# polli-labs/linnaeus

Measured on AMD Instinct MI355X. Metric: images/sec (train fwd+bwd) mFormerV1_sm 3x224x224, higher is better.
Workload: dtype bf16; 1 GPU; mFormerV1_sm train step (forward + 4-task CE loss + backward + AdamW (one HIP launch)), bf16 operands / fp32 accumulate+residual, batch 256/GPU, 3x224x224 synthetic, DropPath 0.2, gradient checkpointing off; per_gpu_batch=256, global_batch=256, parallelism=dp1, grad_mode=direct

## Files before the change

include/lnx.h:

```cpp
#ifndef LNX_H
#define LNX_H
#include <stdint.h>

#ifdef __cplusplus
extern "C" {
#endif

#define LNX_F32 0
#define LNX_BF16 1

const char* lnx_last_error(void);
int lnx_version(void);
int lnx_device_cus(void);
int lnx_set_cu_margin(int cus);

typedef struct lnx_rowmap {
    int group, pad, off;
} lnx_rowmap;

enum { LNX_ACT_NONE = 0, LNX_ACT_GELU = 1, LNX_ACT_RELU = 2, LNX_ACT_GELU_BWD = 3, LNX_ACT_RELU_BWD = 4,
       LNX_ACT_GELU_D = 5, LNX_ACT_MUL_AUX = 6 };
enum { LNX_ADDR_PLAIN = 0, LNX_ADDR_PATCH2 = 1 };

typedef struct lnx_gemm_args {
// ... 238 lines not shown
    int B, Cin, H, W, Cout;
    float eps;
} lnx_stem_args;
int lnx_stem_fwd_ok(int dtype, int Cin, int H, int W, int Cout);
int lnx_stem_fwd(const lnx_stem_args* args, void* stream);

int lnx_scale_cast(const float* in, int64_t ldin, lnx_rowmap in_map, const float* rowscale, int rows_per_sample, void* out,
                   int out_dtype, int64_t ldout, int M, int C, void* stream);

int lnx_layerscale_bwd(const float* g, const void* z, int dtype, const float* gamma, const float* rowscale,
                       int rows_per_sample, void* dz, float* dgamma, int M, int C, void* stream);

int lnx_layerscale_apply_wgrad(const float* s, const float* t, int64_t lds, const float* w, const float* b, int64_t ldw, const float* gamma, float* dw, float* db,
                               int64_t lddw, float* dgamma, int C, int K, void* stream);

int lnx_dropout_mul(void* x, int dtype, const unsigned char* mask, float inv_keep, int M, int C, void* stream);
int lnx_dropout_residual(const void* z, int z_dtype, const unsigned char* mask, float inv_keep, const float* rowscale, int rows_per_sample,
                         const float* res, float* out, int M, int C, void* stream);

int lnx_fill_rows(const float* vec, float* out, int64_t ldout, lnx_rowmap map, int M, int C, void* stream);
int lnx_colsum_rows(const float* in, int64_t ldin, lnx_rowmap map, float* out, int M, int C, void* stream);

int lnx_agg2_fwd(const float* a, const float* b, const float* w2, const float* bias1, float* out, int M, int C, void* stream);
int lnx_agg2_bwd(const float* dout, const float* a, const float* b, const float* w2, float* da, float* db_, float* dw2,
                 float* dbias1, int M, int C, void* stream);

int lnx_pack_meta(const float* meta, int width, int off, int dim, void* out, int dtype, int B, void* stream);

typedef struct lnx_meta_head_args {
    int B, C;
    int dim, off;
    const float* meta;
    int meta_width;
    float eps;
    const float* w0;
    int ldw0;
    const float *b0, *ln0_w, *ln0_b;
    const float* w1;
    int ldw1;
    const float *b1, *ln1_w, *ln1_b;
    const float* w2;
    int ldw2;
    const float *b2, *ln2_w, *ln2_b;
    float* t0;
    float *h0, *x, *h1, *n1, *h2;
    float *m0, *r0, *m1, *r1, *m2, *r2;
    float* tok;
    int64_t tok_row_stride, tok_row_offset;
} lnx_meta_head_args;
int lnx_meta_heads_supported(int C);
int lnx_meta_heads_fwd(const lnx_meta_head_args* heads, int n_heads, void* stream);

typedef struct lnx_meta_head_bwd_args {
    int B, C, dim;
    const float* g;
    int64_t g_row_stride, g_row_offset;
    const float* w1t;
    int ldw1t;
    const float* w2t;
    int ldw2t;
    const float *ln0_w, *ln1_w, *ln2_w;
    const float *t0, *h0, *x, *h1, *n1, *h2, *m0, *r0, *m1, *r1, *m2, *r2;
    float *dp2, *dp1, *dp0;
    float* part;
    float* d_w0;
    float *d_b0, *d_ln0_w, *d_ln0_b;
    float* d_w1;
    float *d_b1, *d_ln1_w, *d_ln1_b;
    float* d_w2;
    float *d_b2, *d_ln2_w, *d_ln2_b;
} lnx_meta_head_bwd_args;
int64_t lnx_meta_heads_bwd_part_floats(int B, int C);
int lnx_meta_heads_bwd(const lnx_meta_head_bwd_args* heads, int n_heads, void* stream);

enum { LNX_PREP_CAST = 0, LNX_PREP_CONV_PERM = 1, LNX_PREP_DW49 = 2 };
typedef struct lnx_prep_desc {
    const float* src;
    void* dst;
    void* dst_t;
    int rows, cols;
    int ld, ld_t;
    int P;
    int mode;
    int block_start;
} lnx_prep_desc;
int lnx_prep_weights(const lnx_prep_desc* descs_dev, int ndesc, int total_blocks, int dtype, void* stream);
int lnx_prep_blocks(int rows, int ld, int cols, int ld_t, int has_t);



typedef struct lnx_softce_args {
    int B, C;
    const float* logits;
    int64_t ld;
    const int64_t* target;
    const float* soft;
    float smoothing;
    const float* class_weight;
    int64_t ignore_index;
    const float* row_scale;
    float scale;
    float* loss;
    float* loss_sum;
    float* dlogits;
    int64_t ldd;
} lnx_softce_args;
int lnx_softce(const lnx_softce_args* args, void* stream);
#define LNX_SOFTCE_MAX_TASKS 8
int lnx_softce_multi(const lnx_softce_args* args, int n, void* stream);

typedef struct lnx_mix_args {
    const float* x;
    const int64_t* perm;
    const unsigned char* valid;
    float* out;
    int B;
    int64_t row;
    int H, W;
    float lam;
    int h0, h1, w0, w1;
    int mode;
} lnx_mix_args;
int lnx_mix_rows(const lnx_mix_args* args, void* stream);
int lnx_mix_meta(const float* aux, const unsigned char* mask, const int64_t* perm, const float* pick, const int* bounds_dev, int nchunk, int B, int D,
                 float* out_aux, unsigned char* out_mask, void* stream);

enum {
    LNX_AUG_CLAMP = 0,
    LNX_AUG_POSTERIZE = 1,
    LNX_AUG_SOLARIZE = 2,
    LNX_AUG_SOLARIZE_ADD = 3,
    LNX_AUG_INVERT = 4,
    LNX_AUG_BRIGHTNESS = 5,
    LNX_AUG_CONTRAST = 6
};
int lnx_aug_pointwise(float* x, int64_t n, int64_t per_image, int op, float p0, float p1, const float* per_image_scalar, void* stream);
int lnx_aug_saturation(float* x, int B, int64_t hw, float factor, void* stream);
int lnx_aug_rowstat(const float* x, int rows, int64_t cols, int kind, float* out, void* stream);
int lnx_aug_rescale(float* x, int64_t rows, int64_t cols, const float* minmax, void* stream);
int lnx_aug_affine(const float* x, float* y, int planes, int H, int W, const float* m6, void* stream);
int lnx_aug_stencil(const float* x, float* y, int planes, int H, int W, const float* taps_dev, int k, int mode, float ratio, void* stream);
int lnx_erase_rects(float* x, int B, int C, int H, int W, const int* rects_dev, const float* values_dev, int n_rects, void* stream);
int lnx_u8hwc_to_f32chw(const unsigned char* src, float* dst, int B, int H, int W, int C, void* stream);

#define LNX_ADAMW_MAX_GROUPS 16
typedef struct lnx_adamw_desc {
    float* p;
    float* m;
    float* v;
    const float* g;
    int64_t n;
    int group;
    int block_start;
} lnx_adamw_desc;
typedef struct lnx_adamw_hyper {
    int ngroups;
    float lr[LNX_ADAMW_MAX_GROUPS], beta1[LNX_ADAMW_MAX_GROUPS], beta2[LNX_ADAMW_MAX_GROUPS], eps[LNX_ADAMW_MAX_GROUPS],
        weight_decay[LNX_ADAMW_MAX_GROUPS];
    float bias_c1[LNX_ADAMW_MAX_GROUPS], bias_c2[LNX_ADAMW_MAX_GROUPS];
    float omb1[LNX_ADAMW_MAX_GROUPS], omb2[LNX_ADAMW_MAX_GROUPS];
} lnx_adamw_hyper;
int lnx_adamw_blocks(int64_t numel);
int lnx_grad_sumsq(const lnx_adamw_desc* descs_dev, int ndesc, int total_blocks, float* out, float* ws, void* stream);
int lnx_adamw_step(const lnx_adamw_desc* descs_dev, int ndesc, int total_blocks, const lnx_adamw_hyper* hyper, const float* sumsq, float max_norm,
                   void* stream);

typedef struct lnx_ademamix_hyper {
    int ngroups;
    float lr[LNX_ADAMW_MAX_GROUPS], beta1[LNX_ADAMW_MAX_GROUPS], beta2[LNX_ADAMW_MAX_GROUPS], eps[LNX_ADAMW_MAX_GROUPS],
        weight_decay[LNX_ADAMW_MAX_GROUPS];
    float bias_c1[LNX_ADAMW_MAX_GROUPS], bias_c2[LNX_ADAMW_MAX_GROUPS];
    float omb1[LNX_ADAMW_MAX_GROUPS], omb2[LNX_ADAMW_MAX_GROUPS];
    float alpha_t[LNX_ADAMW_MAX_GROUPS], beta3_t[LNX_ADAMW_MAX_GROUPS], omb3[LNX_ADAMW_MAX_GROUPS];
} lnx_ademamix_hyper;
int lnx_ademamix_step(const lnx_adamw_desc* descs_dev, float* const* slow_dev, int ndesc, int total_blocks, const lnx_ademamix_hyper* hyper,
                      const float* sumsq, float max_norm, void* stream);

int lnx_gradnorm_sumsq(const lnx_adamw_desc* descs_dev, int ndesc, int total_blocks, int ntasks, int64_t task_stride, float* sumsq, float* norm,
                       float* ws, void* stream);
typedef struct lnx_gradnorm_args {
    int T;
    float alpha;
    const float* norm;
    const float* loss_sum;
    const float* count;
    const float* init_loss;
    float* weights;
    float* initial_losses;
    int* initted;
    float* metrics;
} lnx_gradnorm_args;
int lnx_gradnorm_update(const lnx_gradnorm_args* args, void* stream);

enum { LNX_METRICS_CHAIN_N = 0, LNX_METRICS_CHAIN_CORRECT, LNX_METRICS_PARTIAL_N, LNX_METRICS_PARTIAL_CORRECT, LNX_METRICS_SUBSET_OOR ,
       LNX_METRICS_HEAD = 8 };
enum { LNX_METRICS_N = 0, LNX_METRICS_CORRECT1, LNX_METRICS_CORRECT3, LNX_METRICS_NULL_N, LNX_METRICS_NULL_CORRECT1, LNX_METRICS_NONNULL_N,
       LNX_METRICS_NONNULL_CORRECT1, LNX_METRICS_LOSS_N, LNX_METRICS_TASK_STRIDE = 8 };
enum { LNX_METRICS_SUM_LOSS = 0, LNX_METRICS_SUM_NULL_LOSS, LNX_METRICS_SUM_NONNULL_LOSS, LNX_METRICS_SUM_STRIDE = 4 };
#define LNX_METRICS_TASK(t) (LNX_METRICS_HEAD + LNX_METRICS_TASK_STRIDE * (t))
#define LNX_METRICS_SUBSET(n_tasks, n_bins0, s) (LNX_METRICS_TASK(n_tasks) + ((s) ? 2 * (int64_t)(n_tasks) * (n_bins0) : 0))
#define LNX_METRICS_SUM(t) (LNX_METRICS_SUM_STRIDE * (t))
typedef struct lnx_metrics_task {
    const void* logits;
    int64_t ld;
    const int64_t* target;
    const unsigned char* is_null;
    const float* loss;
    int C;
} lnx_metrics_task;
typedef struct lnx_metrics_args {
    int dtype;
    int B, n_tasks;
    lnx_metrics_task task[LNX_SOFTCE_MAX_TASKS];
    const int64_t* subset_ids[2];
    int n_bins[2];
    int64_t* counts;
    double* sums;
} lnx_metrics_args;
int lnx_metrics_table_sizes(int n_tasks, int n_bins0, int n_bins1, int64_t* n_counts, int64_t* n_sums);
int lnx_metrics_update(const lnx_metrics_args* args, void* stream);

#define LNX_PREDICT_MAX_K 16
typedef struct lnx_predict_task {
    const void* logits;
    int64_t ld;
    int C;
    const int32_t* parent;
    int null_index;
    const int64_t* id_map;
} lnx_predict_task;
typedef struct lnx_predict_args {
    int dtype;
    int B, n_tasks;
    int K;
    int consistency;
    const int32_t* k_per_sample;
    lnx_predict_task task[LNX_SOFTCE_MAX_TASKS];
    int64_t* ids;
    float* probs;
    int32_t* count;
    int32_t* flags;
} lnx_predict_args;
int lnx_predict(const lnx_predict_args* args, void* stream);

int lnx_convmlp_supported(int dtype, int C);
typedef struct lnx_convmlp_args {
    int dtype, M, C;
    const void* ln;
    const void* w1;
    const float* b1;
    const void* w2;
    const float* b2;
    const float* gamma;
    const float* rowscale;
    int rows_per_sample;
    const float* x;
    float* out;
    void* z;
    const void* y;
    const float* ln_w;
    const float* ln_b;
    float ln_eps;
    void* ln_out;
    float* mean;
    float* rstd;
} lnx_convmlp_args;
int lnx_convmlp_fwd(const lnx_convmlp_args* args, void* stream);

typedef struct lnx_convmlp_bwd_args {
    int dtype, M, C;
    const float* g;
    const void* ln;
    const void* z;
    const void* w1;
    const float* b1;
    const void* w2t;
    const void* w1t;
    const float* gamma;
    const float* rowscale;
    int rows_per_sample;
    void* act;
    void* dh;
    void* dz;
    void* dln;
    float* dgamma;
    const void* y;
    const float* ln_w;
    const float* mean;
    const float* rstd;
    float* d_ln_w;
    float* d_ln_b;
    float* ws;
    int64_t ws_floats;
    int dz_plain;
    int ln_defer;
} lnx_convmlp_bwd_args;
int lnx_convmlp_bwd(const lnx_convmlp_bwd_args* args, void* stream);
int64_t lnx_convmlp_bwd_ws_floats(int C, int M);


#define LNX_MAX_META 8
#define LNX_MAX_TASKS 16
typedef struct lnx_mformer_cfg {
    int dtype;
    int batch, img_h, img_w, in_chans;
    int dims[4];
    int conv_depths[2];
    int rope_depths[2];
    int rope_heads[2];
    int mlp_hidden[2];
    int n_meta;
    int meta_dims[LNX_MAX_META];
    int only_last_cls;
    int n_tasks;
    int task_classes[LNX_MAX_TASKS];
    int inference;
    int recompute;
    int fp8;
    int rope_mode;
} lnx_mformer_cfg;

typedef struct lnx_plan lnx_plan;
int lnx_plan_create(const lnx_mformer_cfg* cfg, lnx_plan** out);
void lnx_plan_destroy(lnx_plan* p);
int64_t lnx_plan_workspace_bytes(const lnx_plan* p);
int lnx_plan_num_params(const lnx_plan* p);
const char* lnx_plan_param_name(const lnx_plan* p, int i);
int64_t lnx_plan_param_numel(const lnx_plan* p, int i);
int lnx_plan_num_drop_calls(const lnx_plan* p);
int64_t lnx_plan_logits_numel(const lnx_plan* p);
int64_t lnx_plan_logits_offset(const lnx_plan* p, int task);
int lnx_plan_logits_ld(const lnx_plan* p, int task);
int lnx_plan_bind(lnx_plan* p, const float* const* params, float* const* grads, void* workspace);
int lnx_plan_forward(lnx_plan* p, const float* x, const float* meta, const float* drop_scales, const unsigned char* drop_mask,
                     float* feats, float* logits, void* stream);
int64_t lnx_plan_dropout_bytes(const lnx_plan* p);
int lnx_plan_set_dropout(lnx_plan* p, const unsigned char* masks, float drop_rate);
int64_t lnx_plan_attn_dropout_bytes(const lnx_plan* p);
int lnx_plan_set_attn_dropout(lnx_plan* p, const unsigned char* masks, float drop_rate);
int lnx_plan_backward(lnx_plan* p, const float* dlogits, const float* dfeats, int segment, void* stream);
int lnx_plan_backward_into(lnx_plan* p, const float* dlogits, const float* dfeats, float* const* grads, void* stream);
#define LNX_PROFILE_CLASSES 8
int lnx_plan_profile_begin(lnx_plan* p);
int lnx_plan_profile_end(lnx_plan* p, double* ms, double* work, int* launches);
#define LNX_PROFILE_CLASSES_EX 10
int lnx_plan_profile_begin_spans(lnx_plan* p);
int lnx_plan_profile_end_ex(lnx_plan* p, double* ms, double* work, double* bytes, int* launches);
int lnx_plan_set_wgrad_stream(lnx_plan* p, int on);
int lnx_plan_set_meta_stream(lnx_plan* p, int mode);
int lnx_plan_segment_params(const lnx_plan* p, int segment, int* idx_out, int max_out);

#ifdef __cplusplus
}
#endif
#endif
```

linnaeus_amd/_lib.py:

```python
from __future__ import annotations

import ctypes as C
import os

_HERE = os.path.dirname(os.path.abspath(__file__))
LIB_PATH = os.environ.get("LNX_LIB_PATH") or os.path.join(_HERE, "liblnx_hip.so")

F32, BF16 = 0, 1
ACT_NONE, ACT_GELU, ACT_RELU, ACT_GELU_BWD, ACT_RELU_BWD, ACT_GELU_D, ACT_MUL_AUX = 0, 1, 2, 3, 4, 5, 6
TN_WS_FLOATS = 256 * (256 * 128 + 256)
ADDR_PLAIN, ADDR_PATCH2 = 0, 1


class LnxError(RuntimeError):
    pass


class RowMap(C.Structure):
    _fields_ = [("group", C.c_int), ("pad", C.c_int), ("off", C.c_int)]


class GemmArgs(C.Structure):
    _fields_ = [
        ("dtype", C.c_int), ("M", C.c_int), ("N", C.c_int), ("K", C.c_int),
        ("A", C.c_void_p), ("lda", C.c_int64),
        ("W", C.c_void_p), ("ldw", C.c_int64),
        ("C", C.c_void_p), ("ldc", C.c_int64),
        ("out_f32", C.c_int),
        ("a_mode", C.c_int), ("Hin", C.c_int), ("Win", C.c_int), ("Cin", C.c_int),
        ("c_mode", C.c_int), ("c_map", RowMap),
        ("bias", C.c_void_p),
        ("c2", C.c_void_p), ("ldc2", C.c_int64),
        ("act", C.c_int),
        ("aux", C.c_void_p), ("ldaux", C.c_int64),
        ("gamma", C.c_void_p), ("rowscale", C.c_void_p), ("rows_per_sample", C.c_int),
        ("res", C.c_void_p), ("ldres", C.c_int64),
        ("c8", C.c_void_p), ("ldc8", C.c_int64), ("c8_scales", C.c_void_p),
    ]


class WgradArgs(C.Structure):
    _fields_ = [
        ("dtype", C.c_int), ("M", C.c_int), ("N", C.c_int), ("K", C.c_int),
        ("dY", C.c_void_p), ("lddy", C.c_int64),
        ("A", C.c_void_p), ("lda", C.c_int64),
        ("a_mode", C.c_int), ("Hin", C.c_int), ("Win", C.c_int), ("Cin", C.c_int),
        ("dW", C.c_void_p), ("lddw", C.c_int64),
        ("k_perm_c", C.c_int),
        ("db", C.c_void_p),
        ("splits", C.c_int),
        ("k_store", C.c_int),
        ("ws", C.c_void_p), ("ws_floats", C.c_int64),
        ("defer", C.c_int),
    ]


class SoftCEArgs(C.Structure):
    _fields_ = [
        ("B", C.c_int), ("C", C.c_int),
        ("logits", C.c_void_p), ("ld", C.c_int64),
        ("target", C.c_void_p),
        ("soft", C.c_void_p), ("smoothing", C.c_float),
        ("class_weight", C.c_void_p),
        ("ignore_index", C.c_int64),
        ("row_scale", C.c_void_p), ("scale", C.c_float),
        ("loss", C.c_void_p), ("loss_sum", C.c_void_p),
        ("dlogits", C.c_void_p), ("ldd", C.c_int64),
    ]


ADAMW_MAX_GROUPS = 16


class AdamWDesc(C.Structure):
    _fields_ = [("p", C.c_void_p), ("m", C.c_void_p), ("v", C.c_void_p), ("g", C.c_void_p), ("n", C.c_int64), ("group", C.c_int), ("block_start", C.c_int)]


class AdamWHyper(C.Structure):
    _fields_ = [("ngroups", C.c_int)] + [(k, C.c_float * ADAMW_MAX_GROUPS) for k in ("lr", "beta1", "beta2", "eps", "weight_decay", "bias_c1", "bias_c2", "omb1", "omb2")]


class AdEMAMixHyper(C.Structure):
    _fields_ = [("ngroups", C.c_int)] + [(k, C.c_float * ADAMW_MAX_GROUPS) for k in ("lr", "beta1", "beta2", "eps", "weight_decay", "bias_c1", "bias_c2", "omb1", "omb2",
                                                                                  "alpha_t", "beta3_t", "omb3")]


class GradNormArgs(C.Structure):
    _fields_ = [("T", C.c_int), ("alpha", C.c_float), ("norm", C.c_void_p), ("loss_sum", C.c_void_p), ("count", C.c_void_p), ("init_loss", C.c_void_p),
                ("weights", C.c_void_p), ("initial_losses", C.c_void_p), ("initted", C.c_void_p), ("metrics", C.c_void_p)]


METRICS_MAX_TASKS = 8
METRICS_CHAIN_N, METRICS_CHAIN_CORRECT, METRICS_PARTIAL_N, METRICS_PARTIAL_CORRECT, METRICS_SUBSET_OOR = range(5)
METRICS_HEAD = 8
METRICS_N, METRICS_CORRECT1, METRICS_CORRECT3, METRICS_NULL_N, METRICS_NULL_CORRECT1, METRICS_NONNULL_N, METRICS_NONNULL_CORRECT1, METRICS_LOSS_N = range(8)
METRICS_TASK_STRIDE = 8
METRICS_SUM_LOSS, METRICS_SUM_NULL_LOSS, METRICS_SUM_NONNULL_LOSS = range(3)
METRICS_SUM_STRIDE = 4


def metrics_task(t: int) -> int:
    return METRICS_HEAD + METRICS_TASK_STRIDE * t


def metrics_subset(n_tasks: int, n_bins0: int, s: int) -> int:
    return metrics_task(n_tasks) + (2 * n_tasks * n_bins0 if s else 0)


class MetricsTask(C.Structure):
    _fields_ = [("logits", C.c_void_p), ("ld", C.c_int64), ("target", C.c_void_p), ("is_null", C.c_void_p), ("loss", C.c_void_p), ("C", C.c_int)]


class MetricsArgs(C.Structure):
    _fields_ = [("dtype", C.c_int), ("B", C.c_int), ("n_tasks", C.c_int), ("task", MetricsTask * METRICS_MAX_TASKS),
                ("subset_ids", C.c_void_p * 2), ("n_bins", C.c_int * 2), ("counts", C.c_void_p), ("sums", C.c_void_p)]


PREDICT_MAX_K = 16


class PredictTask(C.Structure):
    _fields_ = [("logits", C.c_void_p), ("ld", C.c_int64), ("C", C.c_int), ("parent", C.c_void_p), ("null_index", C.c_int), ("id_map", C.c_void_p)]


class PredictArgs(C.Structure):
    _fields_ = [("dtype", C.c_int), ("B", C.c_int), ("n_tasks", C.c_int), ("K", C.c_int), ("consistency", C.c_int), ("k_per_sample", C.c_void_p),
                ("task", PredictTask * METRICS_MAX_TASKS), ("ids", C.c_void_p), ("probs", C.c_void_p), ("count", C.c_void_p), ("flags", C.c_void_p)]


_lib = None


def lib() -> C.CDLL:
    global _lib
    if _lib is None:
        if not os.path.exists(LIB_PATH):
            raise LnxError(
                f"{LIB_PATH} is missing: build it with `python -c 'import __graft_entry__ as g; g.build()'` "
                "(or `make -C linnaeus_amd/csrc`). linnaeus_amd has no CPU fallback."
            )
        _lib = C.CDLL(LIB_PATH)
        _lib.lnx_last_error.restype = C.c_char_p
        _lib.lnx_nt_kernel_launches.restype = C.c_int64
        _lib.lnx_convmlp_bwd_ws_floats.restype = C.c_int64
        _lib.lnx_meta_heads_bwd_part_floats.restype = C.c_int64
        if hasattr(_lib, "lnx_ademamix_step"):
            _lib.lnx_ademamix_step.argtypes = [C.c_void_p, C.c_void_p, C.c_int, C.c_int, C.POINTER(AdEMAMixHyper), C.c_void_p, C.c_float, C.c_void_p]
        if hasattr(_lib, "lnx_gradnorm_sumsq"):
            _lib.lnx_gradnorm_sumsq.argtypes = [C.c_void_p, C.c_int, C.c_int, C.c_int, C.c_int64, C.c_void_p, C.c_void_p, C.c_void_p, C.c_void_p]
        if hasattr(_lib, "lnx_metrics_update"):
            _lib.lnx_metrics_update.argtypes = [C.POINTER(MetricsArgs), C.c_void_p]
            _lib.lnx_metrics_table_sizes.argtypes = [C.c_int, C.c_int, C.c_int, C.POINTER(C.c_int64), C.POINTER(C.c_int64)]
        if hasattr(_lib, "lnx_predict"):
            _lib.lnx_predict.argtypes = [C.POINTER(PredictArgs), C.c_void_p]
            _lib.lnx_predict.restype = C.c_int
        older = bool(os.environ.get("LNX_LIB_PATH")) and os.environ.get("LNX_LIB_OLDER") == "1"
        for name in EXPORTS:
            if not hasattr(_lib, name) and not older:
                raise LnxError(f"{LIB_PATH} does not export {name}; rebuild it")
    return _lib


def check(rc: int, what: str) -> None:
    if rc != 0:
        raise LnxError(f"{what} failed (rc={rc}): {lib().lnx_last_error().decode()}")


AUG_CLAMP, AUG_POSTERIZE, AUG_SOLARIZE, AUG_SOLARIZE_ADD, AUG_INVERT, AUG_BRIGHTNESS, AUG_CONTRAST = range(7)

NT_KERNEL_NONE, NT_KERNEL_V1, NT_KERNEL_V2, NT_KERNEL_SKINNY, NT_KERNEL_V4, NT_KERNEL_FP8, NT_KERNEL_V7, NT_KERNEL_MX8, NT_KERNEL_V9, NT_KERNEL_EXPERIMENT = 0, 1, 2, 3, 4, 6, 7, 8, 9, 15

ROPE_COS, ROPE_ROTATE = 0, 1

ATTN_KERNEL_NONE, ATTN_KERNEL_RES4, ATTN_KERNEL_RES8, ATTN_KERNEL_TILED4, ATTN_KERNEL_TILED8 = range(5)

EXPORTS = [
    "lnx_last_error", "lnx_version", "lnx_device_cus", "lnx_set_cu_margin",
    "lnx_gemm_nt", "lnx_last_nt_kernel", "lnx_nt_kernel_launches", "lnx_nt_dispatch", "lnx_gemm_tn", "lnx_gemm_tn_flush", "lnx_gemm_tn_discard", "lnx_amax", "lnx_quantize_fp8", "lnx_gemm_nt_fp8", "lnx_quantize_mxfp8", "lnx_gemm_nt_mxfp8", "lnx_dropout_mul", "lnx_dropout_residual", "lnx_plan_dropout_bytes", "lnx_plan_set_dropout", "lnx_plan_attn_dropout_bytes", "lnx_plan_set_attn_dropout",
    "lnx_layernorm_fwd", "lnx_layernorm_bwd", "lnx_layernorm_bwd_flush", "lnx_layernorm_bwd_discard",
    "lnx_dwconv7_fwd", "lnx_dwconv7_wgrad",
    "lnx_gemm_nt_group_ok", "lnx_gemm_nt_group", "lnx_rope_cos_table", "lnx_rope_cos_table_hd", "lnx_rope_cossin_table_hd", "lnx_rope_cos_tables", "lnx_attn_bwd_ws_floats", "lnx_attn_bwd_ws_floats_hd", "lnx_attn_fwd", "lnx_attn_bwd", "lnx_attn_bwd_flush", "lnx_attn_bwd_discard", "lnx_attn_dispatch", "lnx_last_attn_kernel",
    "lnx_im2col_stem", "lnx_scale_cast", "lnx_layerscale_bwd", "lnx_layerscale_apply_wgrad", "lnx_fill_rows", "lnx_colsum_rows",
    "lnx_agg2_fwd", "lnx_agg2_bwd", "lnx_pack_meta", "lnx_meta_heads_supported", "lnx_meta_heads_fwd", "lnx_meta_heads_bwd", "lnx_meta_heads_bwd_part_floats", "lnx_prep_weights", "lnx_prep_blocks", "lnx_softce", "lnx_softce_multi", "lnx_stem_fwd", "lnx_stem_fwd_ok", "lnx_adamw_blocks", "lnx_grad_sumsq", "lnx_adamw_step", "lnx_ademamix_step", "lnx_gradnorm_sumsq", "lnx_gradnorm_update",
    "lnx_metrics_table_sizes", "lnx_metrics_update", "lnx_predict",
    "lnx_mix_rows", "lnx_mix_meta",
    "lnx_aug_pointwise", "lnx_aug_saturation", "lnx_aug_rowstat", "lnx_aug_rescale", "lnx_aug_affine", "lnx_aug_stencil", "lnx_erase_rects", "lnx_u8hwc_to_f32chw",
    "lnx_convmlp_supported", "lnx_convmlp_fwd", "lnx_convmlp_bwd", "lnx_convmlp_bwd_ws_floats",
    "lnx_plan_create", "lnx_plan_destroy", "lnx_plan_workspace_bytes", "lnx_plan_num_params", "lnx_plan_param_name",
    "lnx_plan_param_numel", "lnx_plan_num_drop_calls", "lnx_plan_logits_numel", "lnx_plan_logits_offset", "lnx_plan_logits_ld",
    "lnx_plan_bind", "lnx_plan_forward", "lnx_plan_backward", "lnx_plan_backward_into", "lnx_plan_segment_params", "lnx_plan_profile_begin", "lnx_plan_profile_end", "lnx_plan_profile_begin_spans", "lnx_plan_profile_end_ex", "lnx_plan_set_wgrad_stream", "lnx_plan_set_meta_stream",
]


class MetaHeadArgs(C.Structure):
    _fields_ = [
        ("B", C.c_int), ("C", C.c_int), ("dim", C.c_int), ("off", C.c_int),
        ("meta", C.c_void_p), ("meta_width", C.c_int), ("eps", C.c_float),
        ("w0", C.c_void_p), ("ldw0", C.c_int), ("b0", C.c_void_p), ("ln0_w", C.c_void_p), ("ln0_b", C.c_void_p),
        ("w1", C.c_void_p), ("ldw1", C.c_int), ("b1", C.c_void_p), ("ln1_w", C.c_void_p), ("ln1_b", C.c_void_p),
        ("w2", C.c_void_p), ("ldw2", C.c_int), ("b2", C.c_void_p), ("ln2_w", C.c_void_p), ("ln2_b", C.c_void_p),
        ("t0", C.c_void_p), ("h0", C.c_void_p), ("x", C.c_void_p), ("h1", C.c_void_p), ("n1", C.c_void_p), ("h2", C.c_void_p),
        ("m0", C.c_void_p), ("r0", C.c_void_p), ("m1", C.c_void_p), ("r1", C.c_void_p), ("m2", C.c_void_p), ("r2", C.c_void_p),
        ("tok", C.c_void_p), ("tok_row_stride", C.c_int64), ("tok_row_offset", C.c_int64),
    ]


class MetaHeadBwdArgs(C.Structure):
    _fields_ = [
        ("B", C.c_int), ("C", C.c_int), ("dim", C.c_int),
        ("g", C.c_void_p), ("g_row_stride", C.c_int64), ("g_row_offset", C.c_int64),
        ("w1t", C.c_void_p), ("ldw1t", C.c_int), ("w2t", C.c_void_p), ("ldw2t", C.c_int),
        ("ln0_w", C.c_void_p), ("ln1_w", C.c_void_p), ("ln2_w", C.c_void_p),
        ("t0", C.c_void_p), ("h0", C.c_void_p), ("x", C.c_void_p), ("h1", C.c_void_p), ("n1", C.c_void_p), ("h2", C.c_void_p),
        ("m0", C.c_void_p), ("r0", C.c_void_p), ("m1", C.c_void_p), ("r1", C.c_void_p), ("m2", C.c_void_p), ("r2", C.c_void_p),
        ("dp2", C.c_void_p), ("dp1", C.c_void_p), ("dp0", C.c_void_p), ("part", C.c_void_p),
        ("d_w0", C.c_void_p), ("d_b0", C.c_void_p), ("d_ln0_w", C.c_void_p), ("d_ln0_b", C.c_void_p),
        ("d_w1", C.c_void_p), ("d_b1", C.c_void_p), ("d_ln1_w", C.c_void_p), ("d_ln1_b", C.c_void_p),
        ("d_w2", C.c_void_p), ("d_b2", C.c_void_p), ("d_ln2_w", C.c_void_p), ("d_ln2_b", C.c_void_p),
    ]


class LnArgs(C.Structure):
    _fields_ = [
        ("M", C.c_int), ("C", C.c_int), ("eps", C.c_float),
        ("x", C.c_void_p), ("x_dtype", C.c_int), ("ldx", C.c_int64), ("x_map", RowMap),
        ("w", C.c_void_p), ("b", C.c_void_p),
        ("y", C.c_void_p), ("y_dtype", C.c_int), ("ldy", C.c_int64), ("y_map", RowMap),
        ("add", C.c_void_p), ("ldadd", C.c_int64),
        ("mean", C.c_void_p), ("rstd", C.c_void_p),
        ("y8", C.c_void_p), ("ldy8", C.c_int64), ("y8_scales", C.c_void_p),
    ]


class LnBwdArgs(C.Structure):
    _fields_ = [
        ("M", C.c_int), ("C", C.c_int),
        ("dy", C.c_void_p), ("dy_dtype", C.c_int), ("lddy", C.c_int64), ("dy_map", RowMap),
        ("x", C.c_void_p), ("x_dtype", C.c_int), ("ldx", C.c_int64), ("x_map", RowMap),
        ("w", C.c_void_p), ("mean", C.c_void_p), ("rstd", C.c_void_p),
        ("gin", C.c_void_p), ("ldgin", C.c_int64),
        ("dx", C.c_void_p), ("dx_dtype", C.c_int), ("lddx", C.c_int64),
        ("dw", C.c_void_p), ("db", C.c_void_p), ("relu_mask", C.c_int),
        ("ws", C.c_void_p), ("ws_floats", C.c_int64),
        ("dx2", C.c_void_p), ("dx2_dtype", C.c_int), ("lddx2", C.c_int64), ("dx2_rowscale", C.c_void_p), ("dx2_rows_per_sample", C.c_int),
        ("dx2_8", C.c_void_p), ("dx2_8_scales", C.c_void_p), ("lddx2_8", C.c_int64),
        ("defer", C.c_int),
    ]


class RopeTable(C.Structure):
    _fields_ = [
        ("freqs", C.c_void_p), ("cos_out", C.c_void_p), ("dsin_out", C.c_void_p),
        ("heads", C.c_int), ("H", C.c_int), ("W", C.c_int), ("head_dim", C.c_int),
        ("rope_mode", C.c_int), ("sin_out", C.c_void_p),
    ]


class DwconvArgs(C.Structure):
    _fields_ = [
        ("B", C.c_int), ("H", C.c_int), ("W", C.c_int), ("C", C.c_int),
        ("x", C.c_void_p), ("x_dtype", C.c_int), ("w49", C.c_void_p), ("bias", C.c_void_p),
        ("flip", C.c_int), ("res", C.c_void_p), ("y", C.c_void_p), ("y_dtype", C.c_int),
    ]


class DwconvWgradArgs(C.Structure):
    _fields_ = [
        ("B", C.c_int), ("H", C.c_int), ("W", C.c_int), ("C", C.c_int),
        ("x", C.c_void_p), ("x_dtype", C.c_int), ("dy", C.c_void_p), ("dy_dtype", C.c_int),
        ("dw", C.c_void_p), ("db", C.c_void_p),
    ]


class AttnArgs(C.Structure):
    _fields_ = [
        ("dtype", C.c_int), ("B", C.c_int), ("N", C.c_int), ("E", C.c_int), ("heads", C.c_int),
        ("qkv", C.c_void_p), ("cos_tab", C.c_void_p), ("o", C.c_void_p), ("lse", C.c_void_p),
        ("drop_mask", C.c_void_p), ("drop_inv_keep", C.c_float), ("head_dim", C.c_int),
        ("rope_mode", C.c_int), ("sin_tab", C.c_void_p),
    ]


class AttnBwdArgs(C.Structure):
    _fields_ = [
        ("dtype", C.c_int), ("B", C.c_int), ("N", C.c_int), ("E", C.c_int), ("heads", C.c_int),
        ("qkv", C.c_void_p), ("cos_tab", C.c_void_p), ("o", C.c_void_p), ("lse", C.c_void_p),
        ("d_o", C.c_void_p), ("dqkv", C.c_void_p), ("freq_ws", C.c_void_p), ("delta", C.c_void_p),
        ("drop_mask", C.c_void_p), ("drop_inv_keep", C.c_float),
        ("dsin_tab", C.c_void_p), ("dfreqs", C.c_void_p), ("defer_freqs", C.c_int), ("head_dim", C.c_int),
        ("rope_mode", C.c_int), ("sin_tab", C.c_void_p), ("grid_w", C.c_int),
    ]


class PrepDesc(C.Structure):
    _fields_ = [
        ("src", C.c_void_p), ("dst", C.c_void_p), ("dst_t", C.c_void_p),
        ("rows", C.c_int), ("cols", C.c_int), ("ld", C.c_int), ("ld_t", C.c_int),
        ("P", C.c_int), ("mode", C.c_int), ("block_start", C.c_int),
    ]


PREP_CAST, PREP_CONV_PERM, PREP_DW49 = 0, 1, 2


class ConvMlpArgs(C.Structure):
    _fields_ = [
        ("dtype", C.c_int), ("M", C.c_int), ("C", C.c_int),
        ("ln", C.c_void_p), ("w1", C.c_void_p), ("b1", C.c_void_p), ("w2", C.c_void_p), ("b2", C.c_void_p),
        ("gamma", C.c_void_p), ("rowscale", C.c_void_p), ("rows_per_sample", C.c_int),
        ("x", C.c_void_p), ("out", C.c_void_p), ("z", C.c_void_p),
        ("y", C.c_void_p), ("ln_w", C.c_void_p), ("ln_b", C.c_void_p), ("ln_eps", C.c_float), ("ln_out", C.c_void_p),
        ("mean", C.c_void_p), ("rstd", C.c_void_p),
    ]


class ConvMlpBwdArgs(C.Structure):
    _fields_ = [
        ("dtype", C.c_int), ("M", C.c_int), ("C", C.c_int),
        ("g", C.c_void_p), ("ln", C.c_void_p), ("z", C.c_void_p), ("w1", C.c_void_p), ("b1", C.c_void_p),
        ("w2t", C.c_void_p), ("w1t", C.c_void_p), ("gamma", C.c_void_p), ("rowscale", C.c_void_p), ("rows_per_sample", C.c_int),
        ("act", C.c_void_p), ("dh", C.c_void_p), ("dz", C.c_void_p), ("dln", C.c_void_p), ("dgamma", C.c_void_p),
        ("y", C.c_void_p), ("ln_w", C.c_void_p), ("mean", C.c_void_p), ("rstd", C.c_void_p), ("d_ln_w", C.c_void_p), ("d_ln_b", C.c_void_p),
        ("ws", C.c_void_p), ("ws_floats", C.c_int64),
        ("dz_plain", C.c_int), ("ln_defer", C.c_int),
    ]


class StemArgs(C.Structure):
    _fields_ = [("x", C.c_void_p), ("w", C.c_void_p), ("bias", C.c_void_p), ("ln_w", C.c_void_p), ("ln_b", C.c_void_p), ("patches", C.c_void_p),
                ("pre", C.c_void_p), ("y", C.c_void_p), ("mean", C.c_void_p), ("rstd", C.c_void_p), ("B", C.c_int), ("Cin", C.c_int), ("H", C.c_int),
                ("W", C.c_int), ("Cout", C.c_int), ("eps", C.c_float)]


class MixArgs(C.Structure):
    _fields_ = [
        ("x", C.c_void_p), ("perm", C.c_void_p), ("valid", C.c_void_p), ("out", C.c_void_p),
        ("B", C.c_int), ("row", C.c_int64), ("H", C.c_int), ("W", C.c_int), ("lam", C.c_float),
        ("h0", C.c_int), ("h1", C.c_int), ("w0", C.c_int), ("w1", C.c_int), ("mode", C.c_int),
    ]
```

linnaeus_amd/csrc/optim.hip:

```cpp
#include "common.hpp"
#include "../../include/lnx.h"

namespace {

constexpr int OPT_ELEMS = 4096;

__device__ __forceinline__ int find_desc_index(const lnx_adamw_desc* __restrict__ descs, int ndesc, int block) {
    int lo = 0, hi = ndesc - 1;
    while (lo < hi) {
        const int mid = (lo + hi + 1) >> 1;
        if (descs[mid].block_start <= block) lo = mid;
        else hi = mid - 1;
    }
    return lo;
}

__device__ __forceinline__ const lnx_adamw_desc& find_desc(const lnx_adamw_desc* __restrict__ descs, int ndesc, int block) {
    return descs[find_desc_index(descs, ndesc, block)];
}

__global__ __launch_bounds__(256) void grad_sumsq_kernel(const lnx_adamw_desc* __restrict__ descs, int ndesc, float* __restrict__ part) {
    __shared__ float red[4];
    const lnx_adamw_desc& d = find_desc(descs, ndesc, blockIdx.x);
    const int64_t base = (int64_t)(blockIdx.x - d.block_start) * OPT_ELEMS;
    const int64_t end = min(d.n, base + OPT_ELEMS);
    float s = 0.f;
    if ((reinterpret_cast<uintptr_t>(d.g) & 15) == 0) {
        for (int64_t i = base + 4 * threadIdx.x; i + 3 < end; i += 1024) {
            const float4 v = *reinterpret_cast<const float4*>(d.g + i);
            s += v.x * v.x + v.y * v.y + v.z * v.z + v.w * v.w;
        }
        const int64_t tail = base + ((end - base) & ~(int64_t)3);
        if (tail + threadIdx.x < end) {
            const float v = d.g[tail + threadIdx.x];
            s += v * v;
        }
    } else {
        for (int64_t i = base + threadIdx.x; i < end; i += 256) s += d.g[i] * d.g[i];
    }
    s = wave_sum(s);
    if ((threadIdx.x & 63) == 0) red[threadIdx.x >> 6] = s;
    __syncthreads();
    if (threadIdx.x == 0) part[blockIdx.x] = (red[0] + red[1]) + (red[2] + red[3]);
}

__global__ __launch_bounds__(1024) void grad_sumsq_fold_kernel(const float* __restrict__ part, int n, float* __restrict__ out) {
    __shared__ float red[16];
    float s0 = 0.f, s1 = 0.f, s2 = 0.f, s3 = 0.f;
    int i = threadIdx.x;
    for (; i + 3 * 1024 < n; i += 4 * 1024) {
        s0 += part[i];
        s1 += part[i + 1024];
        s2 += part[i + 2048];
        s3 += part[i + 3072];
    }
    for (; i < n; i += 1024) s0 += part[i];
    float s = wave_sum((s0 + s1) + (s2 + s3));
    if ((threadIdx.x & 63) == 0) red[threadIdx.x >> 6] = s;
    __syncthreads();
    if (threadIdx.x == 0) {
        float t = 0.f;
#pragma unroll
        for (int k = 0; k < 16; ++k) t += red[k];
        *out = t;
    }
}

__global__ __launch_bounds__(256) void adamw_kernel(const lnx_adamw_desc* __restrict__ descs, int ndesc, const lnx_adamw_hyper h, const float* __restrict__ sumsq,
                                                    float max_norm) {
    const lnx_adamw_desc& d = find_desc(descs, ndesc, blockIdx.x);
    const int gi = d.group;
    const float lr = h.lr[gi], b1 = h.beta1[gi], b2 = h.beta2[gi], eps = h.eps[gi], wd = h.weight_decay[gi];
    const float omb1 = h.omb1[gi], omb2 = h.omb2[gi];
    const float step_size = lr / h.bias_c1[gi], inv_sqrt_bc2 = 1.0f / sqrtf(h.bias_c2[gi]);
    float coef = 1.0f;
    if (sumsq != nullptr && max_norm > 0.f) coef = fminf(1.0f, max_norm / (sqrtf(*sumsq) + 1e-6f));
    const int64_t base = (int64_t)(blockIdx.x - d.block_start) * OPT_ELEMS;
    const int64_t end = min(d.n, base + OPT_ELEMS);
    auto upd = [&](float g, float& p, float& m, float& v) __attribute__((always_inline)) {
        g *= coef;
        p *= 1.0f - lr * wd;
        m = fmaf(b1, m, omb1 * g);
        v = fmaf(b2, v, omb2 * g * g);
        const float denom = sqrtf(v) * inv_sqrt_bc2 + eps;
        p -= step_size * (m / denom);
    };
    const bool vec = ((reinterpret_cast<uintptr_t>(d.p) | reinterpret_cast<uintptr_t>(d.g) | reinterpret_cast<uintptr_t>(d.m) | reinterpret_cast<uintptr_t>(d.v)) & 15) == 0;
    int64_t done = base;
    if (vec) {
        constexpr int R = OPT_ELEMS / 1024;
        float4 g4[R], p4[R], m4[R], v4[R];
        const int64_t full = base + ((end - base) & ~(int64_t)3);
#pragma unroll
        for (int r = 0; r < R; ++r) {
            const int64_t i = base + 1024 * r + 4 * threadIdx.x;
            const int64_t ic = i + 3 < full ? i : base;
            if (full > base) {
                g4[r] = *reinterpret_cast<const float4*>(d.g + ic);
                p4[r] = *reinterpret_cast<const float4*>(d.p + ic);
                m4[r] = *reinterpret_cast<const float4*>(d.m + ic);
                v4[r] = *reinterpret_cast<const float4*>(d.v + ic);
            }
        }
        if (full > base) {
#pragma unroll
            for (int r = 0; r < R; ++r) {
                const int64_t i = base + 1024 * r + 4 * threadIdx.x;
                if (i + 3 < full) {
                    upd(g4[r].x, p4[r].x, m4[r].x, v4[r].x);
                    upd(g4[r].y, p4[r].y, m4[r].y, v4[r].y);
                    upd(g4[r].z, p4[r].z, m4[r].z, v4[r].z);
                    upd(g4[r].w, p4[r].w, m4[r].w, v4[r].w);
                    *reinterpret_cast<float4*>(d.p + i) = p4[r];
                    *reinterpret_cast<float4*>(d.m + i) = m4[r];
                    *reinterpret_cast<float4*>(d.v + i) = v4[r];
                }
            }
        }
        done = full;
    }
    for (int64_t i = done + threadIdx.x; i < end; i += 256) {
        float p = d.p[i], m = d.m[i], v = d.v[i];
        upd(d.g[i], p, m, v);
        d.p[i] = p;
        d.m[i] = m;
        d.v[i] = v;
    }
}

__global__ __launch_bounds__(256) void ademamix_kernel(const lnx_adamw_desc* __restrict__ descs, float* const* __restrict__ slow, int ndesc,
                                                       const lnx_ademamix_hyper h, const float* __restrict__ sumsq, float max_norm) {
    const int di = find_desc_index(descs, ndesc, blockIdx.x);
    const lnx_adamw_desc& d = descs[di];
    float* const m3p = slow[di];
    const int gi = d.group;
    const float lr = h.lr[gi], b1 = h.beta1[gi], b2 = h.beta2[gi], eps = h.eps[gi], nlrwd = -(lr * h.weight_decay[gi]);
    const float omb1 = h.omb1[gi], omb2 = h.omb2[gi], b3 = h.beta3_t[gi], omb3 = h.omb3[gi], alpha = h.alpha_t[gi];
    const float step_size = lr / h.bias_c1[gi], sqrt_bc2 = sqrtf(h.bias_c2[gi]);
    float coef = 1.0f;
    if (sumsq != nullptr && max_norm > 0.f) coef = fminf(1.0f, max_norm / (sqrtf(*sumsq) + 1e-6f));
    const int64_t base = (int64_t)(blockIdx.x - d.block_start) * OPT_ELEMS;
    const int64_t end = min(d.n, base + OPT_ELEMS);
    auto upd = [&](float g, float& p, float& m, float& v, float& s) __attribute__((always_inline)) {
        g *= coef;
        p = fmaf(nlrwd, p, p);
        m = fmaf(b1, m, omb1 * g);
        v = fmaf(b2, v, omb2 * g * g);
        s = fmaf(b3, s, omb3 * g);
        const float denom = sqrtf(v) / sqrt_bc2 + eps;
        p -= step_size * (fmaf(alpha, s, m) / denom);
    };
    const bool vec = ((reinterpret_cast<uintptr_t>(d.p) | reinterpret_cast<uintptr_t>(d.g) | reinterpret_cast<uintptr_t>(d.m) | reinterpret_cast<uintptr_t>(d.v) |
                       reinterpret_cast<uintptr_t>(m3p)) & 15) == 0;
    int64_t done = base;
    if (vec) {
        constexpr int R = OPT_ELEMS / 1024;
        float4 g4[R], p4[R], m4[R], v4[R], s4[R];
        const int64_t full = base + ((end - base) & ~(int64_t)3);
#pragma unroll
        for (int r = 0; r < R; ++r) {
            const int64_t i = base + 1024 * r + 4 * threadIdx.x;
            const int64_t ic = i + 3 < full ? i : base;
            if (full > base) {
                g4[r] = *reinterpret_cast<const float4*>(d.g + ic);
                p4[r] = *reinterpret_cast<const float4*>(d.p + ic);
                m4[r] = *reinterpret_cast<const float4*>(d.m + ic);
                v4[r] = *reinterpret_cast<const float4*>(d.v + ic);
                s4[r] = *reinterpret_cast<const float4*>(m3p + ic);
            }
        }
        if (full > base) {
#pragma unroll
            for (int r = 0; r < R; ++r) {
                const int64_t i = base + 1024 * r + 4 * threadIdx.x;
                if (i + 3 < full) {
                    upd(g4[r].x, p4[r].x, m4[r].x, v4[r].x, s4[r].x);
                    upd(g4[r].y, p4[r].y, m4[r].y, v4[r].y, s4[r].y);
                    upd(g4[r].z, p4[r].z, m4[r].z, v4[r].z, s4[r].z);
                    upd(g4[r].w, p4[r].w, m4[r].w, v4[r].w, s4[r].w);
                    *reinterpret_cast<float4*>(d.p + i) = p4[r];
                    *reinterpret_cast<float4*>(d.m + i) = m4[r];
                    *reinterpret_cast<float4*>(d.v + i) = v4[r];
                    *reinterpret_cast<float4*>(m3p + i) = s4[r];
                }
            }
        }
        done = full;
    }
    for (int64_t i = done + threadIdx.x; i < end; i += 256) {
        float p = d.p[i], m = d.m[i], v = d.v[i], s = m3p[i];
        upd(d.g[i], p, m, v, s);
        d.p[i] = p;
        d.m[i] = m;
        d.v[i] = v;
        m3p[i] = s;
    }
}

}

extern "C" int lnx_adamw_blocks(int64_t numel) { return (int)((numel + OPT_ELEMS - 1) / OPT_ELEMS); }

extern "C" int lnx_grad_sumsq(const lnx_adamw_desc* descs_dev, int ndesc, int total_blocks, float* out, float* ws, void* stream) {
    LNX_CHECK(descs_dev && ndesc > 0 && total_blocks > 0 && out && ws, "lnx_grad_sumsq: bad arguments (ws: total_blocks floats)");
    hipStream_t st = (hipStream_t)stream;
    hipLaunchKernelGGL(grad_sumsq_kernel, dim3(total_blocks), dim3(256), 0, st, descs_dev, ndesc, ws);
    hipLaunchKernelGGL(grad_sumsq_fold_kernel, dim3(1), dim3(1024), 0, st, ws, total_blocks, out);
    LNX_LAUNCH_CHECK();
    return 0;
}

extern "C" int lnx_adamw_step(const lnx_adamw_desc* descs_dev, int ndesc, int total_blocks, const lnx_adamw_hyper* hyper, const float* sumsq, float max_norm,
                              void* stream) {
    LNX_CHECK(descs_dev && ndesc > 0 && total_blocks > 0 && hyper, "lnx_adamw_step: bad arguments");
    LNX_CHECK(hyper->ngroups > 0 && hyper->ngroups <= LNX_ADAMW_MAX_GROUPS, "lnx_adamw_step: ngroups=%d (max %d)", hyper->ngroups, LNX_ADAMW_MAX_GROUPS);
    for (int i = 0; i < hyper->ngroups; ++i)
        LNX_CHECK(hyper->bias_c1[i] > 0.f && hyper->bias_c2[i] > 0.f, "lnx_adamw_step: bias corrections of group %d must be positive (step >= 1)", i);
    hipLaunchKernelGGL(adamw_kernel, dim3(total_blocks), dim3(256), 0, (hipStream_t)stream, descs_dev, ndesc, *hyper, sumsq, max_norm);
    LNX_LAUNCH_CHECK();
    return 0;
}

extern "C" int lnx_ademamix_step(const lnx_adamw_desc* descs_dev, float* const* slow_dev, int ndesc, int total_blocks, const lnx_ademamix_hyper* hyper,
                                 const float* sumsq, float max_norm, void* stream) {
    LNX_CHECK(descs_dev && slow_dev && ndesc > 0 && total_blocks > 0 && hyper, "lnx_ademamix_step: bad arguments");
    LNX_CHECK(hyper->ngroups > 0 && hyper->ngroups <= LNX_ADAMW_MAX_GROUPS, "lnx_ademamix_step: ngroups=%d (max %d)", hyper->ngroups, LNX_ADAMW_MAX_GROUPS);
    for (int i = 0; i < hyper->ngroups; ++i)
        LNX_CHECK(hyper->bias_c1[i] > 0.f && hyper->bias_c2[i] > 0.f, "lnx_ademamix_step: bias corrections of slot %d must be positive (step >= 1)", i);
    hipLaunchKernelGGL(ademamix_kernel, dim3(total_blocks), dim3(256), 0, (hipStream_t)stream, descs_dev, slow_dev, ndesc, *hyper, sumsq, max_norm);
    LNX_LAUNCH_CHECK();
    return 0;
}
```

linnaeus_amd/csrc/plan.cpp:

```cpp
#include <hip/hip_runtime.h>
#include <stdlib.h>
#include <string.h>

#include <mutex>
#include <atomic>
#include <string>
#include <vector>

#include "../../include/lnx.h"

void lnx_set_error(const char* fmt, ...);

#define RUN(expr)                  \
    do {                           \
        const int rc_ = (expr);    \
        if (rc_ != 0) return rc_;  \
    } while (0)
#define FAIL(...)                   \
    do {                            \
        lnx_set_error(__VA_ARGS__); \
        return 1;                   \
    } while (0)
#define HIPRUN(expr)                                                         \
    do {                                                                     \
        const hipError_t e_ = (expr);                                        \
        if (e_ != hipSuccess) FAIL("%s: %s", #expr, hipGetErrorString(e_)); \
    } while (0)

namespace {

constexpr int LN_DEFER_SLOTS = 16;
constexpr int FREQ_DEFER_SLOTS = 8;

inline int64_t align_up(int64_t v, int64_t a) { return (v + a - 1) / a * a; }

struct OpW {
    int param = -1;
    int N = 0, K = 0;
    int ld = 0;
    int ld_t = 0;
    int mode = LNX_PREP_CAST, P = 0;
    bool f32 = false;
    int64_t off = 0, off_t = 0;
    int64_t off8 = 0, off8s = 0;
    int64_t off8t = 0, off8ts = 0;
};

struct ConvBlk {
    bool fused = false;
    bool fused_ln = false;
    bool keep_z = true;
    int gamma, dww, dwb, lnw, lnb, b1, b2;
    OpW w1, w2;
    int64_t w49;
    int64_t xin, y, ln, mean, rstd, hpre, act, z;
};
struct RopeBlk {
    int n1w, n1b, n2w, n2b, freqs, qkvb, projb, fc1b, fc2b;
    OpW qkv, proj, fc1, fc2;
    int64_t xin, n1, mean1, rstd1, qkvbuf, cos, dsin, o, lse, xmid, n2, mean2, rstd2, hpre, act;
    int64_t dm_proj = 0, dm_hid = 0, dm_fc2 = 0;
    int64_t dm_attn = 0;
};
struct MetaHead {
    int b0, lnw0, lnb0, nf1w, nf1b, nf2w, nf2b, b1, b2;
    OpW w0, w1, w2;
    int dim, off;
    int64_t t0, h0, x, m0, r0, h1, n1, m1, r1, h2, m2, r2;
    int64_t dp2 = 0, dp1 = 0, dp0 = 0, part = 0;
};
struct Down {
    int lnw, lnb, cb;
    OpW w;
    int64_t ln, mean, rstd;
};

}

constexpr int TN_WS_SLOTS = 4;

struct lnx_plan {
    lnx_mformer_cfg c;
    int esz;
    int E;
    int H[4], W[4], HW[4];
    int N2, N3;
    std::vector<std::string> names;
    std::vector<int64_t> numel;
    std::vector<const float*> P;
    std::vector<float*> G;
    bool bound = false, has_grads = false, fwd_done = false;
    unsigned char* ws = nullptr;
    int64_t ws_bytes = 0;

    int stem_b, stem_lnw, stem_lnb, cls[2], norm_w[2], norm_b[2], fin_w, fin_b, agg_w, agg_b, cl_b1, cl_b2, cl_lnw, cl_lnb;
    OpW stem_w, cl_w1, cl_w2;
    std::vector<int> head_b;
    std::vector<OpW> head_w;
    std::vector<int> logit_ld;
    std::vector<int64_t> logit_off;
    int64_t logits_numel = 0;
    Down down[3];
    std::vector<ConvBlk> conv[2];
    std::vector<RopeBlk> rope[2];
    std::vector<MetaHead> meta[2];
    std::vector<OpW*> all_w;
    std::vector<int> drop_conv[2], drop_attn[2], drop_mlp[2];
    int n_drop = 0;

    int64_t o_descs = 0, n_descs = 0, prep_blocks = 0;
    int64_t n_descs_t = 0, n_descs_f = 0, prep_blocks_f = 0;
    int64_t o_patches, o_stem_pre, o_stem_mean, o_stem_rstd;
    int64_t o_stage_out[4];
    int64_t o_tok[2];
    int64_t o_t1, o_t1_mean, o_t1_rstd;
    int64_t o_cl_hpre, o_cl_act, o_cl_u, o_cl_mean, o_cl_rstd, o_c1n;
    int64_t o_c2n, o_n2_mean, o_n2_rstd, o_agg, o_fin_mean, o_fin_rstd, o_feats, o_featsT;
    int64_t o_g[4];
    int64_t o_sA, o_sB = 0, o_sC, o_sD;
    int64_t o_lnws = 0, lnws_floats = 0, o_lnws_side = 0, lnws_side_floats = 0;
    int64_t lnws_defer_floats = 0;
    int64_t o_lnws_defer = 0;
    int ln_pending = 0;
    int64_t gcos_floats = 0;
    int freq_pending = 0;
    bool freq_defer = true;
    bool ln_defer = true;
    int64_t o_tnws = 0;
    int64_t o_lsws = 0, lsws_floats = 0;
    int64_t o_gcos , o_delta, o_dt1, o_tail[6], o_mtmp[4], o_dlT;
    int64_t o_a8 = 0, o_a8s = 0, o_h8 = 0, o_h8s = 0;
    const float* last_drop = nullptr;
    const unsigned char* last_mask = nullptr;
    std::vector<unsigned char> mask_host;
    const float* last_meta = nullptr;
    int resident[4] = {-1, -1, -1, -1};
    const unsigned char* dmask = nullptr;
    float inv_keep = 1.0f;
    int64_t dmask_bytes = 0;
    const unsigned char* amask = nullptr;
    float a_inv_keep = 1.0f;
    int64_t amask_bytes = 0;
    hipStream_t side = nullptr;
    hipEvent_t ev_fork = nullptr, ev_meta = nullptr, ev_bfork[2] = {nullptr, nullptr}, ev_bjoin[2] = {nullptr, nullptr};
    hipStream_t wgs = nullptr;
    bool wgs_on = true;
    bool meta_forked[2] = {false, false};
    int meta_mode = 1;
    bool meta_chain = true;
    bool chain_ok[2] = {false, false};
    bool dy8_ready = false;
    hipEvent_t ev_wf[4] = {nullptr, nullptr, nullptr, nullptr}, ev_wj[4] = {nullptr, nullptr, nullptr, nullptr};
    bool profile = false;
    bool profile_spans = false;
    struct Span { hipEvent_t e0, e1; int cls; double work, bytes; };
    std::vector<Span> spans;
    std::vector<hipEvent_t> ev_pool;
    size_t ev_used = 0;

    template <typename U> U* at(int64_t off) const { return reinterpret_cast<U*>(ws + off); }
    const float* drop_ptr(int call) const {
        if (last_drop == nullptr || call < 0 || !mask_host[call]) return nullptr;
        return last_drop + (int64_t)call * c.batch;
    }
};

namespace {

int find_param(const lnx_plan* p, const std::string& n) {
    for (size_t i = 0; i < p->names.size(); ++i)
        if (p->names[i] == n) return (int)i;
    return -1;
}

void add_param(lnx_plan* p, const std::string& n, int64_t numel) {
    p->names.push_back(n);
    p->numel.push_back(numel);
}

void build_inventory(lnx_plan* p) {
    const lnx_mformer_cfg& c = p->c;
    const int* D = c.dims;
    char b[128];
    add_param(p, "cls_token_1", D[2]);
    add_param(p, "cls_token_2", D[3]);
    add_param(p, "stem.0.weight", (int64_t)D[0] * c.in_chans * 16);
    add_param(p, "stem.0.bias", D[0]);
    add_param(p, "stem.1.weight", D[0]);
    add_param(p, "stem.1.bias", D[0]);
    for (int i = 0; i < 3; ++i) {
        snprintf(b, sizeof b, "downsample_layers.%d.", i);
        const std::string pre(b);
        add_param(p, pre + "norm.weight", D[i]);
        add_param(p, pre + "norm.bias", D[i]);
        add_param(p, pre + "conv.weight", (int64_t)D[i + 1] * D[i] * 4);
        add_param(p, pre + "conv.bias", D[i + 1]);
    }
    for (int s = 0; s < 2; ++s)
        for (int i = 0; i < c.conv_depths[s]; ++i) {
            snprintf(b, sizeof b, "stages.%d.%d.", s, i);
            const std::string pre(b);
            const int64_t C = D[s];
            add_param(p, pre + "gamma", C);
            add_param(p, pre + "dwconv.weight", C * 49);
            add_param(p, pre + "dwconv.bias", C);
            add_param(p, pre + "norm.weight", C);
            add_param(p, pre + "norm.bias", C);
            add_param(p, pre + "pwconv1.weight", 4 * C * C);
            add_param(p, pre + "pwconv1.bias", 4 * C);
            add_param(p, pre + "pwconv2.weight", 4 * C * C);
            add_param(p, pre + "pwconv2.bias", C);
        }
    for (int s = 0; s < 2; ++s)
        for (int i = 0; i < c.rope_depths[s]; ++i) {
            snprintf(b, sizeof b, "stages.%d.%d.", s + 2, i);
            const std::string pre(b);
            const int64_t C = D[2 + s], hid = c.mlp_hidden[s];
            add_param(p, pre + "norm1.weight", C);
            add_param(p, pre + "norm1.bias", C);
            add_param(p, pre + "norm2.weight", C);
            add_param(p, pre + "norm2.bias", C);
            add_param(p, pre + "attn.freqs", C);
            add_param(p, pre + "attn.qkv.weight", 3 * C * C);
            add_param(p, pre + "attn.qkv.bias", 3 * C);
            add_param(p, pre + "attn.proj.weight", C * C);
            add_param(p, pre + "attn.proj.bias", C);
            add_param(p, pre + "mlp.fc1.weight", hid * C);
            add_param(p, pre + "mlp.fc1.bias", hid);
            add_param(p, pre + "mlp.fc2.weight", C * hid);
            add_param(p, pre + "mlp.fc2.bias", C);
        }
    add_param(p, "norm_1.weight", D[2]);
    add_param(p, "norm_1.bias", D[2]);
    add_param(p, "norm_2.weight", D[3]);
    add_param(p, "norm_2.bias", D[3]);
    for (int m = 0; m < c.n_meta; ++m)
        for (int s = 0; s < 2; ++s) {
            snprintf(b, sizeof b, "meta.%d.head_%d.", m, s + 1);
            const std::string pre(b);
            const int64_t C = D[2 + s];
            add_param(p, pre + "0.weight", C * c.meta_dims[m]);
            add_param(p, pre + "0.bias", C);
            add_param(p, pre + "2.weight", C);
            add_param(p, pre + "2.bias", C);
            add_param(p, pre + "3.norm_fn1.weight", C);
            add_param(p, pre + "3.norm_fn1.bias", C);
            add_param(p, pre + "3.norm_fn2.weight", C);
            add_param(p, pre + "3.norm_fn2.bias", C);
            add_param(p, pre + "3.w1.weight", C * C);
            add_param(p, pre + "3.w1.bias", C);
            add_param(p, pre + "3.w2.weight", C * C);
            add_param(p, pre + "3.w2.bias", C);
        }
    if (!c.only_last_cls) {
        add_param(p, "cl_1_fc.0.fc1.weight", (int64_t)D[2] * D[2]);
        add_param(p, "cl_1_fc.0.fc1.bias", D[2]);
        add_param(p, "cl_1_fc.0.fc2.weight", (int64_t)D[3] * D[2]);
        add_param(p, "cl_1_fc.0.fc2.bias", D[3]);
        add_param(p, "cl_1_fc.1.weight", D[3]);
        add_param(p, "cl_1_fc.1.bias", D[3]);
        add_param(p, "aggregate.weight", 2);
        add_param(p, "aggregate.bias", 1);
    }
    add_param(p, "final_norm.weight", D[3]);
// ... 413 lines not shown
        }
        p->o_lnws_side = cv.take(p->lnws_side_floats * 4);
        p->o_tnws = cv.take((int64_t)LNX_TN_WS_FLOATS * 4 * TN_WS_SLOTS);
        {
            const int64_t cmax = D[0] > D[1] ? D[0] : D[1];
            p->lsws_floats = cmax * 4 * cmax + cmax;
            p->o_lsws = cv.take(p->lsws_floats * 4);
        }
        p->o_sA = cv.take(maxM4C * esz);
        if (any_fused) p->o_sB = cv.take(maxM4C * esz);
        p->o_sC = cv.take(maxMC * esz);
        p->o_sD = cv.take(maxMC * esz);
    }
    if (!inf) {
        int64_t gmax = 0, dmax = 0;
        for (int s = 0; s < 2; ++s) {
            const int N = s == 0 ? p->N2 : p->N3;
            const int64_t gsz = lnx_attn_bwd_ws_floats_hd(B, N, c.rope_heads[s], D[2 + s] / c.rope_heads[s]) * 4;
            const int64_t dsz = (int64_t)B * c.rope_heads[s] * N * 4;
            if (gsz > gmax) gmax = gsz;
            if (dsz > dmax) dmax = dsz;
        }
        p->gcos_floats = gmax / 4;
        p->o_gcos = cv.take(gmax * FREQ_DEFER_SLOTS);
        p->o_delta = cv.take(dmax);
    }
    for (int s = 0; s < 2; ++s) {
        const int64_t M = (int64_t)B * (s == 0 ? p->N2 : p->N3), C = D[2 + s], hid = c.mlp_hidden[s];
        for (auto& k : p->rope[s]) {
            k.dm_proj = p->dmask_bytes;
            k.dm_hid = k.dm_proj + M * C;
            k.dm_fc2 = k.dm_hid + M * hid;
            p->dmask_bytes = k.dm_fc2 + M * C;
            const int64_t N = s == 0 ? p->N2 : p->N3;
            k.dm_attn = p->amask_bytes;
            p->amask_bytes += (int64_t)B * c.rope_heads[s] * N * ((N + 63) / 64 * 64);
        }
    }
    p->ws_bytes = cv.cur;
    *out = p;
    return 0;
}

extern "C" int64_t lnx_plan_dropout_bytes(const lnx_plan* p) { return p ? p->dmask_bytes : 0; }
extern "C" int64_t lnx_plan_attn_dropout_bytes(const lnx_plan* p) { return p ? p->amask_bytes : 0; }

extern "C" int lnx_plan_set_attn_dropout(lnx_plan* p, const unsigned char* masks, float drop_rate) {
    if (!p) FAIL("lnx_plan_set_attn_dropout: null plan");
    if (masks == nullptr || drop_rate == 0.0f) {
        p->amask = nullptr;
        p->a_inv_keep = 1.0f;
        return 0;
    }
    if (!(drop_rate > 0.0f && drop_rate < 1.0f)) FAIL("lnx_plan_set_attn_dropout: drop_rate %g must be in [0, 1)", (double)drop_rate);
    if (p->c.inference) FAIL("lnx_plan_set_attn_dropout: dropout is a training-time operation; this is an inference plan");
    if ((((uintptr_t)masks) & 3) != 0) FAIL("lnx_plan_set_attn_dropout: the mask buffer must be 4-byte aligned");
    p->amask = masks;
    p->a_inv_keep = 1.0f / (1.0f - drop_rate);
    return 0;
}

extern "C" int lnx_plan_set_dropout(lnx_plan* p, const unsigned char* masks, float drop_rate) {
    if (!p) FAIL("lnx_plan_set_dropout: null plan");
    if (masks == nullptr || drop_rate == 0.0f) {
        p->dmask = nullptr;
        p->inv_keep = 1.0f;
        return 0;
    }
    if (!(drop_rate > 0.0f && drop_rate < 1.0f)) FAIL("lnx_plan_set_dropout: drop_rate %g must be in [0, 1)", (double)drop_rate);
    if (p->c.inference) FAIL("lnx_plan_set_dropout: dropout is a training-time operation; this is an inference plan");
    if (p->c.fp8) FAIL("lnx_plan_set_dropout: dropout is not available on fp8 plans");
    if ((((uintptr_t)masks) & 7) != 0) FAIL("lnx_plan_set_dropout: the mask buffer must be 8-byte aligned");
    p->dmask = masks;
    p->inv_keep = 1.0f / (1.0f - drop_rate);
    return 0;
}

static hipStream_t shared_stream(int which) {
    static std::mutex mu;
    static hipStream_t tab[2][64] = {};
    int dev = 0;
    if (hipGetDevice(&dev) != hipSuccess || dev < 0 || dev >= 64) return nullptr;
    std::lock_guard<std::mutex> lock(mu);
    if (!tab[which][dev] && hipStreamCreateWithFlags(&tab[which][dev], hipStreamNonBlocking) != hipSuccess) tab[which][dev] = nullptr;
    return tab[which][dev];
}

extern "C" void lnx_plan_destroy(lnx_plan* p) {
    if (!p) return;
    (void)lnx_gemm_tn_discard();
    (void)lnx_layernorm_bwd_discard();
    if (p->side) {
        (void)hipStreamSynchronize(p->side);
        (void)hipEventDestroy(p->ev_fork);
        (void)hipEventDestroy(p->ev_meta);
        for (int i = 0; i < 2; ++i) {
            (void)hipEventDestroy(p->ev_bfork[i]);
            (void)hipEventDestroy(p->ev_bjoin[i]);
        }
    }
    if (p->wgs) {
        (void)hipStreamSynchronize(p->wgs);
        for (int i = 0; i < 4; ++i) {
            (void)hipEventDestroy(p->ev_wf[i]);
            (void)hipEventDestroy(p->ev_wj[i]);
        }
    }
    for (hipEvent_t e : p->ev_pool) (void)hipEventDestroy(e);
    delete p;
}
extern "C" int64_t lnx_plan_workspace_bytes(const lnx_plan* p) { return p ? p->ws_bytes : 0; }
extern "C" int lnx_plan_num_params(const lnx_plan* p) { return p ? (int)p->names.size() : 0; }
extern "C" const char* lnx_plan_param_name(const lnx_plan* p, int i) {
    return (p && i >= 0 && i < (int)p->names.size()) ? p->names[i].c_str() : nullptr;
}
extern "C" int64_t lnx_plan_param_numel(const lnx_plan* p, int i) { return (p && i >= 0 && i < (int)p->numel.size()) ? p->numel[i] : -1; }
extern "C" int lnx_plan_num_drop_calls(const lnx_plan* p) { return p ? p->n_drop : 0; }
extern "C" int64_t lnx_plan_logits_numel(const lnx_plan* p) { return p ? p->logits_numel : 0; }
extern "C" int64_t lnx_plan_logits_offset(const lnx_plan* p, int t) { return (p && t >= 0 && t < p->c.n_tasks) ? p->logit_off[t] : -1; }
extern "C" int lnx_plan_logits_ld(const lnx_plan* p, int t) { return (p && t >= 0 && t < p->c.n_tasks) ? p->logit_ld[t] : -1; }

extern "C" int lnx_plan_bind(lnx_plan* p, const float* const* params, float* const* grads, void* workspace) {
    if (!p || !params || !workspace) FAIL("lnx_plan_bind: null argument");
    {
        static std::atomic<int> bound_dev{-1};
        int dev = -1;
        HIPRUN(hipGetDevice(&dev));
        int expect = -1;
        if (!bound_dev.compare_exchange_strong(expect, dev) && expect != dev)
            FAIL("lnx_plan_bind: this process already runs plans on device %d, now device %d is current: the library is one-process-per-GPU", expect, dev);
    }
    const int n = (int)p->names.size();
    p->P.assign(params, params + n);
    for (int i = 0; i < n; ++i)
        if (p->P[i] == nullptr || (((uintptr_t)p->P[i]) & 3) != 0) FAIL("lnx_plan_bind: parameter %s is null or misaligned", p->names[i].c_str());
    p->has_grads = grads != nullptr;
    if (grads) {
        p->G.assign(grads, grads + n);
        for (int i = 0; i < n; ++i)
            if (p->G[i] == nullptr) FAIL("lnx_plan_bind: gradient of %s is null", p->names[i].c_str());
    } else {
        p->G.assign(n, nullptr);
    }
    p->ws = reinterpret_cast<unsigned char*>(workspace);
    if ((((uintptr_t)p->ws) & 255) != 0) FAIL("lnx_plan_bind: workspace must be 256-byte aligned");
    int64_t arena_end = 0;
    for (OpW* w : p->all_w) {
        const int wes = w->f32 ? 4 : 2;
        const int64_t e1 = w->off + (int64_t)w->N * w->ld * wes;
        const int64_t e2 = w->ld_t ? w->off_t + (int64_t)w->K * w->ld_t * wes : 0;
        if (e1 > arena_end) arena_end = e1;
        if (e2 > arena_end) arena_end = e2;
    }
    HIPRUN(hipMemset(p->ws, 0, (size_t)arena_end));
    std::vector<lnx_prep_desc> d;
    int blk = 0;
    auto push_w = [&](OpW* w) {
        lnx_prep_desc e;
        memset(&e, 0, sizeof e);
        e.src = p->P[w->param];
        e.dst = p->ws + w->off;
        e.dst_t = w->ld_t ? p->ws + w->off_t : nullptr;
        e.rows = w->N;
        e.cols = w->K;
        e.ld = w->ld;
        e.ld_t = w->ld_t;
        e.P = w->P;
        e.mode = w->mode;
        e.block_start = blk;
        blk += lnx_prep_blocks(e.rows, e.ld, e.cols, e.ld_t, e.dst_t != nullptr);
        d.push_back(e);
    };
    const bool split = p->esz == 2;
    for (OpW* w : p->all_w)
        if (!split || !w->f32) push_w(w);
    for (int s = 0; s < 2; ++s)
        for (auto& k : p->conv[s]) {
            lnx_prep_desc e;
            memset(&e, 0, sizeof e);
            e.src = p->P[k.dww];
            e.dst = p->ws + k.w49;
            e.rows = p->c.dims[s];
            e.cols = 49;
            e.ld = 49;
            e.mode = LNX_PREP_DW49;
            e.block_start = blk;
            blk += lnx_prep_blocks(e.rows, e.ld, e.cols, 0, 0);
            d.push_back(e);
        }
    p->n_descs_t = (int64_t)d.size();
    p->prep_blocks = blk;
    blk = 0;
    if (split)
        for (OpW* w : p->all_w)
            if (w->f32) push_w(w);
    p->n_descs_f = (int64_t)d.size() - p->n_descs_t;
    p->prep_blocks_f = blk;
    if (getenv("LNX_NO_SIDE_STREAM") != nullptr) p->meta_mode = 0;
    if (const char* e = getenv("LNX_META_STREAM")) p->meta_mode = atoi(e) < 0 || atoi(e) > 2 ? 1 : atoi(e);
    if (p->side == nullptr && p->c.n_meta > 0 && getenv("LNX_NO_SIDE_STREAM") == nullptr) {
        p->side = shared_stream(0);
        if (!p->side) FAIL("lnx_plan: no side stream");
        HIPRUN(hipEventCreateWithFlags(&p->ev_fork, hipEventDisableTiming));
        HIPRUN(hipEventCreateWithFlags(&p->ev_meta, hipEventDisableTiming));
        for (int i = 0; i < 2; ++i) {
            HIPRUN(hipEventCreateWithFlags(&p->ev_bfork[i], hipEventDisableTiming));
            HIPRUN(hipEventCreateWithFlags(&p->ev_bjoin[i], hipEventDisableTiming));
        }
    }
    if (p->wgs == nullptr && !(getenv("LNX_WGRAD_STREAM") && atoi(getenv("LNX_WGRAD_STREAM")) == 0)) {
        p->wgs = shared_stream(1);
        if (!p->wgs) FAIL("lnx_plan: no weight-gradient stream");
        for (int i = 0; i < 4; ++i) {
            HIPRUN(hipEventCreateWithFlags(&p->ev_wf[i], hipEventDisableTiming));
            HIPRUN(hipEventCreateWithFlags(&p->ev_wj[i], hipEventDisableTiming));
        }
    }
    HIPRUN(hipMemcpy(p->ws + p->o_descs, d.data(), d.size() * sizeof(lnx_prep_desc), hipMemcpyHostToDevice));
    HIPRUN(hipDeviceSynchronize());
    p->bound = true;
    p->fwd_done = false;
    return 0;
}

namespace {

hipStream_t meta_stream(const lnx_plan* p) {
    if (p->c.n_meta <= 0 || p->meta_mode == 0) return nullptr;
    if (p->meta_mode == 2 && p->chain_ok[0] && p->chain_ok[1] && p->wgs != nullptr) return p->wgs;
    return p->side;
}

struct Ctx {
    lnx_plan* p;
    void* st;
    int dt;
    template <typename U> U* at(int64_t off) const { return p->at<U>(off); }
    const void* wptr(const OpW& w) const { return p->ws + w.off; }
    const void* wtptr(const OpW& w) const { return p->ws + w.off_t; }
};

hipEvent_t take_event(lnx_plan* p) {
    if (p->ev_used == p->ev_pool.size()) {
        hipEvent_t e;
        (void)hipEventCreate(&e);
        p->ev_pool.push_back(e);
    }
    return p->ev_pool[p->ev_used++];
}
struct Timed {
    lnx_plan* p;
    hipStream_t st;
    bool on;
    lnx_plan::Span sp;
    Timed(const Ctx& c, int cls, double work, double bytes = 0.0)
        : p(c.p), st((hipStream_t)c.st), on(cls >= 0 && (cls >= 8 ? c.p->profile_spans : (c.p->profile && !c.p->profile_spans))) {
        if (on) {
            sp.cls = cls;
            sp.work = work;
            sp.bytes = bytes;
            sp.e0 = take_event(p);
            sp.e1 = take_event(p);
            (void)hipEventRecord(sp.e0, st);
        }
    }
    ~Timed() {
        if (on) {
            (void)hipEventRecord(sp.e1, st);
            p->spans.push_back(sp);
        }
    }
};
double nt_bytes(const Ctx& c, const lnx_gemm_args* a, int a_elem = 0) {
    const double e = c.p->esz, ea = a_elem ? a_elem : e, mn = (double)a->M * a->N;
    return ea * ((double)a->M * a->K + (double)a->N * a->K) + (a->out_f32 ? 4.0 : e) * mn + (a->c2 ? e * mn : 0.0) + (a->aux ? e * mn : 0.0) +
           (a->res ? 4.0 * mn : 0.0) + (a->c8 ? mn * (1.0 + 1.0 / 32) : 0.0);
}
int gemm_nt_t(const Ctx& c, const lnx_gemm_args* a) {
    Timed t(c, a->M >= 1024 ? 0 : -1, 2.0 * a->M * a->N * a->K, nt_bytes(c, a));
    return lnx_gemm_nt(a, c.st);
}

int heads_nt(const Ctx& c, lnx_gemm_args* hg, int n, bool accumulate) {
    static const bool off = getenv("LNX_HEADS_GROUP") != nullptr && atoi(getenv("LNX_HEADS_GROUP")) == 0;
    int gmax = LNX_GEMM_GROUP_MAX;
    if (const char* e = getenv("LNX_HEADS_GROUP_MAX")) {
        const int v = atoi(e);
        if (v >= 1 && v < gmax) gmax = v;
    }
    for (int t0 = 0; t0 < n; t0 += gmax) {
        const int m = n - t0 < gmax ? n - t0 : gmax;
        lnx_gemm_args* g = hg + t0;
        if (accumulate && t0 > 0) {
            g[0].C = hg[0].C; g[0].ldc = hg[0].ldc; g[0].res = (const float*)hg[0].C; g[0].ldres = hg[0].ldc;
        }
        if (!off && lnx_gemm_nt_group_ok(g, m, accumulate ? 1 : 0)) {
            RUN(lnx_gemm_nt_group(g, m, accumulate ? 1 : 0, c.st));
            continue;
        }
        for (int t = 0; t < m; ++t) {
            lnx_gemm_args a = g[t];
            if (accumulate && t > 0) {
                a.C = g[0].C; a.ldc = g[0].ldc; a.res = (const float*)g[0].C; a.ldres = g[0].ldc;
            }
            RUN(gemm_nt_t(c, &a));
        }
    }
    return 0;
}

lnx_gemm_args gemm_base(const Ctx& c, int M, int N, int K, const void* A, int64_t lda, const void* W, int64_t ldw, void* C, int64_t ldc, bool out_f32) {
    lnx_gemm_args a;
    memset(&a, 0, sizeof a);
    a.dtype = c.dt;
    a.M = M;
    a.N = N;
    a.K = K;
    a.A = A;
    a.lda = lda;
    a.W = W;
    a.ldw = ldw;
    a.C = C;
    a.ldc = ldc;
    a.out_f32 = out_f32 ? 1 : 0;
    return a;
}

int ln_fwd(const Ctx& c, int M, int C, float eps, const void* x, int xdt, int64_t ldx, lnx_rowmap xm, int wi, int bi, void* y, int ydt, int64_t ldy,
           lnx_rowmap ym, const void* add, int64_t ldadd, float* mean, float* rstd, void* y8 = nullptr, void* y8s = nullptr) {
    lnx_ln_args a;
    memset(&a, 0, sizeof a);
    a.y8 = y8; a.ldy8 = C; a.y8_scales = y8s;
    a.M = M; a.C = C; a.eps = eps;
    a.x = x; a.x_dtype = xdt; a.ldx = ldx; a.x_map = xm;
    a.w = c.p->P[wi]; a.b = c.p->P[bi];
    a.y = y; a.y_dtype = ydt; a.ldy = ldy; a.y_map = ym;
    a.add = add; a.ldadd = ldadd; a.mean = mean; a.rstd = rstd;
    return lnx_layernorm_fwd(&a, c.st);
}

struct Dx2 {
    void* p = nullptr;
    const float* rowscale = nullptr;
    int rps = 0;
    void* p8 = nullptr;
    void* p8s = nullptr;
};
int ln_bwd(const Ctx& c, int M, int C, const void* dy, int dydt, int64_t lddy, lnx_rowmap dym, const void* x, int xdt, int64_t ldx, lnx_rowmap xm, int wi,
           int bi, const float* mean, const float* rstd, const float* gin, void* dx, int dxdt, int64_t lddx, bool relu, Dx2 d2 = Dx2()) {
    lnx_ln_bwd_args a;
    memset(&a, 0, sizeof a);
    a.dx2 = d2.p; a.dx2_dtype = c.dt; a.lddx2 = C; a.dx2_rowscale = d2.rowscale; a.dx2_rows_per_sample = d2.rps;
    if (d2.p && d2.p8) {
        a.dx2_8 = d2.p8; a.dx2_8_scales = d2.p8s; a.lddx2_8 = C;
    }
    a.M = M; a.C = C;
    a.dy = dy; a.dy_dtype = dydt; a.lddy = lddy; a.dy_map = dym;
    a.x = x; a.x_dtype = xdt; a.ldx = ldx; a.x_map = xm;
    a.w = c.p->P[wi]; a.mean = mean; a.rstd = rstd;
    a.gin = gin; a.ldgin = lddx;
    a.dx = dx; a.dx_dtype = dxdt; a.lddx = lddx;
    a.dw = c.p->G[wi]; a.db = c.p->G[bi];
    a.relu_mask = relu ? 1 : 0;
    const bool on_side = c.p->side != nullptr && c.st == (void*)c.p->side;
    a.ws = c.at<float>(on_side ? c.p->o_lnws_side : c.p->o_lnws);
    a.ws_floats = on_side ? c.p->lnws_side_floats : c.p->lnws_floats;
    lnx_plan* p = c.p;
    const bool on_wgs = p->wgs != nullptr && c.st == (void*)p->wgs;
    if (p->ln_defer && !on_side && !on_wgs && p->o_lnws_defer != 0 && (a.dw || a.db)) {
        if (p->ln_pending == LN_DEFER_SLOTS) {
            RUN(lnx_layernorm_bwd_flush(c.st));
            p->ln_pending = 0;
// ... 131 lines not shown
    g.bias = p->P[d.cb]; g.c_map = om;
    RUN(gemm_nt_t(c, &g));
    return 0;
}

int meta_head_fwd(const Ctx& cc, int s, int m, const float* meta, int meta_width, float* tok, int N) {
    const Ctx c{cc.p, cc.st, LNX_F32};
    lnx_plan* p = c.p;
    MetaHead& k = p->meta[s][m];
    const int B = p->c.batch, C = p->c.dims[2 + s];
    RUN(lnx_pack_meta(meta, meta_width, k.off, k.dim, c.at<void>(k.t0), c.dt, B, c.st));
    lnx_gemm_args g = gemm_base(c, B, C, 16, c.at<void>(k.t0), 16, c.wptr(k.w0), k.w0.ld, c.at<void>(k.h0), C, false);
    g.bias = p->P[k.b0]; g.act = LNX_ACT_RELU;
    RUN(gemm_nt_t(c, &g));
    RUN(ln_fwd(c, B, C, 1e-5f, c.at<void>(k.h0), c.dt, C, IDM, k.lnw0, k.lnb0, c.at<void>(k.x), c.dt, C, IDM, nullptr, 0, c.at<float>(k.m0), c.at<float>(k.r0)));
    g = gemm_base(c, B, C, C, c.at<void>(k.x), C, c.wptr(k.w1), k.w1.ld, c.at<void>(k.h1), C, false);
    g.bias = p->P[k.b1]; g.act = LNX_ACT_RELU;
    RUN(gemm_nt_t(c, &g));
    RUN(ln_fwd(c, B, C, 1e-5f, c.at<void>(k.h1), c.dt, C, IDM, k.nf1w, k.nf1b, c.at<void>(k.n1), c.dt, C, IDM, nullptr, 0, c.at<float>(k.m1), c.at<float>(k.r1)));
    g = gemm_base(c, B, C, C, c.at<void>(k.n1), C, c.wptr(k.w2), k.w2.ld, c.at<void>(k.h2), C, false);
    g.bias = p->P[k.b2]; g.act = LNX_ACT_RELU;
    RUN(gemm_nt_t(c, &g));
    const lnx_rowmap om = {1, N - 1, 1 + m};
    RUN(ln_fwd(c, B, C, 1e-5f, c.at<void>(k.h2), c.dt, C, IDM, k.nf2w, k.nf2b, tok, LNX_F32, C, om, c.at<void>(k.x), C, c.at<float>(k.m2), c.at<float>(k.r2)));
    return 0;
}

int meta_chain_fwd(const Ctx& c, int s_lo, int s_hi, const float* meta, int meta_width) {
    lnx_plan* p = c.p;
    lnx_meta_head_args a[2 * LNX_MAX_META];
    int n = 0;
    for (int s = s_lo; s < s_hi; ++s)
        for (int m = 0; m < p->c.n_meta; ++m) {
            MetaHead& k = p->meta[s][m];
            const int C = p->c.dims[2 + s], N = s == 0 ? p->N2 : p->N3;
            lnx_meta_head_args& h = a[n++];
            memset(&h, 0, sizeof h);
            h.B = p->c.batch; h.C = C; h.dim = k.dim; h.off = k.off; h.meta = meta; h.meta_width = meta_width; h.eps = 1e-5f;
            h.w0 = (const float*)c.wptr(k.w0); h.ldw0 = k.w0.ld; h.b0 = p->P[k.b0]; h.ln0_w = p->P[k.lnw0]; h.ln0_b = p->P[k.lnb0];
            h.w1 = (const float*)c.wptr(k.w1); h.ldw1 = k.w1.ld; h.b1 = p->P[k.b1]; h.ln1_w = p->P[k.nf1w]; h.ln1_b = p->P[k.nf1b];
            h.w2 = (const float*)c.wptr(k.w2); h.ldw2 = k.w2.ld; h.b2 = p->P[k.b2]; h.ln2_w = p->P[k.nf2w]; h.ln2_b = p->P[k.nf2b];
            h.t0 = c.at<float>(k.t0); h.h0 = c.at<float>(k.h0); h.x = c.at<float>(k.x); h.h1 = c.at<float>(k.h1); h.n1 = c.at<float>(k.n1); h.h2 = c.at<float>(k.h2);
            h.m0 = c.at<float>(k.m0); h.r0 = c.at<float>(k.r0); h.m1 = c.at<float>(k.m1); h.r1 = c.at<float>(k.r1); h.m2 = c.at<float>(k.m2); h.r2 = c.at<float>(k.r2);
            h.tok = c.at<float>(p->o_tok[s]); h.tok_row_stride = (int64_t)N * C; h.tok_row_offset = (int64_t)(1 + m) * C;
        }
    return n ? lnx_meta_heads_fwd(a, n, c.st) : 0;
}

int meta_chain_bwd(const Ctx& c, int s, const float* g) {
    lnx_plan* p = c.p;
    lnx_meta_head_bwd_args a[LNX_MAX_META];
    const int C = p->c.dims[2 + s], N = s == 0 ? p->N2 : p->N3;
    for (int m = 0; m < p->c.n_meta; ++m) {
        MetaHead& k = p->meta[s][m];
        lnx_meta_head_bwd_args& h = a[m];
        memset(&h, 0, sizeof h);
        h.B = p->c.batch; h.C = C; h.dim = k.dim;
        h.g = g; h.g_row_stride = (int64_t)N * C; h.g_row_offset = (int64_t)(1 + m) * C;
        h.w1t = (const float*)c.wtptr(k.w1); h.ldw1t = k.w1.ld_t; h.w2t = (const float*)c.wtptr(k.w2); h.ldw2t = k.w2.ld_t;
        h.ln0_w = p->P[k.lnw0]; h.ln1_w = p->P[k.nf1w]; h.ln2_w = p->P[k.nf2w];
        h.t0 = c.at<float>(k.t0); h.h0 = c.at<float>(k.h0); h.x = c.at<float>(k.x); h.h1 = c.at<float>(k.h1); h.n1 = c.at<float>(k.n1); h.h2 = c.at<float>(k.h2);
        h.m0 = c.at<float>(k.m0); h.r0 = c.at<float>(k.r0); h.m1 = c.at<float>(k.m1); h.r1 = c.at<float>(k.r1); h.m2 = c.at<float>(k.m2); h.r2 = c.at<float>(k.r2);
        h.dp2 = c.at<float>(k.dp2); h.dp1 = c.at<float>(k.dp1); h.dp0 = c.at<float>(k.dp0); h.part = c.at<float>(k.part);
        h.d_w0 = p->G[k.w0.param]; h.d_b0 = p->G[k.b0]; h.d_ln0_w = p->G[k.lnw0]; h.d_ln0_b = p->G[k.lnb0];
        h.d_w1 = p->G[k.w1.param]; h.d_b1 = p->G[k.b1]; h.d_ln1_w = p->G[k.nf1w]; h.d_ln1_b = p->G[k.nf1b];
        h.d_w2 = p->G[k.w2.param]; h.d_b2 = p->G[k.b2]; h.d_ln2_w = p->G[k.nf2w]; h.d_ln2_b = p->G[k.nf2b];
    }
    return p->c.n_meta ? lnx_meta_heads_bwd(a, p->c.n_meta, c.st) : 0;
}

double rope_block_flops(int B, int N, int C, int hid) {
    const double M = (double)B * N;
    return 2.0 * M * C * (3.0 * C + C + 2.0 * hid) + 4.0 * B * (double)N * N * C;
}

int rope_block_fwd(const Ctx& c, int s, int i, float* xout) {
    lnx_plan* p = c.p;
    RopeBlk& k = p->rope[s][i];
    const int B = p->c.batch, C = p->c.dims[2 + s], heads = p->c.rope_heads[s], hid = p->c.mlp_hidden[s];
    const int N = s == 0 ? p->N2 : p->N3, M = B * N, E = p->E;
    const float* xin = c.at<float>(k.xin);
    p->resident[2 + s] = i;
    Timed span(c, 8, rope_block_flops(B, N, C, hid));
    const bool f8 = fp8_rows(p, M, C);
    void* a8 = f8 ? c.at<void>(p->o_a8) : nullptr;
    void* a8s = f8 ? c.at<void>(p->o_a8s) : nullptr;
    RUN(ln_fwd(c, M, C, 1e-5f, xin, LNX_F32, C, IDM, k.n1w, k.n1b, c.at<void>(k.n1), c.dt, C, IDM, nullptr, 0, c.at<float>(k.mean1), c.at<float>(k.rstd1), a8, a8s));
    lnx_gemm_args g = gemm_base(c, M, 3 * C, C, c.at<void>(k.n1), C, c.wptr(k.qkv), k.qkv.ld, c.at<void>(k.qkvbuf), 3 * C, false);
    g.bias = p->P[k.qkvb];
    RUN(linear_fwd(c, g, k.qkv, p->o_a8, p->o_a8s));
    lnx_attn_args a;
    memset(&a, 0, sizeof a);
    a.dtype = c.dt; a.B = B; a.N = N; a.E = E; a.heads = heads; a.head_dim = C / heads;
    a.qkv = c.at<void>(k.qkvbuf); a.cos_tab = c.at<float>(k.cos); a.o = c.at<void>(k.o); a.lse = c.at<float>(k.lse);
    if (p->c.rope_mode == LNX_ROPE_ROTATE) {
        a.rope_mode = LNX_ROPE_ROTATE; a.sin_tab = c.at<float>(k.dsin);
    }
    if (p->amask) {
        a.drop_mask = p->amask + k.dm_attn; a.drop_inv_keep = p->a_inv_keep;
    }
    {
        Timed t(c, 2, 4.0 * B * (double)N * N * C);
        RUN(lnx_attn_fwd(&a, c.st));
    }
    if (p->dmask) {
        g = gemm_base(c, M, C, C, c.at<void>(k.o), C, c.wptr(k.proj), k.proj.ld, c.at<void>(p->o_sD), C, false);
        g.bias = p->P[k.projb];
        RUN(gemm_nt_t(c, &g));
        RUN(lnx_dropout_residual(c.at<void>(p->o_sD), c.dt, p->dmask + k.dm_proj, p->inv_keep, p->drop_ptr(p->drop_attn[s][i]), N, xin, c.at<float>(k.xmid), M, C, c.st));
    } else {
        g = gemm_base(c, M, C, C, c.at<void>(k.o), C, c.wptr(k.proj), k.proj.ld, c.at<float>(k.xmid), C, true);
        g.bias = p->P[k.projb]; g.rowscale = p->drop_ptr(p->drop_attn[s][i]); g.rows_per_sample = N; g.res = xin; g.ldres = C;
        RUN(gemm_nt_t(c, &g));
    }
    RUN(ln_fwd(c, M, C, 1e-5f, c.at<float>(k.xmid), LNX_F32, C, IDM, k.n2w, k.n2b, c.at<void>(k.n2), c.dt, C, IDM, nullptr, 0, c.at<float>(k.mean2), c.at<float>(k.rstd2), a8, a8s));
    g = gemm_base(c, M, hid, C, c.at<void>(k.n2), C, c.wptr(k.fc1), k.fc1.ld, c.at<void>(k.act), hid, false);
    g.bias = p->P[k.fc1b]; g.act = f8 ? LNX_ACT_GELU : LNX_ACT_GELU_D; g.c2 = c.at<void>(k.hpre); g.ldc2 = hid;
    if (p->c.inference && !f8) {
        g.act = LNX_ACT_GELU; g.c2 = nullptr; g.ldc2 = 0;
    }
    RUN(linear_fwd(c, g, k.fc1, p->o_a8, p->o_a8s, p->o_h8, p->o_h8s));
    if (p->dmask) {
        RUN(lnx_dropout_mul(c.at<void>(k.act), c.dt, p->dmask + k.dm_hid, p->inv_keep, M, hid, c.st));
        g = gemm_base(c, M, C, hid, c.at<void>(k.act), hid, c.wptr(k.fc2), k.fc2.ld, c.at<void>(p->o_sD), C, false);
        g.bias = p->P[k.fc2b];
        RUN(gemm_nt_t(c, &g));
        RUN(lnx_dropout_residual(c.at<void>(p->o_sD), c.dt, p->dmask + k.dm_fc2, p->inv_keep, p->drop_ptr(p->drop_mlp[s][i]), N, c.at<float>(k.xmid), xout, M, C, c.st));
        return 0;
    }
    g = gemm_base(c, M, C, hid, c.at<void>(k.act), hid, c.wptr(k.fc2), k.fc2.ld, xout, C, true);
    g.bias = p->P[k.fc2b]; g.rowscale = p->drop_ptr(p->drop_mlp[s][i]); g.rows_per_sample = N; g.res = c.at<float>(k.xmid); g.ldres = C;
    RUN(linear_fwd(c, g, k.fc2, p->o_h8, p->o_h8s));
    return 0;
}

}

extern "C" int lnx_plan_forward(lnx_plan* p, const float* x, const float* meta, const float* drop_scales, const unsigned char* drop_mask, float* feats,
                                float* logits, void* stream) {
    if (!p || !p->bound) FAIL("lnx_plan_forward: plan is not bound");
    if (!x) FAIL("lnx_plan_forward: null input");
    const lnx_mformer_cfg& cf = p->c;
    if (cf.n_meta > 0 && !meta) FAIL("lnx_plan_forward: metadata components are configured but meta is NULL");
    if (cf.n_tasks > 0 && !logits) FAIL("lnx_plan_forward: logits buffer is NULL");
    Ctx c{p, stream, cf.dtype};
    const int B = cf.batch;
    const int* D = cf.dims;
    p->last_drop = drop_scales;
    p->mask_host.assign(p->n_drop, 0);
    if (drop_scales && drop_mask)
        for (int i = 0; i < p->n_drop; ++i) p->mask_host[i] = drop_mask[i];
    p->last_meta = meta;

    RUN(lnx_prep_weights(c.at<lnx_prep_desc>(p->o_descs), (int)p->n_descs_t, (int)p->prep_blocks, cf.dtype, stream));
    if (p->n_descs_f > 0)
        RUN(lnx_prep_weights(c.at<lnx_prep_desc>(p->o_descs) + p->n_descs_t, (int)p->n_descs_f, (int)p->prep_blocks_f, LNX_F32, stream));
    if (cf.fp8)
        for (int s = 0; s < 2; ++s)
            for (auto& k : p->rope[s]) {
                for (const OpW* w : {&k.qkv, &k.fc1, &k.fc2})
                    RUN(lnx_quantize_mxfp8(p->P[w->param], LNX_F32, w->K, w->N, w->K, c.at<void>(w->off8), w->K, c.at<void>(w->off8s), stream));
                for (const OpW* w : {&k.proj, &k.fc1, &k.fc2})
                    if (w->off8ts)
                        RUN(lnx_quantize_mxfp8(c.wtptr(*w), LNX_BF16, w->ld_t, w->K, w->N, c.at<void>(w->off8t), w->N, c.at<void>(w->off8ts), stream));
            }

    int mw_all = 0;
    for (int m = 0; m < cf.n_meta; ++m) mw_all += cf.meta_dims[m];
    hipStream_t const mst = meta_stream(p);
    if (mst) {
        HIPRUN(hipEventRecord(p->ev_fork, (hipStream_t)stream));
        HIPRUN(hipStreamWaitEvent(mst, p->ev_fork, 0));
        Ctx cs{p, (void*)mst, cf.dtype};
        if (p->chain_ok[0] && p->chain_ok[1]) {
            RUN(meta_chain_fwd(cs, 0, 2, meta, mw_all));
        } else {
            for (int s2 = 0; s2 < 2; ++s2) {
                if (p->chain_ok[s2]) {
                    RUN(meta_chain_fwd(cs, s2, s2 + 1, meta, mw_all));
                    continue;
                }
                for (int m = 0; m < cf.n_meta; ++m) RUN(meta_head_fwd(cs, s2, m, meta, mw_all, c.at<float>(p->o_tok[s2]), s2 == 0 ? p->N2 : p->N3));
            }
        }
    }
    {
        std::vector<lnx_rope_table> tabs;
        for (int s = 0; s < 2; ++s)
            for (auto& k : p->rope[s]) {
                lnx_rope_table t;
                memset(&t, 0, sizeof t);
                t.freqs = p->P[k.freqs]; t.heads = cf.rope_heads[s]; t.H = p->H[2 + s]; t.W = p->W[2 + s]; t.head_dim = cf.dims[2 + s] / cf.rope_heads[s];
                t.cos_out = c.at<float>(k.cos);
                if (cf.rope_mode == LNX_ROPE_ROTATE) {
                    t.rope_mode = LNX_ROPE_ROTATE; t.sin_out = c.at<float>(k.dsin);
                } else {
                    t.dsin_out = cf.inference ? nullptr : c.at<float>(k.dsin);
                }
                tabs.push_back(t);
            }
        if (!tabs.empty()) RUN(lnx_rope_cos_tables(tabs.data(), (int)tabs.size(), mst ? (void*)mst : stream));
    }
    if (mst) HIPRUN(hipEventRecord(p->ev_meta, mst));

    const int M0 = B * p->HW[0];
    float* first = cf.conv_depths[0] > 0 ? c.at<float>(p->conv[0][0].xin) : c.at<float>(p->o_stage_out[0]);
    if (lnx_stem_fwd_ok(cf.dtype, cf.in_chans, cf.img_h, cf.img_w, D[0])) {
        lnx_stem_args sa;
        memset(&sa, 0, sizeof sa);
        sa.x = x; sa.w = c.wptr(p->stem_w); sa.bias = p->P[p->stem_b]; sa.ln_w = p->P[p->stem_lnw]; sa.ln_b = p->P[p->stem_lnb];
        sa.y = first;
        if (!cf.inference) {
            sa.patches = c.at<void>(p->o_patches); sa.pre = c.at<void>(p->o_stem_pre);
            sa.mean = c.at<float>(p->o_stem_mean); sa.rstd = c.at<float>(p->o_stem_rstd);
        }
        sa.B = B; sa.Cin = cf.in_chans; sa.H = cf.img_h; sa.W = cf.img_w; sa.Cout = D[0]; sa.eps = 1e-6f;
        RUN(lnx_stem_fwd(&sa, stream));
    } else {
        RUN(lnx_im2col_stem(x, B, cf.in_chans, cf.img_h, cf.img_w, c.at<void>(p->o_patches), cf.dtype, 64, stream));
        {
            lnx_gemm_args g = gemm_base(c, M0, D[0], 64, c.at<void>(p->o_patches), 64, c.wptr(p->stem_w), 64, c.at<void>(p->o_stem_pre), D[0], false);
            g.bias = p->P[p->stem_b];
            RUN(gemm_nt_t(c, &g));
        }
        RUN(ln_fwd(c, M0, D[0], 1e-6f, c.at<void>(p->o_stem_pre), cf.dtype, D[0], IDM, p->stem_lnw, p->stem_lnb, first, LNX_F32, D[0], IDM, nullptr, 0,
                   c.at<float>(p->o_stem_mean), c.at<float>(p->o_stem_rstd)));
    }

    for (int s = 0; s < 2; ++s) {
        const int nb = cf.conv_depths[s];
        for (int i = 0; i < nb; ++i) {
            float* xout = i + 1 < nb ? c.at<float>(p->conv[s][i + 1].xin) : c.at<float>(p->o_stage_out[s]);
            RUN(conv_block_fwd(c, s, i, nullptr, xout));
        }
        if (s == 0) {
            float* nxt = cf.conv_depths[1] > 0 ? c.at<float>(p->conv[1][0].xin) : c.at<float>(p->o_stage_out[1]);
            RUN(downsample_fwd(c, 0, c.at<float>(p->o_stage_out[0]), LNX_F32, D[0], IDM, nxt, D[1], IDM));
        } else {
            const lnx_rowmap tm = {p->HW[2], p->E, p->E};
            RUN(downsample_fwd(c, 1, c.at<float>(p->o_stage_out[1]), LNX_F32, D[1], IDM, c.at<float>(p->o_tok[0]), D[2], tm));
        }
    }

    for (int s = 0; s < 2; ++s) {
        const int N = s == 0 ? p->N2 : p->N3, C = D[2 + s];
        float* tok = c.at<float>(p->o_tok[s]);
        const lnx_rowmap clsmap = {1, N - 1, 0};
        RUN(lnx_fill_rows(p->P[p->cls[s]], tok, C, clsmap, B, C, stream));
        if (mst) {
            if (s == 0) HIPRUN(hipStreamWaitEvent((hipStream_t)stream, p->ev_meta, 0));
        } else if (p->chain_ok[s]) {
            RUN(meta_chain_fwd(c, s, s + 1, meta, mw_all));
        } else {
            for (int m = 0; m < cf.n_meta; ++m) RUN(meta_head_fwd(c, s, m, meta, mw_all, tok, N));
        }
        const int nb = cf.rope_depths[s];
        for (int i = 0; i < nb; ++i) {
            float* xout = i + 1 < nb ? c.at<float>(p->rope[s][i + 1].xin) : c.at<float>(p->o_stage_out[2 + s]);
            RUN(rope_block_fwd(c, s, i, xout));
        }
        if (s == 0) {
            const int M2 = B * p->N2;
            RUN(ln_fwd(c, M2, C, 1e-5f, c.at<float>(p->o_stage_out[2]), LNX_F32, C, IDM, p->norm_w[0], p->norm_b[0], c.at<void>(p->o_t1), cf.dtype, C, IDM,
                       nullptr, 0, c.at<float>(p->o_t1_mean), c.at<float>(p->o_t1_rstd)));
            if (!cf.only_last_cls) {
                lnx_gemm_args g = gemm_base(c, B, D[2], D[2], c.at<void>(p->o_t1), (int64_t)p->N2 * D[2], c.wptr(p->cl_w1), p->cl_w1.ld, c.at<void>(p->o_cl_act),
                                            D[2], false);
                g.bias = p->P[p->cl_b1]; g.act = LNX_ACT_GELU; g.c2 = c.at<void>(p->o_cl_hpre); g.ldc2 = D[2];
                RUN(gemm_nt_t(c, &g));
                g = gemm_base(c, B, D[3], D[2], c.at<void>(p->o_cl_act), D[2], c.wptr(p->cl_w2), p->cl_w2.ld, c.at<float>(p->o_cl_u), D[3], true);
                g.bias = p->P[p->cl_b2];
                RUN(gemm_nt_t(c, &g));
                RUN(ln_fwd(c, B, D[3], 1e-5f, c.at<float>(p->o_cl_u), LNX_F32, D[3], IDM, p->cl_lnw, p->cl_lnb, c.at<float>(p->o_c1n), LNX_F32, D[3], IDM, nullptr,
                           0, c.at<float>(p->o_cl_mean), c.at<float>(p->o_cl_rstd)));
            }
            const lnx_rowmap pm = {p->HW[2], p->E, p->E};
            const lnx_rowmap tm = {p->HW[3], p->E, p->E};
            RUN(downsample_fwd(c, 2, c.at<void>(p->o_t1), cf.dtype, C, pm, c.at<float>(p->o_tok[1]), D[3], tm));
        }
    }

    {
        const int C = D[3];
        const lnx_rowmap clsrow = {1, p->N3 - 1, 0};
        RUN(ln_fwd(c, B, C, 1e-5f, c.at<float>(p->o_stage_out[3]), LNX_F32, C, clsrow, p->norm_w[1], p->norm_b[1], c.at<float>(p->o_c2n), LNX_F32, C, IDM, nullptr,
                   0, c.at<float>(p->o_n2_mean), c.at<float>(p->o_n2_rstd)));
        const float* fin_in = c.at<float>(p->o_c2n);
        if (!cf.only_last_cls) {
            RUN(lnx_agg2_fwd(c.at<float>(p->o_c1n), c.at<float>(p->o_c2n), p->P[p->agg_w], p->P[p->agg_b], c.at<float>(p->o_agg), B, C, stream));
            fin_in = c.at<float>(p->o_agg);
        }
        RUN(ln_fwd(c, B, C, 1e-5f, fin_in, LNX_F32, C, IDM, p->fin_w, p->fin_b, c.at<float>(p->o_feats), LNX_F32, C, IDM, nullptr, 0, c.at<float>(p->o_fin_mean),
                   c.at<float>(p->o_fin_rstd)));
        if (feats) HIPRUN(hipMemcpyAsync(feats, c.at<float>(p->o_feats), (size_t)B * C * 4, hipMemcpyDeviceToDevice, (hipStream_t)stream));
        if (cf.n_tasks > 0) {
            RUN(lnx_scale_cast(c.at<float>(p->o_feats), C, IDM, nullptr, 0, c.at<void>(p->o_featsT), cf.dtype, C, B, C, stream));
            lnx_gemm_args hg[LNX_MAX_TASKS];
            for (int t = 0; t < cf.n_tasks; ++t) {
                hg[t] = gemm_base(c, B, cf.task_classes[t], C, c.at<void>(p->o_featsT), C, c.wptr(p->head_w[t]), p->head_w[t].ld, logits + p->logit_off[t],
                                  p->logit_ld[t], true);
                hg[t].bias = p->P[p->head_b[t]];
            }
            RUN(heads_nt(c, hg, cf.n_tasks, false));
        }
    }
    p->fwd_done = true;
    return 0;
}

// ... 329 lines not shown
    (void)lnx_attn_bwd_discard();
    p->freq_pending = 0;
    struct TnGuard {
        lnx_plan* p;
        ~TnGuard() {
            (void)lnx_gemm_tn_discard();
            if (lnx_layernorm_bwd_discard() > 0) p->ln_pending = 0;
            if (lnx_attn_bwd_discard() > 0) p->freq_pending = 0;
        }
    } tn_guard{p};
    const lnx_mformer_cfg& cf = p->c;
    if (segment <= 0) p->dy8_ready = false;
    Ctx c{p, stream, cf.dtype};
    hipStream_t st = (hipStream_t)stream;
    const int B = cf.batch;
    const int* D = cf.dims;
    const bool all = segment < 0;

    if (all || segment == 0) {
        const int C = D[3];
        float* dfe = c.at<float>(p->o_tail[0]);
        bool have = false, heads_forked = false;
        if (dfeats) {
            HIPRUN(hipMemcpyAsync(dfe, dfeats, (size_t)B * C * 4, hipMemcpyDeviceToDevice, st));
            have = true;
        }
        if (cf.n_tasks > 0) {
            if (!dlogits) FAIL("lnx_plan_backward: dlogits is NULL");
            unsigned char* dl0 = c.at<unsigned char>(p->o_dlT);
            RUN(lnx_scale_cast(dlogits, p->logits_numel, IDM, nullptr, 0, dl0, cf.dtype, p->logits_numel, 1, (int)p->logits_numel, stream));
            const Ctx cw = wg_ctx(c);
            RUN(wg_fork(c, 3));
            lnx_gemm_args hg[LNX_MAX_TASKS];
            for (int t = 0; t < cf.n_tasks; ++t) {
                const int ld = p->logit_ld[t], nc = cf.task_classes[t];
                void* dl = dl0 + p->logit_off[t] * p->esz;
                RUN(wgrad(cw, B, nc, C, dl, ld, c.at<void>(p->o_featsT), C, p->head_w[t].param, p->head_b[t], C));
                hg[t] = gemm_base(c, B, C, ld, dl, ld, c.wtptr(p->head_w[t]), p->head_w[t].ld_t, dfe, C, true);
            }
            RUN(wg_done(c, 3));
            heads_forked = true;
            if (have) {
                hg[0].res = dfe;
                hg[0].ldres = C;
            }
            RUN(heads_nt(c, hg, cf.n_tasks, true));
            have = true;
        }
        if (!have) FAIL("lnx_plan_backward: neither dlogits nor dfeats given");
        const float* fin_in = cf.only_last_cls ? c.at<float>(p->o_c2n) : c.at<float>(p->o_agg);
        float* dfin = c.at<float>(p->o_tail[1]);
        RUN(ln_bwd(c, B, C, dfe, LNX_F32, C, IDM, fin_in, LNX_F32, C, IDM, p->fin_w, p->fin_b, c.at<float>(p->o_fin_mean), c.at<float>(p->o_fin_rstd), nullptr, dfin,
                   LNX_F32, C, false));
        float* dc2n = dfin;
        float* dc1n = nullptr;
        if (!cf.only_last_cls) {
            dc1n = c.at<float>(p->o_tail[2]);
            dc2n = c.at<float>(p->o_tail[3]);
            RUN(lnx_agg2_bwd(dfin, c.at<float>(p->o_c1n), c.at<float>(p->o_c2n), p->P[p->agg_w], dc1n, dc2n, p->G[p->agg_w], p->G[p->agg_b], B, C, stream));
        }
        float* g3 = c.at<float>(p->o_g[3]);
        HIPRUN(hipMemsetAsync(g3, 0, (size_t)B * p->N3 * C * 4, st));
        const lnx_rowmap clsrow = {1, p->N3 - 1, 0};
        RUN(ln_bwd(c, B, C, dc2n, LNX_F32, C, IDM, c.at<float>(p->o_stage_out[3]), LNX_F32, C, clsrow, p->norm_w[1], p->norm_b[1], c.at<float>(p->o_n2_mean),
                   c.at<float>(p->o_n2_rstd), nullptr, g3, LNX_F32, C, false));
        for (int i = cf.rope_depths[1] - 1; i >= 0; --i) {
            RUN(rope_block_restore(c, 1, i));
            RUN(rope_block_bwd(c, 1, i, g3, i != cf.rope_depths[1] - 1));
        }
        RUN(tokens_bwd(c, 1, g3));
        const int C2 = D[2];
        void* dt1 = c.at<void>(p->o_dt1);
        HIPRUN(hipMemsetAsync(dt1, 0, (size_t)B * p->N2 * C2 * p->esz, st));
        const lnx_rowmap gm = {p->HW[3], p->E, p->E};
        const lnx_rowmap pm = {p->HW[2], p->E, p->E};
        RUN(downsample_bwd(c, 2, g3, C, gm, c.at<void>(p->o_t1), cf.dtype, C2, pm, dt1, cf.dtype, C2));
        if (!cf.only_last_cls) {
            void* du = c.at<void>(p->o_tail[4]);
            void* dca = c.at<void>(p->o_tail[5]);
            RUN(ln_bwd(c, B, C, dc1n, LNX_F32, C, IDM, c.at<float>(p->o_cl_u), LNX_F32, C, IDM, p->cl_lnw, p->cl_lnb, c.at<float>(p->o_cl_mean), c.at<float>(p->o_cl_rstd),
                       nullptr, du, cf.dtype, C, false));
            RUN(wgrad(c, B, C, C2, du, C, c.at<void>(p->o_cl_act), C2, p->cl_w2.param, p->cl_b2, C2));
            lnx_gemm_args a = gemm_base(c, B, C2, C, du, C, c.wtptr(p->cl_w2), p->cl_w2.ld_t, dca, C2, false);
            a.act = LNX_ACT_GELU_BWD; a.aux = c.at<void>(p->o_cl_hpre); a.ldaux = C2;
            RUN(gemm_nt_t(c, &a));
            RUN(wgrad(c, B, C2, C2, dca, C2, c.at<void>(p->o_t1), (int64_t)p->N2 * C2, p->cl_w1.param, p->cl_b1, C2));
            a = gemm_base(c, B, C2, C2, dca, C2, c.wtptr(p->cl_w1), p->cl_w1.ld_t, dt1, C2, false);
            a.c_map = lnx_rowmap{1, p->N2 - 1, 0};
            RUN(gemm_nt_t(c, &a));
        }
        float* g2 = c.at<float>(p->o_g[2]);
        Dx2 dn;
        dn.p = c.at<void>(p->o_sC); dn.rowscale = p->drop_ptr(p->drop_mlp[0][cf.rope_depths[0] - 1]); dn.rps = p->N2;
        RUN(ln_bwd(c, B * p->N2, C2, dt1, cf.dtype, C2, IDM, c.at<float>(p->o_stage_out[2]), LNX_F32, C2, IDM, p->norm_w[0], p->norm_b[0], c.at<float>(p->o_t1_mean),
                   c.at<float>(p->o_t1_rstd), nullptr, g2, LNX_F32, C2, false, dn));
        RUN(ln_flush(c));
        if (heads_forked) RUN(wg_join(c, 3));
    }
    if (all || segment == 1) {
        float* g2 = c.at<float>(p->o_g[2]);
        for (int i = cf.rope_depths[0] - 1; i >= 0; --i) {
            RUN(rope_block_restore(c, 0, i));
            RUN(rope_block_bwd(c, 0, i, g2, true));
        }
        RUN(tokens_bwd(c, 0, g2));
        const lnx_rowmap gm = {p->HW[2], p->E, p->E};
        RUN(downsample_bwd(c, 1, g2, D[2], gm, c.at<float>(p->o_stage_out[1]), LNX_F32, D[1], IDM, c.at<float>(p->o_g[1]), LNX_F32, D[1]));
        RUN(ln_flush(c));
        RUN(join_side(c, 1));
    }
    if (all || segment == 2) {
        float* g1 = c.at<float>(p->o_g[1]);
        for (int i = cf.conv_depths[1] - 1; i >= 0; --i) {
            RUN(conv_block_restore(c, 1, i));
            RUN(conv_block_bwd(c, 1, i, g1));
        }
        RUN(downsample_bwd(c, 0, g1, D[1], IDM, c.at<float>(p->o_stage_out[0]), LNX_F32, D[0], IDM, c.at<float>(p->o_g[0]), LNX_F32, D[0]));
        RUN(ln_flush(c));
        RUN(join_side(c, 0));
    }
    if (all || segment == 3) {
        float* g0 = c.at<float>(p->o_g[0]);
        for (int i = cf.conv_depths[0] - 1; i >= 0; --i) {
            RUN(conv_block_restore(c, 0, i));
            RUN(conv_block_bwd(c, 0, i, g0));
        }
        const int M0 = B * p->HW[0];
        void* sC = c.at<void>(p->o_sC);
        RUN(ln_bwd(c, M0, D[0], g0, LNX_F32, D[0], IDM, c.at<void>(p->o_stem_pre), cf.dtype, D[0], IDM, p->stem_lnw, p->stem_lnb, c.at<float>(p->o_stem_mean),
                   c.at<float>(p->o_stem_rstd), nullptr, sC, cf.dtype, D[0], false));
        const int kst = cf.in_chans * 16;
        RUN(wgrad(c, M0, D[0], 64, sC, D[0], c.at<void>(p->o_patches), 64, p->stem_w.param, p->stem_b, kst, kst));
        RUN(ln_flush(c));
    }
    return 0;
}

extern "C" int lnx_plan_backward_into(lnx_plan* p, const float* dlogits, const float* dfeats, float* const* grads, void* stream) {
    if (!p || !grads) FAIL("lnx_plan_backward_into: null %s", !p ? "plan" : "gradient pointer set");
    if (!p->bound || !p->has_grads) FAIL("lnx_plan_backward_into: plan is not bound with gradient buffers");
    const size_t n = p->names.size();
    for (size_t i = 0; i < n; ++i)
        if (grads[i] == nullptr || (((uintptr_t)grads[i]) & 3) != 0) FAIL("lnx_plan_backward_into: gradient of %s is null or misaligned", p->names[i].c_str());
    std::vector<float*> into(grads, grads + n);
    struct Swap {
        lnx_plan* p;
        std::vector<float*>& v;
        Swap(lnx_plan* p_, std::vector<float*>& v_) : p(p_), v(v_) { p->G.swap(v); }
        ~Swap() { p->G.swap(v); }
    } swap{p, into};
    return lnx_plan_backward(p, dlogits, dfeats, -1, stream);
}

extern "C" int lnx_plan_segment_params(const lnx_plan* p, int segment, int* idx_out, int max_out) {
    if (!p || segment < 0 || segment > 3) return -1;
    int n = 0;
    auto seg_of = [&](const std::string& nm) -> int {
        if (nm.rfind("stages.3.", 0) == 0 || nm.rfind("head.", 0) == 0 || nm.rfind("norm_", 0) == 0 || nm.rfind("cl_1_fc", 0) == 0 ||
            nm.rfind("aggregate", 0) == 0 || nm.rfind("final_norm", 0) == 0 || nm == "cls_token_2" || nm.rfind("downsample_layers.2", 0) == 0)
            return 0;
        if (nm.rfind("meta.", 0) == 0) return nm.find("head_2") != std::string::npos ? 1 : 2;
        if (nm.rfind("stages.2.", 0) == 0 || nm == "cls_token_1" || nm.rfind("downsample_layers.1", 0) == 0) return 1;
        if (nm.rfind("stages.1.", 0) == 0 || nm.rfind("downsample_layers.0", 0) == 0) return 2;
        return 3;
    };
    for (size_t i = 0; i < p->names.size(); ++i)
        if (seg_of(p->names[i]) == segment) {
            if (idx_out && n < max_out) idx_out[n] = (int)i;
            ++n;
        }
    return n;
}

extern "C" int lnx_plan_profile_begin(lnx_plan* p) {
    if (!p) FAIL("lnx_plan_profile_begin: null plan");
    p->profile = true;
    p->profile_spans = false;
    p->spans.clear();
    p->ev_used = 0;
    return 0;
}

extern "C" int lnx_plan_set_wgrad_stream(lnx_plan* p, int on) {
    if (!p || (on != 0 && on != 1)) {
        lnx_set_error("lnx_plan_set_wgrad_stream: %s", !p ? "null plan" : "on must be 0 or 1");
        return -1;
    }
    const int was = wg_on(p) ? 1 : 0;
    if (p->wgs) (void)hipStreamSynchronize(p->wgs);
    p->wgs_on = on != 0;
    return was;
}

extern "C" int lnx_plan_set_meta_stream(lnx_plan* p, int mode) {
    if (!p || mode < 0 || mode > 2) {
        lnx_set_error("lnx_plan_set_meta_stream: null plan / mode %d (0 launch stream, 1 side stream, 2 weight-gradient stream)", mode);
        return -1;
    }
    const int was = p->meta_mode;
    if (mode == 1 && p->side == nullptr) mode = 0;
    p->meta_mode = mode;
    return was;
}

extern "C" int lnx_plan_profile_begin_spans(lnx_plan* p) {
    if (!p) FAIL("lnx_plan_profile_begin_spans: null plan");
    p->profile = true;
    p->profile_spans = true;
    p->spans.clear();
    p->ev_used = 0;
    return 0;
}

static int profile_collect(lnx_plan* p, int ncls, double* ms, double* work, double* bytes, int* launches) {
    p->profile = false;
    p->profile_spans = false;
    HIPRUN(hipDeviceSynchronize());
    for (int i = 0; i < ncls; ++i) {
        ms[i] = 0;
        work[i] = 0;
        if (bytes) bytes[i] = 0;
        launches[i] = 0;
    }
    for (const auto& sp : p->spans) {
        if (sp.cls >= ncls) continue;
        float t = 0.f;
        HIPRUN(hipEventElapsedTime(&t, sp.e0, sp.e1));
        ms[sp.cls] += t;
        work[sp.cls] += sp.work;
        if (bytes) bytes[sp.cls] += sp.bytes;
        launches[sp.cls] += 1;
    }
    p->spans.clear();
    p->ev_used = 0;
    return 0;
}

extern "C" int lnx_plan_profile_end(lnx_plan* p, double* ms, double* work, int* launches) {
    if (!p || !ms || !work || !launches) FAIL("lnx_plan_profile_end: null argument");
    return profile_collect(p, LNX_PROFILE_CLASSES, ms, work, nullptr, launches);
}

extern "C" int lnx_plan_profile_end_ex(lnx_plan* p, double* ms, double* work, double* bytes, int* launches) {
    if (!p || !ms || !work || !bytes || !launches) FAIL("lnx_plan_profile_end_ex: null argument");
    return profile_collect(p, LNX_PROFILE_CLASSES_EX, ms, work, bytes, launches);
}
```

linnaeus_amd/loss.py:

```python
import ctypes as C
import math
import re
from typing import Any, Callable, Dict, Optional

import torch
import torch.distributed as dist
import torch.nn as nn

from . import _lib as L


def _ptr(t):
    return C.c_void_p(t.data_ptr()) if t is not None else None


def _fill(a, logits, target, soft, smoothing, class_weight, ignore_index, row_scale, scale, loss, loss_sum, dlogits):
    if not logits.is_cuda:
        raise L.LnxError("linnaeus_amd.loss has no CPU path: logits must be on the GPU")
    a.B, a.C = logits.shape
    a.logits, a.ld = _ptr(logits), logits.stride(0)
    a.target = _ptr(target)
    a.soft, a.smoothing = _ptr(soft), float(smoothing)
    a.class_weight = _ptr(class_weight)
    a.ignore_index = -1 if ignore_index is None else int(ignore_index)
# ... 181 lines not shown


def compute_core_loss(outputs, targets, criteria, config=None):
    return {t: criteria[t](outputs[t], targets[t]) for t in _sorted_tasks(outputs)}


def _class_weight_vector(cw_dict, num_classes: int, device) -> torch.Tensor:
    v = torch.ones(num_classes, dtype=torch.float32)
    for i, w in cw_dict.items():
        if 0 <= int(i) < num_classes:
            v[int(i)] = float(w)
    return v.to(device)


def _sample_weights(cw_dict, target: torch.Tensor, cache: Optional[dict] = None, key=None) -> torch.Tensor:
    if target.dim() == 1:
        n = max(int(max(cw_dict.keys(), default=0)) + 1, 1)
        ck = (key, n, str(target.device))
        vec = cache.get(ck) if cache is not None else None
        if vec is None:
            vec = _class_weight_vector(cw_dict, n, target.device)
            if cache is not None:
                cache[ck] = vec
        idx = target.clamp(0, n - 1)
        return torch.where(target < n, vec[idx], torch.ones((), device=target.device))
    vec = _class_weight_vector(cw_dict, target.size(1), target.device)
    return (target.float() * vec.unsqueeze(0)).sum(1)


def apply_class_weighting(per_task_losses, targets, class_weights=None, _cache=None):
    if class_weights is None:
        return per_task_losses
    out = {}
    for t, vec in per_task_losses.items():
        out[t] = vec * _sample_weights(class_weights[t], targets[t], _cache, t).to(vec.dtype) if t in class_weights else vec
    return out


def apply_null_masking(per_task_losses, targets, null_mask_prob: float, logger=None, config=None, _coin=None):
    masked, stats = {}, {"null_mask_prob": null_mask_prob}
    tot = inc = None
    for t, vec in per_task_losses.items():
        null = _is_null(targets[t])
        if null_mask_prob < 1.0:
            u = _coin[t].to(vec.device) if _coin is not None else torch.rand(vec.shape[0], device=vec.device)
            keep = (~null) | (u < null_mask_prob)
        else:
            keep = torch.ones_like(null)
        masked[t] = torch.where(keep, vec, torch.zeros((), dtype=vec.dtype, device=vec.device))
        n, k = null.sum(), (null & keep).sum()
        tot, inc = (n, k) if tot is None else (tot + n, inc + k)
    stats["null_samples_total"], stats["null_samples_included"] = tot, inc
    stats["inclusion_percentage"] = inc.float() * 100.0 / tot.float().clamp_min(1.0) if tot is not None else 0.0
    return masked, stats


def apply_loss_masking(per_task_losses, targets, ops_schedule, current_step, class_weights=None, is_validation=False, logger=None, config=None,
                       _coin=None, _cache=None):
    if is_validation:
        prob = 1.0
    elif config is not None and getattr(config.TRAIN, "PHASE1_MASK_NULL_LOSS", False):
        prob = 0.0
    else:
        prob = float(ops_schedule.get_null_mask_prob(current_step))
    masked, stats = apply_null_masking(per_task_losses, targets, prob, logger, config, _coin)
    stats["num_valid_samples_per_task"] = {t: (v != 0).sum() for t, v in masked.items()}
    if class_weights is not None:
        return apply_class_weighting(masked, targets, class_weights, _cache), stats
    return masked, stats


def _cfg_get(node, path, default):
    for k in path.split("."):
        if node is None:
            return default
        node = node.get(k, None) if isinstance(node, dict) else getattr(node, k, None)
    return default if node is None else node


DEFAULT_EXCLUDE_CONFIG = {"TYPE": "or", "FILTERS": [{"TYPE": "name", "PATTERNS": ["head"]}, {"TYPE": "name", "PATTERNS": ["meta_"]}]}


def param_filter(spec) -> Callable[[str, torch.Tensor], bool]:
    kind = str(_cfg_get(spec, "TYPE", "")).lower()
    if kind == "name":
        pats, how = list(_cfg_get(spec, "PATTERNS", [])), str(_cfg_get(spec, "MATCH_TYPE", "contains"))
        if how == "regex":
            rx = [re.compile(q) for q in pats]
            f = lambda n, p: any(r.search(n) for r in rx)
        elif how in ("contains", "startswith", "endswith"):
            f = {"contains": lambda n, p: any(q in n for q in pats), "startswith": lambda n, p: any(n.startswith(q) for q in pats),
                 "endswith": lambda n, p: any(n.endswith(q) for q in pats)}[how]
        else:
            raise ValueError(f"Unknown match_type: {how}")
    elif kind == "dimension":
        dims = list(_cfg_get(spec, "DIMENSIONS", []))
        f = lambda n, p: p.dim() in dims
    elif kind in ("and", "or"):
        subs = [param_filter(x) for x in _cfg_get(spec, "FILTERS", [])]
        f = (lambda n, p: all(g(n, p) for g in subs)) if kind == "and" else (lambda n, p: any(g(n, p) for g in subs))
    elif kind in ("not", "all_except"):
        sub = param_filter(_cfg_get(spec, "FILTER" if kind == "not" else "EXCEPT", {}))
        f = lambda n, p: not sub(n, p)
    else:
        raise ValueError(f"Unsupported filter type for the GradNorm backbone: {kind!r}")
    return lambda n, p: f(n[7:] if n.startswith("module.") else n, p)


class GradNormModule(nn.Module):

    def __init__(self, task_keys, alpha: float = 1.5, init_weights: Optional[torch.Tensor] = None, label_densities=None, num_classes=None,
                 init_strategy: str = "inverse_density", config: Any = None):
        super().__init__()
        self.num_tasks = len(task_keys)
        self.task_keys = list(task_keys)
        self.alpha = float(alpha)
        self.config = config
        if init_weights is None:
            init_weights = self._compute_init_weights(self.task_keys, label_densities, num_classes, init_strategy)
        self.register_buffer("task_weights", torch.as_tensor(init_weights, dtype=torch.float32).clone())
        self.register_buffer("initial_losses", torch.zeros(self.num_tasks))
        self.register_buffer("_initted", torch.zeros(1, dtype=torch.int32), persistent=False)
        self.has_initted = False

    def _compute_init_weights(self, task_keys, label_densities=None, num_classes=None, strategy: str = "inverse_density") -> torch.Tensor:
        if not label_densities:
            return torch.ones(len(task_keys), dtype=torch.float32)
        dens = [label_densities.get(k, 1.0) for k in task_keys]
        if strategy == "inverse_density" or (strategy == "class_complexity" and num_classes is None):
            w = [1.0 / max(d, 0.001) for d in dens]
        elif strategy == "class_complexity":
            counts = [num_classes.get(k, 1) for k in task_keys]
            mx = max(counts)
            w = [1.0 / max(d, 0.001) * (math.log(c) / math.log(mx)) for d, c in zip(dens, counts)]
        else:
            w = [1.0] * len(task_keys)
        tot = sum(w)
        return torch.tensor([x * len(task_keys) / tot for x in w], dtype=torch.float32)

    def forward(self, losses):
        return (torch.stack([losses[k] for k in sorted(losses.keys())]) * self.task_weights).sum()

    def get_task_weights(self) -> Dict[str, float]:
        return {t: float(w) for t, w in zip(sorted(self.task_keys), self.task_weights.tolist())}


def backbone_slices(layout, backbone) -> list:
    ids = {id(p) for p in backbone}
    out = [(o, n) for o, n, p in zip(layout["offsets"], layout["numels"], layout["params"]) if id(p) in ids]
    return sorted(out)


def gradnorm_desc_table(slices, base_ptr: int):
    arr = (L.AdamWDesc * len(slices))()
    blk = 0
    for d, (off, n) in zip(arr, slices):
        d.g, d.n, d.group, d.block_start = base_ptr + 4 * off, n, 0, blk
        blk += (n + 4095) // 4096
    return arr, blk


class GradientWeighting(nn.Module):

    def __init__(self, task_keys, config=None, task_weighting_type: str = "static", init_weights=None, class_weights=None,
                 use_subset_weights: bool = False, alpha: float = 1.5, label_densities=None, num_classes=None, init_strategy: str = "inverse_density",
                 update_interval: int = 100, exclude_patterns=None, zero_aux_info: bool = True, keep_step_grads: bool = False, **kwargs):
        super().__init__()
        if task_weighting_type not in ("static", "gradnorm"):
            raise NotImplementedError(f"task weighting type {task_weighting_type!r}: 'static' or 'gradnorm'")
        self.task_keys = list(task_keys)
        self.config = config
        self.task_weighting_type = task_weighting_type
        if isinstance(init_weights, dict):
            init_weights = [init_weights.get(k, 1.0) for k in self.task_keys]
        init_weights = list(init_weights or [1.0] * len(self.task_keys))
        self.task_weights = torch.tensor(init_weights, dtype=torch.float32)
        self.gradnorm = None
        self.update_interval, self.exclude_patterns = 0, []
        self.backbone_params = None
        self.model = None
        if task_weighting_type == "gradnorm":
            self.gradnorm = GradNormModule(self.task_keys, alpha=alpha, init_weights=torch.tensor(init_weights, dtype=torch.float32),
                                           label_densities=label_densities, num_classes=num_classes, init_strategy=init_strategy, config=config)
            self.update_interval = update_interval
            self.exclude_patterns = exclude_patterns or ["head", "meta_"]
            self.zero_aux_info = bool(_cfg_get(config, "LOSS.GRAD_WEIGHTING.TASK.ZERO_AUX_INFO", zero_aux_info))
            self.keep_step_grads = bool(keep_step_grads)
        self.class_weights = class_weights
        self.use_subset_weights = use_subset_weights
        self._cache: dict = {}
        self._gn: dict = {}

    def _normalize_weights(self, w):
        return w

    def set_model(self, model: nn.Module) -> None:
        if self.task_weighting_type != "gradnorm":
            return
        self.model = model
        net = model
        while hasattr(net, "module") and isinstance(net.module, nn.Module):
            net = net.module
        self._net = net
        spec = _cfg_get(self.config, "LOSS.GRAD_WEIGHTING.TASK.EXCLUDE_CONFIG", None) or DEFAULT_EXCLUDE_CONFIG
        f = param_filter(spec)
        self.backbone_names = [n for n, p in net.named_parameters() if p.requires_grad and not f(n, p)]
        self.backbone_params = [net.get_parameter(n) for n in self.backbone_names]
        self._gn = {}

    def scratch_arenas(self) -> int:
        if self.gradnorm is None:
            return 0
        return 1 if int(_cfg_get(self.config, "LOSS.GRAD_WEIGHTING.TASK.GRADNORM_ACCUM_STEPS", 1)) <= 1 else len(self.task_keys)

    def _descs(self, arenas: torch.Tensor):
        net = self._net
        key = (arenas.data_ptr(), tuple(arenas.shape), net._arena_layout)
        if self._gn.get("key") != key:
            layout = net.grad_arena_layout()
            if layout["total"] != arenas.shape[1]:
                raise L.LnxError(f"gradient arena layout mismatch: {layout['total']} floats, scratch rows hold {arenas.shape[1]}")
            slices = backbone_slices(layout, self.backbone_params)
            if not slices:
                raise L.LnxError("GradNorm: no backbone parameter is differentiated by the model's plan")
            arr, blk = gradnorm_desc_table(slices, arenas.data_ptr())
            table = torch.frombuffer(bytearray(arr), dtype=torch.uint8).to(arenas.device)
            self._gn = {"key": key, "table": table, "ndesc": len(slices), "blocks": blk,
                        "ws": torch.empty(len(self.task_keys) * blk, device=arenas.device, dtype=torch.float32)}
        return self._gn

    def _sumsq(self, arenas, first: int, ntasks: int, norm: torch.Tensor, stream) -> None:
        g = self._descs(arenas)
        L.check(L.lib().lnx_gradnorm_sumsq(C.c_void_p(g["table"].data_ptr()), g["ndesc"], g["blocks"], ntasks, arenas.stride(0), None,
                                           C.c_void_p(norm.data_ptr() + 4 * first), C.c_void_p(g["ws"].data_ptr()), stream), "lnx_gradnorm_sumsq")

    def update_gradnorm_weights_reforward(self, data_batch, criteria, amp_enabled: bool = True, ops_schedule=None, current_step=None, *,
                                          sync: bool = True, keep_step_grads: Optional[bool] = None) -> Dict[str, Any]:
        if self.task_weighting_type != "gradnorm" or self.gradnorm is None:
            return {}
        if self.model is None or not self.backbone_params:
            raise RuntimeError("GradientWeighting.set_model(model) must be called before a GradNorm update")
        net = self._net
        keep = self.keep_step_grads if keep_step_grads is None else bool(keep_step_grads)
        images, targets, aux = data_batch[0], data_batch[1], data_batch[2]
        dev = images.device
        aux_g = torch.zeros_like(aux) if (self.zero_aux_info and aux is not None) else aux
        S = max(1, int(_cfg_get(self.config, "LOSS.GRAD_WEIGHTING.TASK.GRADNORM_ACCUM_STEPS", 1)))
        ckpt = bool(_cfg_get(self.config, "TRAIN.GRADIENT_CHECKPOINTING.ENABLED_GRADNORM_STEPS", False))
        T = len(self.task_keys)
        plan_tasks = net._task_list()
        order = sorted(self.task_keys)
        if sorted(plan_tasks) != order:
            raise ValueError(f"GradNorm tasks {self.task_keys} differ from the model's heads {plan_tasks}")
        gn = self.gradnorm.to(dev)
        stats = torch.zeros(2, T, device=dev, dtype=torch.float32)
        norm_plan = torch.zeros(T, device=dev, dtype=torch.float32)
        stream = C.c_void_p(torch.cuda.current_stream(dev).cuda_stream)
        was_training = net.training
        net.train()
        try:
            B = images.shape[0]
            for s in range(S):
                lo = s * (B // S)
                hi = B if s == S - 1 else (s + 1) * (B // S)
                sb_t = {k: v[lo:hi].to(dev) for k, v in targets.items()}

                def seed(t, logits_t, dl_t, sb_t=sb_t):
                    name = plan_tasks[t]
                    y = sb_t[name]
                    valid = (y != 0) if y.dim() == 1 else (y[:, 0] <= 0.5)
                    cnt = valid.sum().float()
                    crit = criteria[name]
                    if isinstance(crit, TaxonomyAwareLabelSmoothingCE):
                        tgt = (y.argmax(dim=1) if y.dim() == 2 else y).to(torch.long).contiguous()
                        cw = crit.weight.to(dev) if (crit.apply_class_weights and crit.weight is not None) else None
                        rs = valid.float() / cnt.clamp_min(1.0)
                        per = torch.empty(y.shape[0], device=dev, dtype=torch.float32)
                        _launch(_as_rows(logits_t), tgt, crit.soft_labels.to(dev), 0.0, cw, crit.ignore_index, rs, 1.0, per, None, dl_t)
                        lsum = torch.where(valid, per, torch.zeros((), device=dev)).sum()
                    else:
                        leaf = logits_t.detach().clone().requires_grad_(True)
                        with torch.enable_grad():
                            vec = crit(leaf, y)
                            lsum = vec[valid].sum()
                            g, = torch.autograd.grad(lsum / cnt.clamp_min(1.0), leaf, allow_unused=True)
                        if g is not None:
                            dl_t.copy_(g)
                        lsum = lsum.detach().float()
                    stats[0, t] += lsum
                    stats[1, t] += cnt

                after = None
                if S == 1:
                    after = lambda t: self._sumsq(net._gn_scratch, t, 1, norm_plan, stream)
                with torch.no_grad():
                    net._task_backbone_grads(images[lo:hi], aux_g[lo:hi] if aux_g is not None else None, seed, 1 if S == 1 else T, ckpt,
                                             accumulate=s > 0, after_task=after)
            if S > 1:
                self._sumsq(net._gn_scratch, 0, T, norm_plan, stream)
        finally:
            net.train(was_training)
        if self._gn.get("perm") is None or self._gn["perm"].device != dev:
            self._gn["perm"] = torch.tensor([plan_tasks.index(k) for k in order], device=dev)
        perm = self._gn["perm"]
        norm = norm_plan[perm]
        loss_sum, count = stats[0][perm].contiguous(), stats[1][perm].contiguous()
        init_loss = None
# ... 83 lines not shown
```

linnaeus_amd/model.py:

```python
from __future__ import annotations

import ctypes as C
import math
import os
from collections import OrderedDict
from typing import Any, Dict, List, Optional, Sequence

import torch
import torch.nn as nn

from . import _lib as L
from .heads import configure_classification_heads
from .registry import register_model

_DTYPES = {"bf16": L.BF16, "bfloat16": L.BF16, "fp32": L.F32, "float32": L.F32}


class _Cfg(C.Structure):
    _fields_ = [
        ("dtype", C.c_int), ("batch", C.c_int), ("img_h", C.c_int), ("img_w", C.c_int), ("in_chans", C.c_int),
        ("dims", C.c_int * 4), ("conv_depths", C.c_int * 2), ("rope_depths", C.c_int * 2), ("rope_heads", C.c_int * 2),
        ("mlp_hidden", C.c_int * 2), ("n_meta", C.c_int), ("meta_dims", C.c_int * 8), ("only_last_cls", C.c_int),
        ("n_tasks", C.c_int), ("task_classes", C.c_int * 16), ("inference", C.c_int), ("recompute", C.c_int), ("fp8", C.c_int),
        ("rope_mode", C.c_int),
# ... 135 lines not shown
        cs = M.CONVNEXT_STAGES
        depths, dims = list(cs.DEPTHS), list(cs.DIMS)
        self.convnext_ls_init = cs.get("LAYER_SCALE_INIT_VALUE", 1e-6)
        if len(depths) != 4 or len(dims) != 4:
            raise ValueError("CONVNEXT_STAGES depths and dims must be lists of length 4.")
        if "ROPE_STAGES" not in M:
            raise ValueError("mFormerV1 requires MODEL.ROPE_STAGES config")
        rs = M.ROPE_STAGES
        rdepths, rdims, rheads, rratio = list(rs.DEPTHS), list(rs.DIMS), list(rs.NUM_HEADS), list(rs.MLP_RATIO)
        self.rope_theta = rs.get("ROPE_THETA", 10000.0)
        self.rope_mixed = rs.get("ROPE_MIXED", True)
        self.rope_rotate = bool(rs.get("ROPE_ROTATE", False))
        if len(rdepths) != 2 or len(rdims) != 2 or len(rheads) != 2 or len(rratio) != 2:
            raise ValueError("ROPE_STAGES depths, dims, num_heads, mlp_ratio must be lists of length 2.")
        if not self.rope_mixed:
            raise NotImplementedError("ROPE_MIXED=False (axial) is broken in the reference (SURVEY F8) and unused by every config")
        if rdims[0] != dims[2]:
            raise ValueError(f"ConvNeXt dim[2] ({dims[2]}) must match RoPE dim[0] ({rdims[0]})")
        if rdims[1] != dims[3]:
            raise ValueError(f"ConvNeXt dim[3] ({dims[3]}) must match RoPE dim[1] ({rdims[1]})")
        for d_, h_ in zip(rdims, rheads):
            if h_ <= 0 or d_ % h_ != 0 or d_ // h_ not in (32, 64, 128):
                raise NotImplementedError(f"HIP attention kernels are built for head_dim 32, 64 or 128 (got dim {d_}, heads {h_})")
        self.use_flash_attn = M.get("USE_FLASH_ATTN", False)

        self.use_meta = False
        self.meta_components: Dict[str, Dict[str, int]] = {}
        self.meta_dims: List[int] = []
        meta_cfg = config.DATA.get("META", None) if hasattr(config, "DATA") else None
        if meta_cfg is not None and meta_cfg.get("ACTIVE", False) and "COMPONENTS" in meta_cfg:
            self.use_meta = True
            items = []
            for name, cc in meta_cfg.COMPONENTS.items():
                if cc.get("ENABLED", False) and cc.get("IDX", -1) >= 0:
                    items.append((cc.get("IDX"), name, cc))
            items.sort(key=lambda t: t[0])
            off = 0
            for _, name, cc in items:
                self.meta_dims.append(cc.DIM)
                self.meta_components[name] = {"dim": cc.DIM, "offset": off}
                off += cc.DIM
        self.extra_token_num = 1 + len(self.meta_dims)

        total = sum(depths[:2]) + sum(rdepths)
        dpr = [x.item() for x in torch.linspace(0, self.drop_path_rate, total)]

        self.stem = _Holder(nn.Conv2d(in_chans, dims[0], kernel_size=4, stride=4), _LNCF(dims[0]))
        self.downsample_layers = nn.ModuleList([_Down(dims[i], dims[i + 1]) for i in range(3)])
        self.stages = nn.ModuleList()
        k = 0
        for s in range(2):
            self.stages.append(nn.ModuleList([_ConvBlk(dims[s], self.convnext_ls_init, dpr[k + i]) for i in range(depths[s])]))
            k += depths[s]
        for s in range(2):
            self.stages.append(nn.ModuleList([_RopeBlk(rdims[s], rheads[s], rratio[s], self.rope_theta, dpr[k + i]) for i in range(rdepths[s])]))
            k += rdepths[s]
        self.norm_1 = nn.LayerNorm(rdims[0])
        self.norm_2 = nn.LayerNorm(rdims[1])
        self.cls_token_1 = nn.Parameter(torch.zeros(1, 1, rdims[0]))
        self.cls_token_2 = nn.Parameter(torch.zeros(1, 1, rdims[1]))
        _trunc_normal_(self.cls_token_1, std=0.02)
        _trunc_normal_(self.cls_token_2, std=0.02)
        for name, info in self.meta_components.items():
            for s in range(2):
                setattr(self, f"meta_{name.lower()}_head_{s + 1}",
                        _Holder(nn.Linear(info["dim"], rdims[s]), nn.ReLU(inplace=True), nn.LayerNorm(rdims[s]), _ResNorm(rdims[s])))
        if not self.only_last_cls:
            self.cl_1_fc = _Holder(_Mlp(rdims[0], rdims[0], rdims[1]), nn.LayerNorm(rdims[1]))
            self.aggregate = nn.Conv1d(in_channels=2, out_channels=1, kernel_size=1)
        else:
            self.cl_1_fc = None
            self.aggregate = None
        self.final_norm = nn.LayerNorm(rdims[1])

        self.task_keys = list(config.DATA.TASK_KEYS_H5)
        self.head = configure_classification_heads(
            heads_config=M.CLASSIFICATION.HEADS, in_features=rdims[1], num_classes_dict=kwargs.get("num_classes"),
            task_keys=self.task_keys, taxonomy_tree=kwargs.get("taxonomy_tree"))
        self.apply(self._init_weights)

        self._dims, self._depths, self._rdepths, self._rheads = dims, depths, rdepths, rheads
        self._hidden = [int(rdims[s] * rratio[s]) for s in range(2)]
        self._in_chans = in_chans
        dt_name = str(kwargs.get("compute_dtype", os.environ.get("LNX_DTYPE", M.get("LNX_DTYPE", "bf16")))).lower()
        self._fp8 = dt_name in ("fp8", "mxfp8")
        self._dtype_code = L.BF16 if self._fp8 else _DTYPES[dt_name]
        self.grad_mode = str(kwargs.get("grad_mode", "autograd"))
        self.max_cached_plans = 4
        self._plans: "OrderedDict[Any, Dict[str, Any]]" = OrderedDict()
        self._active = None
        self._inject_drop = None
        self._inject_dropout = None
        self._inject_attn_dropout = None
        self._segment_hook = None
        self._grad_arena = None
        self._grad_views: Optional[List[torch.Tensor]] = None
        self._arena_layout = None
        self.use_checkpoint = False
        self.hierarchical_refinement = bool(M.CLASSIFICATION.get("HIERARCHICAL_REFINEMENT", False)) if hasattr(M, "CLASSIFICATION") else False

    @staticmethod
    def _init_weights(m):
        if isinstance(m, (nn.Conv2d, nn.Linear)):
            _trunc_normal_(m.weight, std=0.02)
            if isinstance(m, nn.Linear) and m.bias is not None:
                nn.init.constant_(m.bias, 0)
        elif isinstance(m, nn.LayerNorm):
            nn.init.constant_(m.bias, 0)
            nn.init.constant_(m.weight, 1.0)

    @property
    def parameter_groups_metadata(self) -> Dict[str, Any]:
        return {
            "stages": {
                "convnext_stages": ["stem.", "stages.0.", "stages.1.", "downsample_layers.0", "downsample_layers.1"],
                "rope_stages": ["stages.2.", "stages.3.", "downsample_layers.2", "downsample_layers.3"],
                "rope_freqs": ["freqs"],
            },
            "heads": {"classification_heads": ["head."], "meta_heads": ["meta_"]},
            "embeddings": ["cls_token"],
            "norm_layers": ["norm", ".bn", "LayerNorm"],
            "aggregation": ["cl_1_fc.", "aggregate.", "final_norm."],
        }

    @property
    def pretrained_ckpt_handling_metadata(self) -> Dict[str, Any]:
        return {
            "drop_buffers": [],
            "drop_params": ["head.", "meta_", "pos_embed", "norm.", "downsample_layers."],
            "interpolate_rel_pos_bias": False,
            "supports_module_prefix": True,
            "strict": False,
        }

    def set_compute_dtype(self, name: str) -> None:
        name = name.lower()
        self._fp8 = name in ("fp8", "mxfp8")
        self._dtype_code = L.BF16 if self._fp8 else _DTYPES[name]
        self.release_plans()

    def set_wgrad_stream(self, on: bool) -> None:
        self._wgrad_stream = bool(on)
        for st in self._plans.values():
            if st.get("handle") is not None and L.lib().lnx_plan_set_wgrad_stream(st["handle"], int(self._wgrad_stream)) < 0:
                L.check(1, "lnx_plan_set_wgrad_stream")

    def set_meta_stream(self, mode: int) -> None:
        if mode not in (0, 1, 2):
            raise ValueError(f"meta stream mode {mode!r}: 0 (launch stream), 1 (side stream) or 2 (weight-gradient stream)")
        self._meta_stream = int(mode)
        for st in self._plans.values():
            if st.get("handle") is not None and L.lib().lnx_plan_set_meta_stream(st["handle"], self._meta_stream) < 0:
                L.check(1, "lnx_plan_set_meta_stream")

    def _destroy_plan(self, st) -> None:
        if st.get("destroyed"):
            return
        st["destroyed"] = True
        try:
            L.lib().lnx_plan_destroy(st["handle"])
        finally:
            st["handle"] = None
            st["ws"] = None
            st["dl_buf"] = st["dl_views"] = None
            st["dropout_masks"] = st["attn_dropout_masks"] = None
            st["saved_inputs"] = None

    def release_plans(self) -> None:
        if torch.cuda.is_available() and self._plans:
            torch.cuda.synchronize()
        for st in list(self._plans.values()):
            self._destroy_plan(st)
        self._plans.clear()
        self._active = None

    @property
    def compute_dtype(self) -> str:
        return "fp8" if self._fp8 else ("bf16" if self._dtype_code == L.BF16 else "fp32")

    def _task_list(self) -> List[str]:
        return list(self.head.keys())

    def _param_for(self, plan_name: str) -> torch.Tensor:
        if plan_name.startswith("meta."):
            _, m, rest = plan_name.split(".", 2)
            comp = list(self.meta_components.keys())[int(m)]
            stage, tail = rest.split(".", 1)
            return self.get_parameter(f"meta_{comp.lower()}_{stage}.{tail}")
        if plan_name.startswith("head."):
            _, t, kind = plan_name.split(".")
            lin = self.head[self._task_list()[int(t)]].effective_linear
            if kind == "bias" and lin.bias is None:
                raise NotImplementedError("heads without bias are not supported by the HIP plan")
            return lin.weight if kind == "weight" else lin.bias
        return self.get_parameter(plan_name)

    def _wants_recompute(self, force_checkpointing: Optional[bool] = None) -> bool:
        want = bool(force_checkpointing) if force_checkpointing is not None else self._checkpoint_policy()
        return want and self.training

    def _checkpoint_policy(self) -> bool:
        want = bool(self.use_checkpoint)
        try:
            want = want or bool(self.config.TRAIN.GRADIENT_CHECKPOINTING.ENABLED_NORMAL_STEPS)
        except (AttributeError, KeyError):
            pass
        return want

    def _make_cfg(self, B: int, H: int, W: int, train: bool, recompute: bool = False) -> "_Cfg":
        cfg = _Cfg()
        cfg.inference = 0 if train else 1
        cfg.recompute = 1 if (train and recompute) else 0
        cfg.fp8 = 1 if self._fp8 else 0
        cfg.rope_mode = L.ROPE_ROTATE if self.rope_rotate else L.ROPE_COS
        cfg.dtype, cfg.batch, cfg.img_h, cfg.img_w, cfg.in_chans = self._dtype_code, B, H, W, self._in_chans
        cfg.dims[:] = self._dims
        cfg.conv_depths[:] = self._depths[:2]
        cfg.rope_depths[:] = self._rdepths
        cfg.rope_heads[:] = self._rheads
        cfg.mlp_hidden[:] = self._hidden
        cfg.n_meta = len(self.meta_dims)
        for i, d in enumerate(self.meta_dims):
            cfg.meta_dims[i] = d
        cfg.only_last_cls = int(bool(self.only_last_cls))
        tasks = self._task_list()
        cfg.n_tasks = len(tasks)
        for i, t in enumerate(tasks):
            cfg.task_classes[i] = self.head[t].effective_linear.out_features
        return cfg

    def workspace_bytes(self, batch: int, img_h: Optional[int] = None, img_w: Optional[int] = None, train: bool = True,
                        recompute: Optional[bool] = None) -> int:
        H = img_h or self.img_size[0]
        W = img_w or img_h or self.img_size[1]
        return self.plan_footprint(batch, H, W, train, recompute)["workspace"]

    def plan_footprint(self, batch: int, img_h: Optional[int] = None, img_w: Optional[int] = None, train: bool = True,
                       recompute: Optional[bool] = None, gradnorm_arenas: int = 0) -> Dict[str, int]:
        if gradnorm_arenas:
            fp = self.plan_footprint(batch, img_h, img_w, train, recompute)
            fp["gradnorm"] = int(gradnorm_arenas) * 4 * self.grad_arena_layout()["total"] + fp["logits"] // 2
            return fp
        lib = L.lib()
        for fn in (lib.lnx_plan_workspace_bytes, lib.lnx_plan_dropout_bytes, lib.lnx_plan_attn_dropout_bytes, lib.lnx_plan_logits_numel):
            fn.restype = C.c_int64
        H = img_h or self.img_size[0]
        W = img_w or img_h or self.img_size[1]
        if recompute is None:
            recompute = self._checkpoint_policy()
        cfg = self._make_cfg(int(batch), int(H), int(W), train, bool(recompute))
        handle = C.c_void_p()
        L.check(lib.lnx_plan_create(C.byref(cfg), C.byref(handle)), "lnx_plan_create")
        try:
            drop = int(lib.lnx_plan_dropout_bytes(handle)) if (train and self.drop_rate > 0.0) else 0
            adrop = int(lib.lnx_plan_attn_dropout_bytes(handle)) if (train and self.attn_drop_rate > 0.0) else 0
            logits = int(lib.lnx_plan_logits_numel(handle)) * 4 * (2 if train else 1)
            return {"workspace": int(lib.lnx_plan_workspace_bytes(handle)) + 256, "dropout": drop, "attn_dropout": adrop, "logits": logits}
        finally:
            lib.lnx_plan_destroy(handle)

    def _get_plan(self, B: int, H: int, W: int, train: bool = True, recompute: bool = False) -> Dict[str, Any]:
        recompute = bool(train and recompute)
        key = (B, H, W, self._dtype_code, self._fp8, bool(train), recompute)
        st = self._plans.get(key)
        lib = L.lib()
        if st is not None:
            self._plans.move_to_end(key)
        if st is None:
            while len(self._plans) >= max(1, int(self.max_cached_plans)):
                _, old = self._plans.popitem(last=False)
                if old is self._active:
                    self._active = None
                torch.cuda.current_stream().synchronize()
                self._destroy_plan(old)
            cfg = self._make_cfg(B, H, W, train, recompute)
            tasks = self._task_list()
            handle = C.c_void_p()
            L.check(lib.lnx_plan_create(C.byref(cfg), C.byref(handle)), "lnx_plan_create")
            if not getattr(self, "_wgrad_stream", True) and lib.lnx_plan_set_wgrad_stream(handle, 0) < 0:
                L.check(1, "lnx_plan_set_wgrad_stream")
            if getattr(self, "_meta_stream", None) is not None and lib.lnx_plan_set_meta_stream(handle, self._meta_stream) < 0:
                L.check(1, "lnx_plan_set_meta_stream")
            lib.lnx_plan_workspace_bytes.restype = C.c_int64
            lib.lnx_plan_param_name.restype = C.c_char_p
            lib.lnx_plan_param_numel.restype = C.c_int64
            lib.lnx_plan_logits_numel.restype = C.c_int64
            lib.lnx_plan_logits_offset.restype = C.c_int64
            n = lib.lnx_plan_num_params(handle)
            names = [lib.lnx_plan_param_name(handle, i).decode() for i in range(n)]
            params = [self._param_for(nm) for nm in names]
            for nm, p_, i in zip(names, params, range(n)):
                if p_.numel() != lib.lnx_plan_param_numel(handle, i):
                    raise L.LnxError(f"parameter {nm}: module has {p_.numel()} elements, plan expects {lib.lnx_plan_param_numel(handle, i)}")
            dev = params[0].device
            wsb = lib.lnx_plan_workspace_bytes(handle)
            ws = torch.empty(wsb + 256, dtype=torch.uint8, device=dev)
            seg_of = [3] * n
            buf = (C.c_int * n)()
            for seg in range(4):
                cnt = lib.lnx_plan_segment_params(handle, seg, buf, n)
                for j in range(cnt):
                    seg_of[buf[j]] = seg
            st = dict(handle=handle, names=names, params=params, ws=ws, ptrs=None, n=n, seg_of=seg_of,
                      ndrop=lib.lnx_plan_num_drop_calls(handle), logits_numel=lib.lnx_plan_logits_numel(handle),
                      logit_off=[lib.lnx_plan_logits_offset(handle, i) for i in range(len(tasks))],
                      logit_ld=[lib.lnx_plan_logits_ld(handle, i) for i in range(len(tasks))], tasks=tasks, B=B, fwd_id=0, train=bool(train))
            self._plans[key] = st
        self._ensure_bound(st)
        return st

    @staticmethod
    def _arena_offsets(numels: List[int], seg_of: List[int]):
        order = sorted(range(len(numels)), key=lambda i: (seg_of[i], i))
        offs, cur, seg_bounds = {}, 0, {}
        for i in order:
            seg = seg_of[i]
            seg_bounds.setdefault(seg, [cur, cur])
            offs[i] = cur
            cur += (numels[i] + 3) // 4 * 4
            seg_bounds[seg][1] = cur
        return offs, cur, {s: tuple(b) for s, b in seg_bounds.items()}

    def grad_arena_layout(self, batch: int = 1, img_h: Optional[int] = None, img_w: Optional[int] = None) -> Dict[str, Any]:
        lib = L.lib()
        lib.lnx_plan_param_name.restype = C.c_char_p
        lib.lnx_plan_param_numel.restype = C.c_int64
        H = img_h or self.img_size[0]
        W = img_w or img_h or self.img_size[1]
        cfg = self._make_cfg(int(batch), int(H), int(W), True, False)
        handle = C.c_void_p()
        L.check(lib.lnx_plan_create(C.byref(cfg), C.byref(handle)), "lnx_plan_create")
        try:
            n = lib.lnx_plan_num_params(handle)
            names = [lib.lnx_plan_param_name(handle, i).decode() for i in range(n)]
            numels = [int(lib.lnx_plan_param_numel(handle, i)) for i in range(n)]
            seg_of = [3] * n
            buf = (C.c_int * n)()
            for seg in range(4):
                for j in range(lib.lnx_plan_segment_params(handle, seg, buf, n)):
                    seg_of[buf[j]] = seg
        finally:
            lib.lnx_plan_destroy(handle)
        params = [self._param_for(nm) for nm in names]
        offs, total, bounds = self._arena_offsets(numels, seg_of)
        return dict(names=names, params=params, numels=numels, seg_of=seg_of, offsets=[offs[i] for i in range(n)], total=total, bounds=bounds)

    def _ensure_grad_arena(self, st) -> None:
        params = st["params"]
        ident = tuple(id(p) for p in params)
        dev = params[0].device
        if self._grad_arena is not None and self._arena_layout == (ident, dev):
            return
        offs, cur, seg_bounds = self._arena_offsets([p_.numel() for p_ in params], st["seg_of"])
        self._grad_arena = torch.zeros(cur, dtype=torch.float32, device=dev)
        self._grad_views = [self._grad_arena[offs[i]: offs[i] + params[i].numel()].view(params[i].shape) for i in range(st["n"])]
        self._segment_bounds = seg_bounds
        self._arena_layout = (ident, dev)
        for s2 in self._plans.values():
            s2["ptrs"] = None

    def _ensure_bound(self, st) -> None:
        params = st["params"]
        if not params[0].is_cuda:
            raise L.LnxError("mFormerV1 (linnaeus_amd) runs on the MI355X HIP kernels only: call model.cuda() first; there is no CPU fallback")
        for p_ in params:
            if p_.dtype != torch.float32 or not p_.is_contiguous():
                raise L.LnxError("parameters must be contiguous fp32 (master weights); the bf16 operand copies are made by the plan")
        if st["train"]:
            self._ensure_grad_arena(st)
        ptrs = tuple(p_.data_ptr() for p_ in params)
        if st["ptrs"] == ptrs:
            return
        n = st["n"]
        parr = (C.c_void_p * n)(*ptrs)
        garr = (C.c_void_p * n)(*[v.data_ptr() for v in self._grad_views]) if st["train"] else None
        wsp = (st["ws"].data_ptr() + 255) // 256 * 256
        L.check(L.lib().lnx_plan_bind(st["handle"], parr, garr, C.c_void_p(wsp)), "lnx_plan_bind")
        st["ptrs"] = ptrs

    def _draw_drop_scales(self, st, B: int, dev) -> Optional[torch.Tensor]:
        probs: List[float] = []
        for s in range(2):
            probs += [blk.drop_prob for blk in self.stages[s]]
        for s in range(2, 4):
            for blk in self.stages[s]:
                probs += [blk.drop_prob, blk.drop_prob]
        assert len(probs) == st["ndrop"]
        if self._inject_drop is not None:
            inj = list(self._inject_drop)
            assert len(inj) == len(probs)
            mask = bytes(int(v is not None) for v in inj)
            if not any(mask):
                return None
            rows = [v.to(dev, torch.float32) if v is not None else torch.ones(B, device=dev) for v in inj]
            st["drop_mask"] = mask
            return torch.stack(rows, 0).contiguous()
        if not self.training or all(p == 0.0 for p in probs):
            return None
        cache = st.get("drop_keep")
        if cache is None or cache[0] != tuple(probs) or cache[1].device != dev:
            keep = torch.tensor([1.0 - p for p in probs], device=dev).unsqueeze(1)
            cache = st["drop_keep"] = (tuple(probs), keep, bytes(int(p > 0.0) for p in probs))
        _, keep, mask = cache
        scales = torch.bernoulli(keep.expand(len(probs), B)).div_(keep)
        st["drop_mask"] = mask
        return scales

    def _task_views(self, st, logits: torch.Tensor, B: int) -> List[torch.Tensor]:
        out = []
        for i, t in enumerate(st["tasks"]):
            ld = st["logit_ld"][i]
            nc = self.head[t].effective_linear.out_features
            out.append(logits[st["logit_off"][i]: st["logit_off"][i] + B * ld].view(B, ld)[:, :nc])
        return out

    def _set_dropout(self, st, train: bool, dev) -> None:
        lib = L.lib()
        active = train and self.training
        for key, rate, inject, nbytes_fn, set_fn in (
                ("dropout_masks", self.drop_rate, self._inject_dropout, lib.lnx_plan_dropout_bytes, lib.lnx_plan_set_dropout),
                ("attn_dropout_masks", self.attn_drop_rate, self._inject_attn_dropout, lib.lnx_plan_attn_dropout_bytes, lib.lnx_plan_set_attn_dropout)):
            if not (active and rate > 0.0):
                if st.get(key) is not None:
                    L.check(set_fn(st["handle"], None, C.c_float(0.0)), "lnx_plan_set_dropout")
                    st[key] = None
                continue
            if key == "dropout_masks" and self._fp8:
                raise NotImplementedError("DROP_RATE > 0 is not available in fp8 mode")
            nbytes_fn.restype = C.c_int64
            nbytes = int(nbytes_fn(st["handle"]))
            if inject is not None:
                masks = inject.to(dev, torch.uint8).contiguous()
                assert masks.numel() == nbytes, (key, masks.numel(), nbytes)
            else:
                masks = torch.empty(nbytes, dtype=torch.uint8, device=dev).bernoulli_(1.0 - rate)
            L.check(set_fn(st["handle"], C.c_void_p(masks.data_ptr()), C.c_float(rate)), "lnx_plan_set_dropout")
            st[key] = masks

    def _plan_forward(self, x, meta, drop):
        st = self._active
        B = x.shape[0]
        feats = torch.empty(B, self._dims[3], device=x.device, dtype=torch.float32)
        logits = torch.empty(max(st["logits_numel"], 1), device=x.device, dtype=torch.float32)
        mask = st.get("drop_mask") if drop is not None else None
        L.check(L.lib().lnx_plan_forward(
            st["handle"], C.c_void_p(x.data_ptr()), C.c_void_p(meta.data_ptr()) if meta is not None else None,
            C.c_void_p(drop.data_ptr()) if drop is not None else None, mask, C.c_void_p(feats.data_ptr()),
            C.c_void_p(logits.data_ptr()), C.c_void_p(torch.cuda.current_stream().cuda_stream)), "lnx_plan_forward")
        st["saved_inputs"] = (x, meta, drop)
        st["fwd_id"] = st.get("fwd_id", 0) + 1
        return feats, logits

    def _plan_backward(self, st, dfeats, dlogits):
        direct = self.grad_mode == "direct"
        params = st["params"]
        views = self._grad_views
        if direct:
            alias = [p_.grad is not None and p_.grad.data_ptr() == v.data_ptr() for p_, v in zip(params, views)]
            if not any(alias):
                self._grad_arena.zero_()
            elif not all(alias):
                for a, v in zip(alias, views):
                    if not a:
                        v.zero_()
        else:
            alias = None
            self._grad_arena.zero_()
        stream = C.c_void_p(torch.cuda.current_stream().cuda_stream)
        dl = dlogits.contiguous() if dlogits is not None else None
        df = dfeats.contiguous() if dfeats is not None else None
        if st["logits_numel"] == 0:
            dl = None
        lib = L.lib()
        if self._segment_hook is None:
            L.check(lib.lnx_plan_backward(st["handle"], C.c_void_p(dl.data_ptr()) if dl is not None else None,
                                          C.c_void_p(df.data_ptr()) if df is not None else None, -1, stream), "lnx_plan_backward")
        else:
            for seg in range(4):
                L.check(lib.lnx_plan_backward(st["handle"], C.c_void_p(dl.data_ptr()) if dl is not None else None,
                                              C.c_void_p(df.data_ptr()) if df is not None else None, seg, stream), "lnx_plan_backward")
                self._segment_hook(seg)
        if direct:
            for p_, v, a in zip(params, views, alias):
                if p_.grad is None:
                    p_.grad = v
                elif not a:
                    p_.grad.add_(v)
            return [None] * len(params)
        snap = self._grad_arena.clone()
        base = self._grad_arena.data_ptr()
        return [snap[(v.data_ptr() - base) // 4: (v.data_ptr() - base) // 4 + v.numel()].view(v.shape) for v in views]

    def _gradnorm_arenas(self, n: int) -> torch.Tensor:
        total = self._grad_arena.numel()
        cur = getattr(self, "_gn_scratch", None)
        if cur is None or cur.shape != (n, total) or cur.device != self._grad_arena.device:
            self._gn_scratch = None
            try:
                self._gn_scratch = torch.empty(n, total, dtype=torch.float32, device=self._grad_arena.device)
            except torch.cuda.OutOfMemoryError as e:
                raise L.LnxError(f"GradNorm needs {n} scratch gradient arena(s) of {4 * total / 2**20:.1f} MiB each: {e}") from e
        return self._gn_scratch

    def _task_backbone_grads(self, x: torch.Tensor, meta: Optional[torch.Tensor], seeds, n_arenas: int = 1, force_checkpointing: Optional[bool] = None,
                             accumulate: bool = False, after_task=None) -> torch.Tensor:
        if not x.is_cuda:
            raise L.LnxError("mFormerV1 (linnaeus_amd) has no CPU path: inputs must be on the GPU")
        x = x.float().contiguous()
        B, _, H, W = x.shape
        meta = meta.float().contiguous() if (self.use_meta and self.meta_dims) else None
        st = self._get_plan(B, H, W, True, self._wants_recompute(force_checkpointing))
        self._active = st
        drop = self._draw_drop_scales(st, B, x.device)
        self._set_dropout(st, True, x.device)
        _, logits = self._plan_forward(x, meta, drop)
        views = self._task_views(st, logits, B)
        dl = torch.zeros(max(st["logits_numel"], 1), device=x.device, dtype=torch.float32)
        dl_views = self._task_views(st, dl, B)
        n, T = st["n"], len(st["tasks"])
        if n_arenas not in (1, T):
            raise L.LnxError(f"GradNorm uses 1 or {T} scratch gradient arenas, not {n_arenas}")
        arenas = self._gradnorm_arenas(n_arenas)
        base = self._grad_arena.data_ptr()
        offs = [v.data_ptr() - base for v in self._grad_views]
        stream = C.c_void_p(torch.cuda.current_stream().cuda_stream)
        lib = L.lib()
        for t in range(T):
            row = arenas[t if arenas.shape[0] > 1 else 0]
            if not accumulate or arenas.shape[0] == 1:
                row.zero_()
            seeds(t, views[t], dl_views[t])
            ptrs = (C.c_void_p * n)(*[row.data_ptr() + o for o in offs])
            L.check(lib.lnx_plan_backward_into(st["handle"], C.c_void_p(dl.data_ptr()) if st["logits_numel"] else None, None, ptrs, stream),
                    "lnx_plan_backward_into")
            dl_views[t].zero_()
            if after_task is not None:
                after_task(t)
        return arenas

    def _run(self, x: torch.Tensor, meta: Optional[torch.Tensor], force_checkpointing: Optional[bool] = None):
        if not x.is_cuda:
            raise L.LnxError("mFormerV1 (linnaeus_amd) has no CPU path: inputs must be on the GPU")
        if x.dim() != 4 or x.shape[1] != self._in_chans:
            raise ValueError(f"expected input [B, {self._in_chans}, H, W], got {tuple(x.shape)}")
        x = x.float().contiguous()
        B, _, H, W = x.shape
        if self.use_meta and self.meta_dims:
            if meta is None:
                raise AssertionError("metadata components are configured but meta is None")
            if meta.shape[-1] != sum(self.meta_dims):
                raise ValueError(f"meta must be [B, {sum(self.meta_dims)}] (components in IDX order), got {tuple(meta.shape)}")
            meta = meta.float().contiguous()
        else:
            meta = None
        train = torch.is_grad_enabled() and any(p_.requires_grad for p_ in self.parameters())
        st = self._get_plan(B, H, W, train, self._wants_recompute(force_checkpointing))
        self._active = st
        drop = self._draw_drop_scales(st, B, x.device)
        self._set_dropout(st, train, x.device)
        if train:
            feats, *views = _PlanFn.apply(self, x, meta, drop, *st["params"])
        else:
            feats, logits = self._plan_forward(x, meta, drop)
            views = self._task_views(st, logits, B)
        return st, feats, views

    def forward_features(self, x: torch.Tensor, meta: Optional[torch.Tensor] = None, force_checkpointing: Optional[bool] = None) -> torch.Tensor:
        return self._run(x, meta, force_checkpointing)[1]

    def forward(self, x: torch.Tensor, meta: Optional[torch.Tensor] = None, force_checkpointing: Optional[bool] = None) -> Dict[str, torch.Tensor]:
        st, feats, views = self._run(x, meta, force_checkpointing)
        acast = torch.get_autocast_dtype("cuda") if torch.is_autocast_enabled("cuda") else None
        out = {}
        for t, v in zip(st["tasks"], views):
            out[t] = v
            if acast is not None:
                out[t] = out[t].to(acast)
        self._last_feats = feats
        if self.hierarchical_refinement:
            from .heads import refine_logits_top_down

            out = refine_logits_top_down(out, self.head, self.task_keys)
        return out

    def __del__(self):
        try:
            for st in self._plans.values():
                self._destroy_plan(st)
        except Exception:
            pass
```

linnaeus_amd/optim.py:

```python
import ctypes as C
import math
from typing import Optional

import numpy as np
import torch

from . import _lib as L


def _slot_items(state, items, name):
    slots = {}
    for gi, p in items:
        slots.setdefault((gi, int(state[p]["step"])), len(slots))
    if len(slots) > L.ADAMW_MAX_GROUPS:
        raise L.LnxError(f"{name}: {len(slots)} distinct (parameter group, step count) combinations, at most {L.ADAMW_MAX_GROUPS} are supported")
    return slots, [(slots[(gi, int(state[p]["step"]))], p) for gi, p in items]


def _adamw_descs(state, items):
    lib = L.lib()
    arr = (L.AdamWDesc * len(items))()
    blk = 0
    for i, (gi, p) in enumerate(items):
        st = state[p]
        arr[i].p, arr[i].m, arr[i].v, arr[i].g = p.data_ptr(), st["exp_avg"].data_ptr(), st["exp_avg_sq"].data_ptr(), p.grad.data_ptr()
        arr[i].n, arr[i].group, arr[i].block_start = p.numel(), gi, blk
        blk += lib.lnx_adamw_blocks(C.c_int64(p.numel()))
    return arr, blk


class FusedAdamW(torch.optim.Optimizer):
    def __init__(self, params, lr: float = 1e-3, betas=(0.9, 0.999), eps: float = 1e-8, weight_decay: float = 1e-2, max_grad_norm: Optional[float] = None):
        if lr < 0 or eps < 0 or not (0 <= betas[0] < 1) or not (0 <= betas[1] < 1) or weight_decay < 0:
            raise ValueError("invalid AdamW hyper-parameters")
        super().__init__(params, dict(lr=lr, betas=betas, eps=eps, weight_decay=weight_decay))
        if len(self.param_groups) > L.ADAMW_MAX_GROUPS:
            raise ValueError(f"at most {L.ADAMW_MAX_GROUPS} parameter groups")
        self.max_grad_norm = max_grad_norm
        self._table = None
        self._key = None
        self._sumsq = None
        self._sumsq_ws = None

    def _build(self, items):
        dev = items[0][1].device
        arr, blk = _adamw_descs(self.state, items)
        host = torch.from_numpy(np.frombuffer(arr, dtype=np.uint8).copy())
        self._table = (host.to(dev), len(items), blk)
        if self._sumsq is None or self._sumsq.device != dev:
            self._sumsq = torch.zeros(1, device=dev, dtype=torch.float32)
        if self._sumsq_ws is None or self._sumsq_ws.device != dev or self._sumsq_ws.numel() < blk:
            self._sumsq_ws = torch.empty(blk, device=dev, dtype=torch.float32)

    @torch.no_grad()
    def step(self, closure=None):
        loss = None
        if closure is not None:
            with torch.enable_grad():
                loss = closure()
        items = []
        for gi, group in enumerate(self.param_groups):
            for p in group["params"]:
                if p.grad is None:
                    continue
                if not p.is_cuda or p.dtype != torch.float32 or not p.is_contiguous() or p.grad.dtype != torch.float32 or not p.grad.is_contiguous():
                    raise L.LnxError("FusedAdamW needs contiguous fp32 parameters and gradients on the GPU")
                st = self.state[p]
                if len(st) == 0:
                    st["step"] = 0
                    st["exp_avg"] = torch.zeros_like(p, memory_format=torch.preserve_format)
                    st["exp_avg_sq"] = torch.zeros_like(p, memory_format=torch.preserve_format)
                st["step"] = int(st["step"]) + 1
                items.append((gi, p))
        if not items:
            return loss
        slots, items = _slot_items(self.state, items, "FusedAdamW")
        key = tuple((si, p.data_ptr(), p.grad.data_ptr(), self.state[p]["exp_avg"].data_ptr(), self.state[p]["exp_avg_sq"].data_ptr()) for si, p in items)
        if key != self._key:
            self._build(items)
            self._key = key
        h = L.AdamWHyper()
        h.ngroups = len(slots)
        for (gi, t), si in slots.items():
            group = self.param_groups[gi]
            b1, b2 = group["betas"]
            h.lr[si], h.beta1[si], h.beta2[si], h.eps[si], h.weight_decay[si] = group["lr"], b1, b2, group["eps"], group["weight_decay"]
            h.bias_c1[si], h.bias_c2[si] = 1.0 - b1 ** float(t), 1.0 - b2 ** float(t)
            h.omb1[si], h.omb2[si] = 1.0 - b1, 1.0 - b2
        table, n, blocks = self._table
        lib = L.lib()
        stream = C.c_void_p(torch.cuda.current_stream().cuda_stream)
        clip = self.max_grad_norm is not None and self.max_grad_norm > 0
        if clip:
            L.check(lib.lnx_grad_sumsq(C.c_void_p(table.data_ptr()), n, blocks, C.c_void_p(self._sumsq.data_ptr()), C.c_void_p(self._sumsq_ws.data_ptr()), stream),
                    "lnx_grad_sumsq")
        L.check(lib.lnx_adamw_step(C.c_void_p(table.data_ptr()), n, blocks, C.byref(h), C.c_void_p(self._sumsq.data_ptr()) if clip else None,
                                   C.c_float(self.max_grad_norm if clip else 0.0), stream), "lnx_adamw_step")
        return loss

    def grad_norm(self) -> Optional[torch.Tensor]:
        if self._sumsq is None or self.max_grad_norm is None:
            return None
        return self._sumsq.sqrt()[0]


def ademamix_schedule(step: int, alpha: float, beta1: float, beta3: float, T_alpha_beta3: Optional[float]):
    if T_alpha_beta3 is None:
        return float(alpha), float(beta3)
    f = step / T_alpha_beta3
    lb1, lb3 = math.log(beta1), math.log(beta3)
    return min(step * alpha / T_alpha_beta3, alpha), min(math.exp(lb1 * lb3 / ((1.0 - f) * lb3 + f * lb1)), beta3)


def _check_ademamix_group(lr, betas, eps, weight_decay, T_alpha_beta3):
    if not 0.0 <= lr:
        raise ValueError(f"Invalid learning rate: {lr}")
    if not 0.0 <= eps:
        raise ValueError(f"Invalid epsilon value: {eps}")
    if len(betas) != 3 or not all(0.0 <= b < 1.0 for b in betas):
        raise ValueError(f"Invalid beta parameters: {betas}, expected three in [0, 1)")
    if not 0.0 <= weight_decay:
        raise ValueError(f"Invalid weight_decay value: {weight_decay}")
    if T_alpha_beta3 is not None:
        if not T_alpha_beta3 > 0:
            raise ValueError(f"Invalid T_alpha_beta3 value: {T_alpha_beta3} (must be > 0, or None)")
        if betas[0] == 0.0 or betas[2] == 0.0:
            raise ValueError(f"Invalid beta parameters: {betas}: the T_alpha_beta3 schedule needs beta1 > 0 and beta3 > 0")


class FusedAdEMAMix(torch.optim.Optimizer):

    def __init__(self, params, lr: float = 1e-3, betas=(0.9, 0.999, 0.9999), eps: float = 1e-8, weight_decay: float = 0, alpha: float = 5.0,
                 T_alpha_beta3: Optional[float] = None, max_grad_norm: Optional[float] = None):
        _check_ademamix_group(lr, betas, eps, weight_decay, T_alpha_beta3)
        super().__init__(params, dict(lr=lr, betas=betas, eps=eps, weight_decay=weight_decay, alpha=alpha, T_alpha_beta3=T_alpha_beta3))
        for g in self.param_groups:
            _check_ademamix_group(g["lr"], g["betas"], g["eps"], g["weight_decay"], g["T_alpha_beta3"])
        if len(self.param_groups) > L.ADAMW_MAX_GROUPS:
            raise ValueError(f"at most {L.ADAMW_MAX_GROUPS} parameter groups")
        self.max_grad_norm = max_grad_norm
        self._table = None
        self._key = None
        self._sumsq = None
        self._sumsq_ws = None

    def _build(self, items):
        dev = items[0][1].device
        for _, p in items:
            for k in ("exp_avg", "exp_avg_sq", "exp_avg_slow"):
                t = self.state[p][k]
                if t.device != dev or t.dtype != torch.float32 or t.shape != p.shape or not t.is_contiguous():
                    raise L.LnxError(f"FusedAdEMAMix: state '{k}' must be a contiguous fp32 tensor of the parameter's shape on its device")
        arr, blk = _adamw_descs(self.state, items)
        slow = (C.c_uint64 * len(items))(*(self.state[p]["exp_avg_slow"].data_ptr() for _, p in items))
        descs = np.frombuffer(arr, dtype=np.uint8)
        host = torch.from_numpy(np.concatenate([descs, np.frombuffer(slow, dtype=np.uint8)]))
        self._table = (host.to(dev), len(descs), len(items), blk)
        if self._sumsq is None or self._sumsq.device != dev:
            self._sumsq = torch.zeros(1, device=dev, dtype=torch.float32)
        if self._sumsq_ws is None or self._sumsq_ws.device != dev or self._sumsq_ws.numel() < blk:
            self._sumsq_ws = torch.empty(blk, device=dev, dtype=torch.float32)

    @torch.no_grad()
    def step(self, closure=None):
        loss = None
        if closure is not None:
            with torch.enable_grad():
                loss = closure()
        items = []
        for gi, group in enumerate(self.param_groups):
            for p in group["params"]:
                if p.grad is None:
                    continue
                if not p.is_cuda or p.dtype != torch.float32 or not p.is_contiguous() or p.grad.dtype != torch.float32 or not p.grad.is_contiguous():
                    raise L.LnxError("FusedAdEMAMix needs contiguous fp32 parameters and gradients on the GPU")
                st = self.state[p]
                if len(st) == 0:
                    st["step"] = 0
                    st["exp_avg"] = torch.zeros_like(p, memory_format=torch.preserve_format)
                    st["exp_avg_sq"] = torch.zeros_like(p, memory_format=torch.preserve_format)
                    st["exp_avg_slow"] = torch.zeros_like(p, memory_format=torch.preserve_format)
                st["step"] = int(st["step"]) + 1
                items.append((gi, p))
        if not items:
            return loss
        slots, items = _slot_items(self.state, items, "FusedAdEMAMix")
        key = tuple((si, p.data_ptr(), p.grad.data_ptr(), self.state[p]["exp_avg"].data_ptr(), self.state[p]["exp_avg_sq"].data_ptr(),
                     self.state[p]["exp_avg_slow"].data_ptr()) for si, p in items)
        if key != self._key:
            self._build(items)
            self._key = key
        h = L.AdEMAMixHyper()
        h.ngroups = len(slots)
        for (gi, t), si in slots.items():
            group = self.param_groups[gi]
            b1, b2, b3 = group["betas"]
            alpha_t, beta3_t = ademamix_schedule(t, group["alpha"], b1, b3, group["T_alpha_beta3"])
            h.lr[si], h.beta1[si], h.beta2[si], h.eps[si], h.weight_decay[si] = group["lr"], b1, b2, group["eps"], group["weight_decay"]
            h.bias_c1[si], h.bias_c2[si] = 1.0 - b1 ** float(t), 1.0 - b2 ** float(t)
            h.omb1[si], h.omb2[si] = 1.0 - b1, 1.0 - b2
            h.alpha_t[si], h.beta3_t[si], h.omb3[si] = alpha_t, beta3_t, 1.0 - beta3_t
        table, nbytes, n, blocks = self._table
        lib = L.lib()
        stream = C.c_void_p(torch.cuda.current_stream().cuda_stream)
        clip = self.max_grad_norm is not None and self.max_grad_norm > 0
        if clip:
            L.check(lib.lnx_grad_sumsq(C.c_void_p(table.data_ptr()), n, blocks, C.c_void_p(self._sumsq.data_ptr()), C.c_void_p(self._sumsq_ws.data_ptr()), stream),
                    "lnx_grad_sumsq")
        L.check(lib.lnx_ademamix_step(table.data_ptr(), table.data_ptr() + nbytes, n, blocks, C.byref(h), self._sumsq.data_ptr() if clip else None,
                                      self.max_grad_norm if clip else 0.0, stream), "lnx_ademamix_step")
        return loss

    def grad_norm(self) -> Optional[torch.Tensor]:
        if self._sumsq is None or self.max_grad_norm is None:
            return None
        return self._sumsq.sqrt()[0]


def zeropower_via_newtonschulz5(G: torch.Tensor, steps: int = 5) -> torch.Tensor:
    from . import ops

    assert G.ndim == 2, "2-D matrices (4-D conv weights are flattened by the optimizer)"
    if not G.is_cuda:
        raise L.LnxError("linnaeus_amd.optim.Muon runs on the HIP GEMM kernels: parameters must be on the GPU")
    a, b, c = 3.4445, -4.7750, 2.0315
    X = G.bfloat16()
    tall = G.size(0) > G.size(1)
    if tall:
        X = X.t()
    m, n = X.shape
    mp, npad = (m + 7) // 8 * 8, (n + 7) // 8 * 8
    X = X / (X.float().norm() + 1e-7).to(torch.bfloat16)
    if (mp, npad) != (m, n):
        X = torch.nn.functional.pad(X, (0, npad - n, 0, mp - m))
    X = X.contiguous()
    dev = X.device
    cvec = torch.full((mp,), c, device=dev, dtype=torch.float32)
    ones = None
    A = torch.empty(mp, mp, device=dev, dtype=torch.bfloat16)
    Bm = torch.empty(mp, mp, device=dev, dtype=torch.bfloat16)
    Xn = torch.empty(mp, npad, device=dev, dtype=torch.bfloat16)
    for _ in range(steps):
        XT = X.t().contiguous()
        ops.gemm_nt(X, X, A)
        ops.gemm_nt(A, A, Bm, gamma=cvec, res=A.float() * b)
        ops.gemm_nt(Bm, XT, Xn, res=X.float() * a)
        X, Xn = Xn, X
    X = X[:m, :n]
    return (X.t() if tall else X).contiguous()


class Muon(torch.optim.Optimizer):

    def __init__(self, params, lr=0.02, weight_decay=0.01, momentum=0.95, nesterov=True, ns_steps=5, strict=False):
        if not 0.0 <= lr:
            raise ValueError(f"Invalid learning rate: {lr}")
        if not 0.0 <= momentum < 1.0:
            raise ValueError(f"Invalid momentum value: {momentum}")
        if not 0.0 <= weight_decay:
            raise ValueError(f"Invalid weight_decay value: {weight_decay}")
        params = list(params)
        if strict:
            for p in (q for g in params for q in (g["params"] if isinstance(g, dict) else [g])):
                if p.dim() not in (2, 4):
                    raise ValueError(f"Muon optimizer requires 2D or 4D parameters, got shape {p.shape}")
        super().__init__(params, dict(lr=lr, weight_decay=weight_decay, momentum=momentum, nesterov=nesterov, ns_steps=ns_steps))

    @torch.no_grad()
    def step(self, closure=None):
        loss = None
        if closure is not None:
            with torch.enable_grad():
                loss = closure()
        for group in self.param_groups:
            lr, wd, mom = group["lr"], group["weight_decay"], group["momentum"]
            for p in group["params"]:
                if p.grad is None:
                    continue
                g = p.grad
                if wd != 0:
                    p.mul_(1 - lr * wd)
                st = self.state[p]
                if "momentum_buffer" not in st:
                    st["momentum_buffer"] = torch.zeros_like(g)
                buf = st["momentum_buffer"]
                buf.lerp_(g, 1 - mom)
                g = g.lerp_(buf, mom) if group["nesterov"] else buf.clone()
                g2 = g.view(g.size(0), -1) if g.ndim == 4 else g
                o = zeropower_via_newtonschulz5(g2, steps=group["ns_steps"])
                if p.dim() == 4:
                    scaling = max(1, p.size(0) / (p.size(1) * p.size(2) * p.size(3))) ** 0.5
                else:
                    scaling = max(1, p.size(-2) / p.size(-1)) ** 0.5
                p.add_(o.view_as(p).to(p.dtype), alpha=-lr * scaling)
        return loss
```

Measured before the change: 13360 images/sec.

## Fuse bf16 operand copy refresh into AdamW step, skip forward weight prep

The AdamW kernel now writes the updated fp32 parameters straight into the plan's bf16 (or fp32) operand copies, including transposed and permuted layouts through a 64x64 shared-memory tile path. When the optimizer has refreshed every operand, the next forward skips its lnx_prep_weights pass. This removes one full read of the parameters plus a separate kernel launch each step. In exchange it adds validity tracking through pointer and version tuples, a larger descriptor ABI, and tiled update blocks that may coalesce less well than the flat path.

```diff
diff --git a/include/lnx.h b/include/lnx.h
--- a/include/lnx.h
+++ b/include/lnx.h
@@ -414,6 +414,14 @@
     int64_t n;
     int group;
     int block_start;
+    void* w;
+    void* w_t;
+    int rows, cols;
+    int ld, ld_t;
+    int P;
+    int w_dtype;
+    int ublock_start;
+    int pad_;
 } lnx_adamw_desc;
 typedef struct lnx_adamw_hyper {
     int ngroups;
@@ -423,6 +431,7 @@
     float omb1[LNX_ADAMW_MAX_GROUPS], omb2[LNX_ADAMW_MAX_GROUPS];
 } lnx_adamw_hyper;
 int lnx_adamw_blocks(int64_t numel);
+int lnx_adamw_update_blocks(const lnx_adamw_desc* desc);
 int lnx_grad_sumsq(const lnx_adamw_desc* descs_dev, int ndesc, int total_blocks, float* out, float* ws, void* stream);
 int lnx_adamw_step(const lnx_adamw_desc* descs_dev, int ndesc, int total_blocks, const lnx_adamw_hyper* hyper, const float* sumsq, float max_norm,
                    void* stream);
@@ -612,6 +621,11 @@
 int lnx_plan_set_meta_stream(lnx_plan* p, int mode);
 int lnx_plan_segment_params(const lnx_plan* p, int segment, int* idx_out, int max_out);
 
+int lnx_plan_adamw_copy(const lnx_plan* p, int param, lnx_adamw_desc* desc);
+int lnx_plan_operands_fresh(lnx_plan* p);
+int64_t lnx_plan_refresh_count(const lnx_plan* p);
+int lnx_plan_operand_arena(const lnx_plan* p, int64_t* offset, int64_t* bytes);
+
 #ifdef __cplusplus
 }
 #endif
diff --git a/linnaeus_amd/_lib.py b/linnaeus_amd/_lib.py
--- a/linnaeus_amd/_lib.py
+++ b/linnaeus_amd/_lib.py
@@ -73,7 +73,21 @@
 
 
 class AdamWDesc(C.Structure):
+    _fields_ = [("p", C.c_void_p), ("m", C.c_void_p), ("v", C.c_void_p), ("g", C.c_void_p), ("n", C.c_int64), ("group", C.c_int), ("block_start", C.c_int),
+                ("w", C.c_void_p), ("w_t", C.c_void_p), ("rows", C.c_int), ("cols", C.c_int), ("ld", C.c_int), ("ld_t", C.c_int), ("P", C.c_int),
+                ("w_dtype", C.c_int), ("ublock_start", C.c_int), ("pad_", C.c_int)]
+
+
+class AdamWDescV1(C.Structure):
     _fields_ = [("p", C.c_void_p), ("m", C.c_void_p), ("v", C.c_void_p), ("g", C.c_void_p), ("n", C.c_int64), ("group", C.c_int), ("block_start", C.c_int)]
+
+
+def adamw_copy_abi() -> bool:
+    return hasattr(lib(), "lnx_adamw_update_blocks")
+
+
+def adamw_desc_type():
+    return AdamWDesc if adamw_copy_abi() else AdamWDescV1
 
 
 class AdamWHyper(C.Structure):
@@ -144,6 +158,13 @@
         _lib.lnx_nt_kernel_launches.restype = C.c_int64
         _lib.lnx_convmlp_bwd_ws_floats.restype = C.c_int64
         _lib.lnx_meta_heads_bwd_part_floats.restype = C.c_int64
+        if hasattr(_lib, "lnx_plan_refresh_count"):
+            _lib.lnx_plan_refresh_count.restype = C.c_int64
+            _lib.lnx_plan_refresh_count.argtypes = [C.c_void_p]
+            _lib.lnx_plan_adamw_copy.argtypes = [C.c_void_p, C.c_int, C.POINTER(AdamWDesc)]
+            _lib.lnx_plan_operands_fresh.argtypes = [C.c_void_p]
+            _lib.lnx_plan_operand_arena.argtypes = [C.c_void_p, C.POINTER(C.c_int64), C.POINTER(C.c_int64)]
+            _lib.lnx_adamw_update_blocks.argtypes = [C.POINTER(AdamWDesc)]
         if hasattr(_lib, "lnx_ademamix_step"):
             _lib.lnx_ademamix_step.argtypes = [C.c_void_p, C.c_void_p, C.c_int, C.c_int, C.POINTER(AdEMAMixHyper), C.c_void_p, C.c_float, C.c_void_p]
         if hasattr(_lib, "lnx_gradnorm_sumsq"):
@@ -181,7 +202,7 @@
     "lnx_dwconv7_fwd", "lnx_dwconv7_wgrad",
     "lnx_gemm_nt_group_ok", "lnx_gemm_nt_group", "lnx_rope_cos_table", "lnx_rope_cos_table_hd", "lnx_rope_cossin_table_hd", "lnx_rope_cos_tables", "lnx_attn_bwd_ws_floats", "lnx_attn_bwd_ws_floats_hd", "lnx_attn_fwd", "lnx_attn_bwd", "lnx_attn_bwd_flush", "lnx_attn_bwd_discard", "lnx_attn_dispatch", "lnx_last_attn_kernel",
     "lnx_im2col_stem", "lnx_scale_cast", "lnx_layerscale_bwd", "lnx_layerscale_apply_wgrad", "lnx_fill_rows", "lnx_colsum_rows",
-    "lnx_agg2_fwd", "lnx_agg2_bwd", "lnx_pack_meta", "lnx_meta_heads_supported", "lnx_meta_heads_fwd", "lnx_meta_heads_bwd", "lnx_meta_heads_bwd_part_floats", "lnx_prep_weights", "lnx_prep_blocks", "lnx_softce", "lnx_softce_multi", "lnx_stem_fwd", "lnx_stem_fwd_ok", "lnx_adamw_blocks", "lnx_grad_sumsq", "lnx_adamw_step", "lnx_ademamix_step", "lnx_gradnorm_sumsq", "lnx_gradnorm_update",
+    "lnx_agg2_fwd", "lnx_agg2_bwd", "lnx_pack_meta", "lnx_meta_heads_supported", "lnx_meta_heads_fwd", "lnx_meta_heads_bwd", "lnx_meta_heads_bwd_part_floats", "lnx_prep_weights", "lnx_prep_blocks", "lnx_softce", "lnx_softce_multi", "lnx_stem_fwd", "lnx_stem_fwd_ok", "lnx_adamw_blocks", "lnx_adamw_update_blocks", "lnx_grad_sumsq", "lnx_adamw_step", "lnx_ademamix_step", "lnx_gradnorm_sumsq", "lnx_gradnorm_update",
     "lnx_metrics_table_sizes", "lnx_metrics_update", "lnx_predict",
     "lnx_mix_rows", "lnx_mix_meta",
     "lnx_aug_pointwise", "lnx_aug_saturation", "lnx_aug_rowstat", "lnx_aug_rescale", "lnx_aug_affine", "lnx_aug_stencil", "lnx_erase_rects", "lnx_u8hwc_to_f32chw",
@@ -189,6 +210,7 @@
     "lnx_plan_create", "lnx_plan_destroy", "lnx_plan_workspace_bytes", "lnx_plan_num_params", "lnx_plan_param_name",
     "lnx_plan_param_numel", "lnx_plan_num_drop_calls", "lnx_plan_logits_numel", "lnx_plan_logits_offset", "lnx_plan_logits_ld",
     "lnx_plan_bind", "lnx_plan_forward", "lnx_plan_backward", "lnx_plan_backward_into", "lnx_plan_segment_params", "lnx_plan_profile_begin", "lnx_plan_profile_end", "lnx_plan_profile_begin_spans", "lnx_plan_profile_end_ex", "lnx_plan_set_wgrad_stream", "lnx_plan_set_meta_stream",
+    "lnx_plan_adamw_copy", "lnx_plan_operands_fresh", "lnx_plan_refresh_count", "lnx_plan_operand_arena",
 ]
 
 
diff --git a/linnaeus_amd/csrc/optim.hip b/linnaeus_amd/csrc/optim.hip
--- a/linnaeus_amd/csrc/optim.hip
+++ b/linnaeus_amd/csrc/optim.hip
@@ -4,6 +4,11 @@
 namespace {
 
 constexpr int OPT_ELEMS = 4096;
+constexpr int OPT_TILE = 64;
+
+__host__ __device__ inline bool adamw_tiled(const lnx_adamw_desc& d) {
+    return (d.w != nullptr || d.w_t != nullptr) && (d.w_t != nullptr || d.P > 1 || d.ld != d.cols);
+}
 
 __device__ __forceinline__ int find_desc_index(const lnx_adamw_desc* __restrict__ descs, int ndesc, int block) {
     int lo = 0, hi = ndesc - 1;
@@ -66,17 +71,41 @@
     }
 }
 
+__device__ __forceinline__ int find_update_desc(const lnx_adamw_desc* __restrict__ descs, int ndesc, int block) {
+    int lo = 0, hi = ndesc - 1;
+    while (lo < hi) {
+        const int mid = (lo + hi + 1) >> 1;
+        if (descs[mid].ublock_start <= block) lo = mid;
+        else hi = mid - 1;
+    }
+    return lo;
+}
+
+__device__ __forceinline__ void store_copy(void* base, int dt, int64_t idx, float v) {
+    if (dt == LNX_BF16) reinterpret_cast<bf16_t*>(base)[idx] = from_f<bf16_t>(v);
+    else reinterpret_cast<float*>(base)[idx] = v;
+}
+__device__ __forceinline__ void store_copy4(void* base, int dt, int64_t idx, const float4& v) {
+    if (dt == LNX_BF16) {
+        uint2 pk;
+        bf16_t* hh = reinterpret_cast<bf16_t*>(&pk);
+        hh[0] = from_f<bf16_t>(v.x); hh[1] = from_f<bf16_t>(v.y); hh[2] = from_f<bf16_t>(v.z); hh[3] = from_f<bf16_t>(v.w);
+        *reinterpret_cast<uint2*>(reinterpret_cast<bf16_t*>(base) + idx) = pk;
+    } else {
+        *reinterpret_cast<float4*>(reinterpret_cast<float*>(base) + idx) = v;
+    }
+}
+
 __global__ __launch_bounds__(256) void adamw_kernel(const lnx_adamw_desc* __restrict__ descs, int ndesc, const lnx_adamw_hyper h, const float* __restrict__ sumsq,
                                                     float max_norm) {
-    const lnx_adamw_desc& d = find_desc(descs, ndesc, blockIdx.x);
+    __shared__ float tile[OPT_TILE][OPT_TILE + 1];
+    const lnx_adamw_desc& d = descs[find_update_desc(descs, ndesc, blockIdx.x)];
     const int gi = d.group;
     const float lr = h.lr[gi], b1 = h.beta1[gi], b2 = h.beta2[gi], eps = h.eps[gi], wd = h.weight_decay[gi];
     const float omb1 = h.omb1[gi], omb2 = h.omb2[gi];
     const float step_size = lr / h.bias_c1[gi], inv_sqrt_bc2 = 1.0f / sqrtf(h.bias_c2[gi]);
     float coef = 1.0f;
     if (sumsq != nullptr && max_norm > 0.f) coef = fminf(1.0f, max_norm / (sqrtf(*sumsq) + 1e-6f));
-    const int64_t base = (int64_t)(blockIdx.x - d.block_start) * OPT_ELEMS;
-    const int64_t end = min(d.n, base + OPT_ELEMS);
     auto upd = [&](float g, float& p, float& m, float& v) __attribute__((always_inline)) {
         g *= coef;
         p *= 1.0f - lr * wd;
@@ -85,7 +114,89 @@
         const float denom = sqrtf(v) * inv_sqrt_bc2 + eps;
         p -= step_size * (m / denom);
     };
-    const bool vec = ((reinterpret_cast<uintptr_t>(d.p) | reinterpret_cast<uintptr_t>(d.g) | reinterpret_cast<uintptr_t>(d.m) | reinterpret_cast<uintptr_t>(d.v)) & 15) == 0;
+    if (adamw_tiled(d)) {
+        const int rows = d.rows, cols = d.cols, dt = d.w_dtype;
+        const int tiles_k = (cols + OPT_TILE - 1) / OPT_TILE;
+        const int tt = blockIdx.x - d.ublock_start;
+        const int r0 = (tt / tiles_k) * OPT_TILE, k0 = (tt % tiles_k) * OPT_TILE;
+        const int Cc = d.P > 1 ? cols / d.P : 1;
+        auto dst_col = [&](int k) {
+            if (d.P <= 1) return k;
+            const int cc = k / d.P;
+            return (k - cc * d.P) * Cc + cc;
+        };
+        const bool vec4 = (cols & 3) == 0 &&
+                          ((reinterpret_cast<uintptr_t>(d.p) | reinterpret_cast<uintptr_t>(d.g) | reinterpret_cast<uintptr_t>(d.m) | reinterpret_cast<uintptr_t>(d.v)) & 15) == 0;
+        if (vec4) {
+            constexpr int R = OPT_TILE / 16;
+            const int tr = threadIdx.x >> 4, tk = (threadIdx.x & 15) * 4;
+            const int k = k0 + tk;
+            float4 g4[R], p4[R], m4[R], v4[R];
+#pragma unroll
+            for (int r = 0; r < R; ++r) {
+                const int row = r0 + 16 * r + tr;
+                const bool ok = row < rows && k < cols;
+                const int64_t i = ok ? (int64_t)row * cols + k : 0;
+                g4[r] = *reinterpret_cast<const float4*>(d.g + i);
+                p4[r] = *reinterpret_cast<const float4*>(d.p + i);
+                m4[r] = *reinterpret_cast<const float4*>(d.m + i);
+                v4[r] = *reinterpret_cast<const float4*>(d.v + i);
+            }
+            const bool wvec = d.w != nullptr && d.P <= 1 && (reinterpret_cast<uintptr_t>(d.w) & 15) == 0 && ((int64_t)d.ld * (dt == LNX_BF16 ? 2 : 4)) % 16 == 0;
+#pragma unroll
+            for (int r = 0; r < R; ++r) {
+                const int row = r0 + 16 * r + tr;
+                if (row < rows && k < cols) {
+                    const int64_t i = (int64_t)row * cols + k;
+                    upd(g4[r].x, p4[r].x, m4[r].x, v4[r].x);
+                    upd(g4[r].y, p4[r].y, m4[r].y, v4[r].y);
+                    upd(g4[r].z, p4[r].z, m4[r].z, v4[r].z);
+                    upd(g4[r].w, p4[r].w, m4[r].w, v4[r].w);
+                    *reinterpret_cast<float4*>(d.p + i) = p4[r];
+                    *reinterpret_cast<float4*>(d.m + i) = m4[r];
+                    *reinterpret_cast<float4*>(d.v + i) = v4[r];
+                    const float pv[4] = {p4[r].x, p4[r].y, p4[r].z, p4[r].w};
+                    if (wvec) {
+                        store_copy4(d.w, dt, (int64_t)row * d.ld + k, p4[r]);
+                    } else if (d.w != nullptr) {
+#pragma unroll
+                        for (int j = 0; j < 4; ++j) store_copy(d.w, dt, (int64_t)row * d.ld + dst_col(k + j), pv[j]);
+                    }
+#pragma unroll
+                    for (int j = 0; j < 4; ++j) tile[tk + j][16 * r + tr] = pv[j];
+                }
+            }
+        } else {
+            for (int e = threadIdx.x; e < OPT_TILE * OPT_TILE; e += 256) {
+                const int rr = e / OPT_TILE, kk = e % OPT_TILE;
+                const int row = r0 + rr, k = k0 + kk;
+                if (row < rows && k < cols) {
+                    const int64_t i = (int64_t)row * cols + k;
+                    float p = d.p[i], m = d.m[i], v = d.v[i];
+                    upd(d.g[i], p, m, v);
+                    d.p[i] = p;
+                    d.m[i] = m;
+                    d.v[i] = v;
+                    if (d.w != nullptr) store_copy(d.w, dt, (int64_t)row * d.ld + dst_col(k), p);
+                    tile[kk][rr] = p;
+                }
+            }
+        }
+        if (d.w_t == nullptr) return;
+        __syncthreads();
+        for (int e = threadIdx.x; e < OPT_TILE * OPT_TILE; e += 256) {
+            const int kk = e / OPT_TILE, rr = e % OPT_TILE;
+            const int row = r0 + rr, k = k0 + kk;
+            if (row < rows && k < cols) store_copy(d.w_t, dt, (int64_t)dst_col(k) * d.ld_t + row, tile[kk][rr]);
+        }
+        return;
+    }
+    const int64_t base = (int64_t)(blockIdx.x - d.ublock_start) * OPT_ELEMS;
+    const int64_t end = min(d.n, base + OPT_ELEMS);
+    void* const wc = d.w;
+    const int wdt = d.w_dtype;
+    const bool vec = ((reinterpret_cast<uintptr_t>(d.p) | reinterpret_cast<uintptr_t>(d.g) | reinterpret_cast<uintptr_t>(d.m) | reinterpret_cast<uintptr_t>(d.v) |
+                       reinterpret_cast<uintptr_t>(wc)) & 15) == 0;
     int64_t done = base;
     if (vec) {
         constexpr int R = OPT_ELEMS / 1024;
@@ -114,6 +225,7 @@
                     *reinterpret_cast<float4*>(d.p + i) = p4[r];
                     *reinterpret_cast<float4*>(d.m + i) = m4[r];
                     *reinterpret_cast<float4*>(d.v + i) = v4[r];
+                    if (wc != nullptr) store_copy4(wc, wdt, i, p4[r]);
                 }
             }
         }
@@ -125,6 +237,7 @@
         d.p[i] = p;
         d.m[i] = m;
         d.v[i] = v;
+        if (wc != nullptr) store_copy(wc, wdt, i, p);
     }
 }
 
@@ -201,6 +314,12 @@
 
 extern "C" int lnx_adamw_blocks(int64_t numel) { return (int)((numel + OPT_ELEMS - 1) / OPT_ELEMS); }
 
+extern "C" int lnx_adamw_update_blocks(const lnx_adamw_desc* d) {
+    if (d == nullptr) return 0;
+    if (!adamw_tiled(*d)) return lnx_adamw_blocks(d->n);
+    return ((d->rows + OPT_TILE - 1) / OPT_TILE) * ((d->cols + OPT_TILE - 1) / OPT_TILE);
+}
+
 extern "C" int lnx_grad_sumsq(const lnx_adamw_desc* descs_dev, int ndesc, int total_blocks, float* out, float* ws, void* stream) {
     LNX_CHECK(descs_dev && ndesc > 0 && total_blocks > 0 && out && ws, "lnx_grad_sumsq: bad arguments (ws: total_blocks floats)");
     hipStream_t st = (hipStream_t)stream;
diff --git a/linnaeus_amd/csrc/plan.cpp b/linnaeus_amd/csrc/plan.cpp
--- a/linnaeus_amd/csrc/plan.cpp
+++ b/linnaeus_amd/csrc/plan.cpp
@@ -110,6 +110,11 @@
 
     int64_t o_descs = 0, n_descs = 0, prep_blocks = 0;
     int64_t n_descs_t = 0, n_descs_f = 0, prep_blocks_f = 0;
+    std::vector<lnx_prep_desc> prep_host;
+    std::vector<int> prep_param;
+    int64_t arena_lo = 0, arena_hi = 0;
+    bool operands_fresh = false;
+    int64_t refresh_count = 0;
     int64_t o_patches, o_stem_pre, o_stem_mean, o_stem_rstd;
     int64_t o_stage_out[4];
     int64_t o_tok[2];
@@ -829,7 +834,13 @@
         if (e1 > arena_end) arena_end = e1;
         if (e2 > arena_end) arena_end = e2;
     }
-    HIPRUN(hipMemset(p->ws, 0, (size_t)arena_end));
+    p->arena_lo = p->all_w.empty() ? 0 : p->all_w.front()->off;
+    p->arena_hi = arena_end;
+    for (int s = 0; s < 2; ++s)
+        for (auto& k : p->conv[s])
+            if (k.w49 + (int64_t)49 * p->c.dims[s] * 4 > p->arena_hi) p->arena_hi = k.w49 + (int64_t)49 * p->c.dims[s] * 4;
+    HIPRUN(hipMemset(p->ws, 0, (size_t)p->arena_hi));
+    p->prep_param.clear();
     std::vector<lnx_prep_desc> d;
     int blk = 0;
     auto push_w = [&](OpW* w) {
@@ -847,6 +858,7 @@
         e.block_start = blk;
         blk += lnx_prep_blocks(e.rows, e.ld, e.cols, e.ld_t, e.dst_t != nullptr);
         d.push_back(e);
+        p->prep_param.push_back(w->param);
     };
     const bool split = p->esz == 2;
     for (OpW* w : p->all_w)
@@ -864,6 +876,7 @@
             e.block_start = blk;
             blk += lnx_prep_blocks(e.rows, e.ld, e.cols, 0, 0);
             d.push_back(e);
+            p->prep_param.push_back(k.dww);
         }
     p->n_descs_t = (int64_t)d.size();
     p->prep_blocks = blk;
@@ -895,6 +908,8 @@
     }
     HIPRUN(hipMemcpy(p->ws + p->o_descs, d.data(), d.size() * sizeof(lnx_prep_desc), hipMemcpyHostToDevice));
     HIPRUN(hipDeviceSynchronize());
+    p->prep_host = d;
+    p->operands_fresh = false;
     p->bound = true;
     p->fwd_done = false;
     return 0;
@@ -1332,9 +1347,14 @@
         for (int i = 0; i < p->n_drop; ++i) p->mask_host[i] = drop_mask[i];
     p->last_meta = meta;
 
-    RUN(lnx_prep_weights(c.at<lnx_prep_desc>(p->o_descs), (int)p->n_descs_t, (int)p->prep_blocks, cf.dtype, stream));
-    if (p->n_descs_f > 0)
-        RUN(lnx_prep_weights(c.at<lnx_prep_desc>(p->o_descs) + p->n_descs_t, (int)p->n_descs_f, (int)p->prep_blocks_f, LNX_F32, stream));
+    const bool fresh = p->operands_fresh && !cf.fp8;
+    p->operands_fresh = false;
+    if (!fresh) {
+        RUN(lnx_prep_weights(c.at<lnx_prep_desc>(p->o_descs), (int)p->n_descs_t, (int)p->prep_blocks, cf.dtype, stream));
+        if (p->n_descs_f > 0)
+            RUN(lnx_prep_weights(c.at<lnx_prep_desc>(p->o_descs) + p->n_descs_t, (int)p->n_descs_f, (int)p->prep_blocks_f, LNX_F32, stream));
+        ++p->refresh_count;
+    }
     if (cf.fp8)
         for (int s = 0; s < 2; ++s)
             for (auto& k : p->rope[s]) {
@@ -1970,6 +1990,56 @@
     return lnx_plan_backward(p, dlogits, dfeats, -1, stream);
 }
 
+extern "C" int lnx_plan_adamw_copy(const lnx_plan* p, int param, lnx_adamw_desc* desc) {
+    if (!p || !p->bound || !desc || param < 0 || param >= (int)p->names.size()) {
+        lnx_set_error("lnx_plan_adamw_copy: plan is not bound / bad arguments");
+        return -1;
+    }
+    desc->w = desc->w_t = nullptr;
+    desc->rows = desc->cols = desc->ld = desc->ld_t = desc->P = desc->w_dtype = 0;
+    int found = 0;
+    for (size_t i = 0; i < p->prep_host.size(); ++i) {
+        if (p->prep_param[i] != param) continue;
+        if (found++) {
+            lnx_set_error("lnx_plan_adamw_copy: parameter %s has more than one arena copy", p->names[param].c_str());
+            return -1;
+        }
+        const lnx_prep_desc& e = p->prep_host[i];
+        desc->rows = e.rows;
+        desc->cols = e.cols;
+        if (e.mode == LNX_PREP_DW49) {
+            desc->w_t = e.dst;
+            desc->ld = e.cols;
+            desc->ld_t = e.rows;
+            desc->w_dtype = LNX_F32;
+            continue;
+        }
+        desc->w = e.dst;
+        desc->w_t = e.dst_t;
+        desc->ld = e.ld;
+        desc->ld_t = e.ld_t;
+        desc->P = e.mode == LNX_PREP_CONV_PERM ? e.P : 0;
+        desc->w_dtype = (int64_t)i < p->n_descs_t ? p->c.dtype : LNX_F32;
+    }
+    return found;
+}
+
+extern "C" int lnx_plan_operands_fresh(lnx_plan* p) {
+    if (!p || !p->bound) FAIL("lnx_plan_operands_fresh: plan is not bound");
+    if (p->c.fp8) FAIL("lnx_plan_operands_fresh: fp8 plans quantise their MXFP8 weight copies in the refresh; it cannot be skipped");
+    p->operands_fresh = true;
+    return 0;
+}
+
+extern "C" int64_t lnx_plan_refresh_count(const lnx_plan* p) { return p ? p->refresh_count : -1; }
+
+extern "C" int lnx_plan_operand_arena(const lnx_plan* p, int64_t* offset, int64_t* bytes) {
+    if (!p || !p->bound || !offset || !bytes) FAIL("lnx_plan_operand_arena: plan is not bound / bad arguments");
+    *offset = p->arena_lo;
+    *bytes = p->arena_hi - p->arena_lo;
+    return 0;
+}
+
 extern "C" int lnx_plan_segment_params(const lnx_plan* p, int segment, int* idx_out, int max_out) {
     if (!p || segment < 0 || segment > 3) return -1;
     int n = 0;
diff --git a/linnaeus_amd/loss.py b/linnaeus_amd/loss.py
--- a/linnaeus_amd/loss.py
+++ b/linnaeus_amd/loss.py
@@ -357,7 +357,7 @@
 
 
 def gradnorm_desc_table(slices, base_ptr: int):
-    arr = (L.AdamWDesc * len(slices))()
+    arr = (L.adamw_desc_type() * len(slices))()
     blk = 0
     for d, (off, n) in zip(arr, slices):
         d.g, d.n, d.group, d.block_start = base_ptr + 4 * off, n, 0, blk
diff --git a/linnaeus_amd/model.py b/linnaeus_amd/model.py
--- a/linnaeus_amd/model.py
+++ b/linnaeus_amd/model.py
@@ -311,6 +311,55 @@
         for st in self._plans.values():
             if st.get("handle") is not None and L.lib().lnx_plan_set_meta_stream(st["handle"], self._meta_stream) < 0:
                 L.check(1, "lnx_plan_set_meta_stream")
+
+    def _refresh_target(self):
+        st = self._active
+        if st is None or self._fp8 or not st["train"] or st.get("destroyed") or st["ptrs"] is None:
+            return None
+        return st if self._operand_copies(st) is not None else None
+
+    def _operand_key(self, st):
+        return (id(st), st["handle"].value, st["ws"].data_ptr(), st["ptrs"])
+
+    def _operand_copies(self, st):
+        cached = st.get("copies")
+        if cached is not None and cached[0] is st["ptrs"]:
+            return cached[1]
+        lib = L.lib()
+        out = {}
+        for i, p_ in enumerate(st["params"]):
+            d = L.AdamWDesc()
+            rc = lib.lnx_plan_adamw_copy(st["handle"], i, C.byref(d))
+            if rc < 0:
+                L.check(1, "lnx_plan_adamw_copy")
+            if rc > 0:
+                if id(p_) in out:
+                    out = None
+                    break
+                out[id(p_)] = d
+        st["copies"] = (st["ptrs"], out)
+        return out
+
+    def _operands_written(self, st) -> None:
+        st["fresh"] = (st["ptrs"], tuple(p_._version for p_ in st["params"]))
+
+    def _operands_stale(self, ids=None) -> None:
+        for st in self._plans.values():
+            if st.get("fresh") is not None and (ids is None or any(id(q) in ids for q in st["params"])):
+                st["fresh"] = None
+
+    invalidate_operands = _operands_stale
+
+    def operand_arena(self, st=None) -> torch.Tensor:
+        st = st or self._active
+        off, nb = C.c_int64(), C.c_int64()
+        L.check(L.lib().lnx_plan_operand_arena(st["handle"], C.byref(off), C.byref(nb)), "lnx_plan_operand_arena")
+        base = (st["ws"].data_ptr() + 255) // 256 * 256 - st["ws"].data_ptr()
+        return st["ws"][base + off.value: base + off.value + nb.value]
+
+    def refresh_count(self, st=None) -> int:
+        st = st or self._active
+        return int(L.lib().lnx_plan_refresh_count(st["handle"]))
 
     def _destroy_plan(self, st) -> None:
         if st.get("destroyed"):
@@ -465,6 +514,10 @@
                       logit_off=[lib.lnx_plan_logits_offset(handle, i) for i in range(len(tasks))],
                       logit_ld=[lib.lnx_plan_logits_ld(handle, i) for i in range(len(tasks))], tasks=tasks, B=B, fwd_id=0, train=bool(train))
             self._plans[key] = st
+            if train:
+                from . import optim
+
+                optim.register_operand_provider(self)
         self._ensure_bound(st)
         return st
 
@@ -602,6 +655,9 @@
         feats = torch.empty(B, self._dims[3], device=x.device, dtype=torch.float32)
         logits = torch.empty(max(st["logits_numel"], 1), device=x.device, dtype=torch.float32)
         mask = st.get("drop_mask") if drop is not None else None
+        fresh, st["fresh"] = st.get("fresh"), None
+        if fresh is not None and fresh[0] is st["ptrs"] and fresh[1] == tuple(p_._version for p_ in st["params"]):
+            L.check(L.lib().lnx_plan_operands_fresh(st["handle"]), "lnx_plan_operands_fresh")
         L.check(L.lib().lnx_plan_forward(
             st["handle"], C.c_void_p(x.data_ptr()), C.c_void_p(meta.data_ptr()) if meta is not None else None,
             C.c_void_p(drop.data_ptr()) if drop is not None else None, mask, C.c_void_p(feats.data_ptr()),
diff --git a/linnaeus_amd/optim.py b/linnaeus_amd/optim.py
--- a/linnaeus_amd/optim.py
+++ b/linnaeus_amd/optim.py
@@ -1,5 +1,7 @@
 import ctypes as C
 import math
+import os
+import weakref
 from typing import Optional
 
 import numpy as np
@@ -17,16 +19,42 @@
     return slots, [(slots[(gi, int(state[p]["step"]))], p) for gi, p in items]
 
 
-def _adamw_descs(state, items):
+_operand_providers = weakref.WeakSet()
+
+
+def register_operand_provider(model) -> None:
+    _operand_providers.add(model)
+
+
+def _operands_stale(items) -> set:
+    ids = {id(p) for _, p in items}
+    for m in list(_operand_providers):
+        m._operands_stale(ids)
+    return ids
+
+
+def _adamw_descs(state, items, copies=None):
     lib = L.lib()
-    arr = (L.AdamWDesc * len(items))()
-    blk = 0
+    new_abi = L.adamw_copy_abi()
+    arr = (L.adamw_desc_type() * len(items))()
+    blk = ublk = 0
     for i, (gi, p) in enumerate(items):
         st = state[p]
-        arr[i].p, arr[i].m, arr[i].v, arr[i].g = p.data_ptr(), st["exp_avg"].data_ptr(), st["exp_avg_sq"].data_ptr(), p.grad.data_ptr()
-        arr[i].n, arr[i].group, arr[i].block_start = p.numel(), gi, blk
+        d = arr[i]
+        d.p, d.m, d.v, d.g = p.data_ptr(), st["exp_avg"].data_ptr(), st["exp_avg_sq"].data_ptr(), p.grad.data_ptr()
+        d.n, d.group, d.block_start = p.numel(), gi, blk
         blk += lib.lnx_adamw_blocks(C.c_int64(p.numel()))
-    return arr, blk
+        if not new_abi:
+            ublk = blk
+            continue
+        c = copies.get(id(p)) if copies else None
+        if c is not None:
+            if c.rows * c.cols != p.numel():
+                raise L.LnxError(f"operand copy of a {tuple(p.shape)} parameter is described as [{c.rows}, {c.cols}]")
+            d.w, d.w_t, d.rows, d.cols, d.ld, d.ld_t, d.P, d.w_dtype = c.w, c.w_t, c.rows, c.cols, c.ld, c.ld_t, c.P, c.w_dtype
+        d.ublock_start = ublk
+        ublk += lib.lnx_adamw_update_blocks(C.byref(d))
+    return arr, blk, ublk
 
 
 class FusedAdamW(torch.optim.Optimizer):
@@ -42,11 +70,21 @@
         self._sumsq = None
         self._sumsq_ws = None
 
-    def _build(self, items):
+    def _refresh_target(self, ids):
+        if os.environ.get("LNX_ADAMW_REFRESH", "1") == "0" or not _operand_providers or not L.adamw_copy_abi():
+            return None
+        for m in list(_operand_providers):
+            st = m._refresh_target()
+            if st is not None and all(id(q) in ids for q in st["params"]):
+                return m, st
+        return None
+
+    def _build(self, items, target=None):
         dev = items[0][1].device
-        arr, blk = _adamw_descs(self.state, items)
+        copies = target[0]._operand_copies(target[1]) if target is not None else None
+        arr, blk, ublk = _adamw_descs(self.state, items, copies)
         host = torch.from_numpy(np.frombuffer(arr, dtype=np.uint8).copy())
-        self._table = (host.to(dev), len(items), blk)
+        self._table = (host.to(dev), len(items), blk, ublk)
         if self._sumsq is None or self._sumsq.device != dev:
             self._sumsq = torch.zeros(1, device=dev, dtype=torch.float32)
         if self._sumsq_ws is None or self._sumsq_ws.device != dev or self._sumsq_ws.numel() < blk:
@@ -75,9 +113,11 @@
         if not items:
             return loss
         slots, items = _slot_items(self.state, items, "FusedAdamW")
+        target = self._refresh_target(_operands_stale(items))
         key = tuple((si, p.data_ptr(), p.grad.data_ptr(), self.state[p]["exp_avg"].data_ptr(), self.state[p]["exp_avg_sq"].data_ptr()) for si, p in items)
+        key = (target[0]._operand_key(target[1]) if target is not None else None, key)
         if key != self._key:
-            self._build(items)
+            self._build(items, target)
             self._key = key
         h = L.AdamWHyper()
         h.ngroups = len(slots)
@@ -87,15 +127,17 @@
             h.lr[si], h.beta1[si], h.beta2[si], h.eps[si], h.weight_decay[si] = group["lr"], b1, b2, group["eps"], group["weight_decay"]
             h.bias_c1[si], h.bias_c2[si] = 1.0 - b1 ** float(t), 1.0 - b2 ** float(t)
             h.omb1[si], h.omb2[si] = 1.0 - b1, 1.0 - b2
-        table, n, blocks = self._table
+        table, n, blocks, ublocks = self._table
         lib = L.lib()
         stream = C.c_void_p(torch.cuda.current_stream().cuda_stream)
         clip = self.max_grad_norm is not None and self.max_grad_norm > 0
         if clip:
             L.check(lib.lnx_grad_sumsq(C.c_void_p(table.data_ptr()), n, blocks, C.c_void_p(self._sumsq.data_ptr()), C.c_void_p(self._sumsq_ws.data_ptr()), stream),
                     "lnx_grad_sumsq")
-        L.check(lib.lnx_adamw_step(C.c_void_p(table.data_ptr()), n, blocks, C.byref(h), C.c_void_p(self._sumsq.data_ptr()) if clip else None,
+        L.check(lib.lnx_adamw_step(C.c_void_p(table.data_ptr()), n, ublocks, C.byref(h), C.c_void_p(self._sumsq.data_ptr()) if clip else None,
                                    C.c_float(self.max_grad_norm if clip else 0.0), stream), "lnx_adamw_step")
+        if target is not None:
+            target[0]._operands_written(target[1])
         return loss
 
     def grad_norm(self) -> Optional[torch.Tensor]:
@@ -151,7 +193,7 @@
                 t = self.state[p][k]
                 if t.device != dev or t.dtype != torch.float32 or t.shape != p.shape or not t.is_contiguous():
                     raise L.LnxError(f"FusedAdEMAMix: state '{k}' must be a contiguous fp32 tensor of the parameter's shape on its device")
-        arr, blk = _adamw_descs(self.state, items)
+        arr, blk, _ = _adamw_descs(self.state, items)
         slow = (C.c_uint64 * len(items))(*(self.state[p]["exp_avg_slow"].data_ptr() for _, p in items))
         descs = np.frombuffer(arr, dtype=np.uint8)
         host = torch.from_numpy(np.concatenate([descs, np.frombuffer(slow, dtype=np.uint8)]))
@@ -185,6 +227,7 @@
         if not items:
             return loss
         slots, items = _slot_items(self.state, items, "FusedAdEMAMix")
+        _operands_stale(items)
         key = tuple((si, p.data_ptr(), p.grad.data_ptr(), self.state[p]["exp_avg"].data_ptr(), self.state[p]["exp_avg_sq"].data_ptr(),
                      self.state[p]["exp_avg_slow"].data_ptr()) for si, p in items)
         if key != self._key:
```

New measurement: 13430 images/sec (median of 4 runs). About the same (+0.5%).
